# NealB/Bijective-BWT

Measured on AMD Instinct MI355X. Metric: BWTS build MB/s on 1 GiB input (+ inverse MB/s); bit-exact round-trip, higher is better.
Workload: dtype u8

## Files before the change

### bijective-bwt_amd/__init__.py

```python
import ctypes
import os
import subprocess

import numpy as np

PKG_DIR = os.path.dirname(os.path.abspath(__file__))
LIB_PATH = os.environ.get("BWTS_LIB_OVERRIDE") or os.path.join(PKG_DIR, "libbwts_hip.so")

KINDS = {"uniform256": 0, "zipf": 1, "dna": 2, "text": 3}

K_NAMES = ["histogram", "keybuild", "radix_hist", "radix_scan", "radix_scatter", "rerank", "lyndon", "emit",
           "lf_build", "walk", "listrank", "walk_emit", "other", "radix_scatter_main", "round"]
K_COUNT = len(K_NAMES)
MAX_ROUND_STATS = 40
H_NAMES = ["init", "module_load", "io_alloc", "staging_alloc", "arena_alloc"]
H_COUNT = len(H_NAMES)

EXPORTS = [
    "bwts_ctx_create", "bwts_ctx_destroy", "bwts_ctx_release_memory", "bwts_forward", "bwts_inverse", "bwts_forward_sink", "bwts_inverse_sink",
    "bwts_forward_device", "bwts_inverse_device", "bwts_last_timings", "bwts_kernel_class_name", "bwts_strerror",
    "bwts_last_hip_error", "bwts_set_timing", "bwts_host_alloc", "bwts_host_free", "bwts_host_cost_name",
    "bwts_forward_batch", "bwts_inverse_batch",
    "bwts_forward_segments", "bwts_inverse_segments", "bwts_forward_segments_device", "bwts_inverse_segments_device",
]
MTF_EXPORTS = [
    "bwts_mtf_forward_device", "bwts_mtf_inverse_device", "bwts_mtf_forward", "bwts_mtf_inverse",
    "bwts_mtf_forward_segments_device", "bwts_mtf_inverse_segments_device", "bwts_mtf_forward_segments", "bwts_mtf_inverse_segments",
]
EC_EXPORTS = [
    "bwts_ec_bound", "bwts_ec_bound_segments", "bwts_ec_decoded_size", "bwts_ec_encode_device", "bwts_ec_decode_device",
    "bwts_ec_encode", "bwts_ec_decode", "bwts_ec_encode_segments_device", "bwts_ec_decode_segments_device",
]
E_FORMAT, E_SPACE = -8, -9
ZRL_EXPORTS = [
    "bwts_zrl_bound", "bwts_zrl_encode_device", "bwts_zrl_decode_device", "bwts_zrl_encode", "bwts_zrl_decode",
    "bwts_zrl_encode_segments_device", "bwts_zrl_decode_segments_device",
]
PACK_EXPORTS = [
    "bwts_crc32_device", "bwts_crc32_segments_device", "bwts_pack_bound", "bwts_unpack_size",
    "bwts_pack_device", "bwts_unpack_device", "bwts_pack", "bwts_unpack",
    "bwts_pack_bound_v", "bwts_pack_device_v", "bwts_pack_v",
]
E_CHECKSUM = -10
TEST_EXPORTS = [
    "bwts_generate_device", "bwts_device_alloc", "bwts_device_free", "bwts_copy_to_device", "bwts_copy_to_host",
    "bwts_device_equal", "bwts_debug_sort_pairs", "bwts_debug_suffix_array", "bwts_debug_lyndon",
    "bwts_debug_chunk_plan", "bwts_debug_inverse_arena", "bwts_debug_forward_arena", "bwts_debug_wide_forward_arena", "bwts_debug_inverse_report",
    "bwts_debug_forward_report", "bwts_debug_segments_plan", "bwts_debug_segments_report",
    "bwts_debug_mtf_plan", "bwts_debug_last_spans", "bwts_debug_ec_plan", "bwts_debug_crc_plan",
    "bwts_debug_zrl_plan",
]
INV_REPORT_FIELDS = ["g", "mark", "outcome", "s", "virtual", "node_cap", "nu", "nu2", "ucap_first", "second_collect",
                     "listed_classes", "mom_fallback", "unit_rank", "kc", "kt", "form"]
INV_MARKS = {0: "log", 1: "sentinel", 2: "bytemap", 3: "moments"}
INV_OUTCOMES = {0: "DONE", 1: "RETRY_DENSE", 2: "AMBIGUOUS", 3: "NEED_LOG", 255: "ERROR"}
INV_FORMS = {0: "narrow", 1: "wide", 2: "wide_compact", 3: "segmented"}
SEG_PLANS = {0: "lane", 1: "shared", 2: "shared_nomem"}
FWD_HEADER_WORDS, FWD_ROUND_WORDS = 48, 12
FWD_SORT_WORDS = FWD_HEADER_WORDS + MAX_ROUND_STATS * FWD_ROUND_WORDS
FWD_HEADER_FIELDS = ["cyclic", "n", "k", "sigma", "bits", "msym", "key_bits", "varlen", "hstep", "keys", "flags_outside_rank", "tied0",
                     "rank_early", "form", "no_chunks", "need_sa", "end", "rest_chunks", "rest_big", "rest_tiles", "rounds", "directory",
                     "order_sort", "left"]
FWD_DIRECT_WORD = 36
FWD_DIRECT = {0: "not_tried", 1: "settled", 2: "fallback_group", 3: "fallback_depth"}
FWD_CHUNK_FIELDS = ["S", "maxchunks", "a_small", "big0", "m_exit", "m_stay", "groups", "wide_possible", "fsl", "compactions",
                    "compactions_skipped", "enqueued_behind_last"]
FWD_ROUND_FIELDS = {"sparse": ["form", "h", "in", "out", "splits", "probe", "m_big", "whole", "skip_next"],
                    "chunks": ["form", "h", "in", "out", "splits", "chunks_in", "chunks_out", "big_in", "big_stays", "big_leaves", "nchunks"],
                    "tiles": ["form", "h", "in", "out", "splits", "m_big"],
                    "direct": ["form", "h", "in", "out", "splits"]}
FWD_FORMS = {0: "none", 1: "sparse", 2: "chunks", 3: "tiles", 4: "direct"}
FWD_KEYS = {0: "wide", 1: "split32", 2: "split40"}
FWD_NO_CHUNKS = {0: None, 1: "short_list", 2: "knob", 3: "no_room_store", 4: "no_room_order", 5: "no_room_biglist"}
FWD_ENDS = {0: "none", 1: "empty", 2: "stable"}
FWD_PROBES = {0: "short_list", 1: "ran", 2: "skipped"}


class BwtsError(RuntimeError):
    def __init__(self, code, msg):
        super().__init__("bwts error %d: %s" % (code, msg))
        self.code = code


class KernelStat(ctypes.Structure):
    _fields_ = [("ms", ctypes.c_double), ("launches", ctypes.c_uint64), ("elems", ctypes.c_uint64),
                ("alg_bytes", ctypes.c_uint64)]


class Timings(ctypes.Structure):
    _fields_ = [("total_ms", ctypes.c_double), ("h2d_ms", ctypes.c_double), ("d2h_ms", ctypes.c_double),
                ("n", ctypes.c_uint64), ("factors", ctypes.c_uint64), ("rounds", ctypes.c_uint32),
                ("lyndon_rounds", ctypes.c_uint32), ("key_symbols", ctypes.c_uint32), ("key_bits", ctypes.c_uint32),
                ("active_after_round0", ctypes.c_uint64), ("unvisited", ctypes.c_uint64), ("device_bytes", ctypes.c_uint64),
                ("round_active", ctypes.c_uint64 * MAX_ROUND_STATS), ("k", KernelStat * K_COUNT),
                ("host_ms", ctypes.c_double * H_COUNT), ("attempts", ctypes.c_uint32), ("reserved_", ctypes.c_uint32)]

    def as_dict(self):
        d = {f: getattr(self, f) for f, _ in self._fields_ if f not in ("k", "round_active", "host_ms")}
        d["host_ms"] = {H_NAMES[i]: float(self.host_ms[i]) for i in range(H_COUNT)}
        d["round_active"] = [int(v) for v in self.round_active[: max(int(self.rounds), 1)]]
        d["kernels"] = {K_NAMES[i]: {"ms": self.k[i].ms, "launches": self.k[i].launches, "elems": self.k[i].elems,
                                     "alg_bytes": self.k[i].alg_bytes} for i in range(K_COUNT) if self.k[i].launches}
        return d


SINK_FN = ctypes.CFUNCTYPE(ctypes.c_int, ctypes.c_void_p, ctypes.c_void_p, ctypes.c_uint64)

_lib = None


def build(verbose=False):
    out = None if verbose else subprocess.DEVNULL
    subprocess.check_call(["make", "-C", PKG_DIR, "-j4", "all"], stdout=out)


def lib():
    global _lib
    if _lib is None:
        if not os.path.exists(LIB_PATH):
            raise BwtsError(-2, "libbwts_hip.so is not built (run `make -C bijective-bwt_amd` or __graft_entry__.build())")
        L = ctypes.CDLL(LIB_PATH)
        vp, u64, i32 = ctypes.c_void_p, ctypes.c_uint64, ctypes.c_int
        L.bwts_ctx_create.argtypes = [ctypes.POINTER(vp), i32]
        L.bwts_ctx_destroy.argtypes = [vp]
        L.bwts_ctx_destroy.restype = None
        L.bwts_ctx_release_memory.argtypes = [vp]
        L.bwts_ctx_release_memory.restype = ctypes.c_int
        for name in ("bwts_forward", "bwts_inverse", "bwts_forward_device", "bwts_inverse_device"):
            getattr(L, name).argtypes = [vp, vp, u64, vp]
        L.bwts_last_timings.argtypes = [vp, ctypes.POINTER(Timings)]
        L.bwts_kernel_class_name.argtypes = [i32]
        L.bwts_kernel_class_name.restype = ctypes.c_char_p
        L.bwts_strerror.argtypes = [i32]
        L.bwts_strerror.restype = ctypes.c_char_p
        L.bwts_last_hip_error.argtypes = [vp]
        L.bwts_set_timing.argtypes = [vp, i32]
        L.bwts_host_alloc.argtypes = [vp, u64, ctypes.POINTER(vp)]
        L.bwts_host_free.argtypes = [vp, vp]
        for name in ("bwts_forward_batch", "bwts_inverse_batch"):
            getattr(L, name).argtypes = [vp, i32, ctypes.POINTER(vp), ctypes.POINTER(u64), ctypes.POINTER(vp)]
        for name in ("bwts_forward_segments", "bwts_inverse_segments", "bwts_forward_segments_device", "bwts_inverse_segments_device"):
            getattr(L, name).argtypes = [vp, vp, vp, u64, vp]
        for name in ("bwts_mtf_forward", "bwts_mtf_inverse", "bwts_mtf_forward_device", "bwts_mtf_inverse_device"):
            getattr(L, name).argtypes = [vp, vp, u64, vp]
        for name in ("bwts_mtf_forward_segments", "bwts_mtf_inverse_segments", "bwts_mtf_forward_segments_device", "bwts_mtf_inverse_segments_device"):
            getattr(L, name).argtypes = [vp, vp, vp, u64, vp]
        L.bwts_debug_mtf_plan.argtypes = [u64, ctypes.POINTER(u64)]
        L.bwts_debug_last_spans.argtypes = [vp, ctypes.POINTER(ctypes.c_double), u64]
        L.bwts_ec_bound.argtypes = [u64]
        L.bwts_ec_bound.restype = u64
        L.bwts_ec_bound_segments.argtypes = [vp, u64, ctypes.POINTER(u64)]
        L.bwts_ec_decoded_size.argtypes = [vp, u64, ctypes.POINTER(u64)]
        for name in ("bwts_ec_encode_device", "bwts_ec_decode_device", "bwts_ec_encode", "bwts_ec_decode"):
            getattr(L, name).argtypes = [vp, vp, u64, vp, u64, ctypes.POINTER(u64)]
        L.bwts_ec_encode_segments_device.argtypes = [vp, vp, vp, u64, vp, u64, vp]
        L.bwts_ec_decode_segments_device.argtypes = [vp, vp, vp, vp, u64, vp]
        L.bwts_debug_ec_plan.argtypes = [u64, ctypes.POINTER(u64)]
        L.bwts_zrl_bound.argtypes = [u64]
        L.bwts_zrl_bound.restype = u64
        for name in ("bwts_zrl_encode_device", "bwts_zrl_encode"):
            getattr(L, name).argtypes = [vp, vp, u64, vp, u64, ctypes.POINTER(u64)]
        for name in ("bwts_zrl_decode_device", "bwts_zrl_decode"):
            getattr(L, name).argtypes = [vp, vp, u64, vp, u64]
        L.bwts_zrl_encode_segments_device.argtypes = [vp, vp, vp, u64, vp, u64, vp]
        L.bwts_zrl_decode_segments_device.argtypes = [vp, vp, vp, vp, u64, vp]
        L.bwts_debug_zrl_plan.argtypes = [u64, ctypes.POINTER(u64)]
        L.bwts_crc32_device.argtypes = [vp, vp, u64, ctypes.POINTER(ctypes.c_uint32)]
        L.bwts_crc32_segments_device.argtypes = [vp, vp, vp, u64, vp]
        L.bwts_pack_bound.argtypes = [u64, u64]
        L.bwts_pack_bound.restype = u64
        L.bwts_unpack_size.argtypes = [vp, u64, ctypes.POINTER(u64), ctypes.POINTER(u64)]
        for name in ("bwts_pack_device", "bwts_pack"):
            getattr(L, name).argtypes = [vp, vp, u64, u64, vp, u64, ctypes.POINTER(u64)]
        u32 = ctypes.c_uint32
        L.bwts_pack_bound_v.argtypes = [u32, u64, u64]
        L.bwts_pack_bound_v.restype = u64
        for name in ("bwts_pack_device_v", "bwts_pack_v"):
            getattr(L, name).argtypes = [vp, u32, vp, u64, u64, vp, u64, ctypes.POINTER(u64)]
        for name in ("bwts_unpack_device", "bwts_unpack"):
            getattr(L, name).argtypes = [vp, vp, u64, vp, u64, ctypes.POINTER(u64)]
        L.bwts_debug_crc_plan.argtypes = [u64, ctypes.POINTER(u64)]
        for name in ("bwts_forward_sink", "bwts_inverse_sink"):
            getattr(L, name).argtypes = [vp, vp, u64, SINK_FN, vp]
        L.bwts_generate_device.argtypes = [vp, i32, u64, u64, vp]
        L.bwts_device_alloc.argtypes = [vp, u64, ctypes.POINTER(vp)]
        L.bwts_device_free.argtypes = [vp, vp]
        L.bwts_copy_to_device.argtypes = [vp, vp, vp, u64]
        L.bwts_copy_to_host.argtypes = [vp, vp, vp, u64]
        L.bwts_device_equal.argtypes = [vp, vp, vp, u64, ctypes.POINTER(i32)]
        L.bwts_debug_sort_pairs.argtypes = [vp, vp, vp, u64, i32]
        L.bwts_debug_suffix_array.argtypes = [vp, vp, u64, vp]
        L.bwts_debug_lyndon.argtypes = [vp, vp, u64, vp, u64, ctypes.POINTER(u64)]
        L.bwts_debug_chunk_plan.argtypes = [u64, u64, ctypes.POINTER(u64)]
        L.bwts_debug_inverse_arena.argtypes = [u64, i32, i32, ctypes.POINTER(u64)]
        L.bwts_debug_forward_arena.argtypes = [u64, ctypes.POINTER(u64)]
        L.bwts_debug_wide_forward_arena.argtypes = [u64, i32, i32, u64, ctypes.POINTER(u64)]
        L.bwts_debug_inverse_report.argtypes = [vp, ctypes.POINTER(u64), u64, ctypes.POINTER(u64)]
        L.bwts_debug_forward_report.argtypes = [vp, ctypes.POINTER(u64), u64, ctypes.POINTER(u64)]
        L.bwts_debug_segments_plan.argtypes = [vp, u64, ctypes.POINTER(u64)]
        L.bwts_debug_segments_report.argtypes = [vp, ctypes.POINTER(u64)]
        _lib = L
    return _lib


def _u8(data):
    if isinstance(data, np.ndarray):
        return np.ascontiguousarray(data, dtype=np.uint8)
    return np.frombuffer(bytes(data), dtype=np.uint8)


class DeviceBuffer:

    def __init__(self, ctx, nbytes):
        self.ctx, self.nbytes = ctx, int(nbytes)
        p = ctypes.c_void_p()
        ctx._check(lib().bwts_device_alloc(ctx._h, self.nbytes, ctypes.byref(p)))
        self.ptr = p.value

    def free(self):
        if self.ptr:
            lib().bwts_device_free(self.ctx._h, self.ptr)
            self.ptr = None

    def upload(self, data):
        a = _u8(data)
        assert a.size <= self.nbytes
        self.ctx._check(lib().bwts_copy_to_device(self.ctx._h, self.ptr, a.ctypes.data, a.size))

    def download(self, nbytes=None):
        n = self.nbytes if nbytes is None else int(nbytes)
        out = np.empty(n, dtype=np.uint8)
        self.ctx._check(lib().bwts_copy_to_host(self.ctx._h, out.ctypes.data, self.ptr, n))
        return out


class Context:

    def __init__(self, device=0):
        self._h = None
        h = ctypes.c_void_p()
        rc = lib().bwts_ctx_create(ctypes.byref(h), int(device))
        if rc != 0:
            raise BwtsError(rc, lib().bwts_strerror(rc).decode())
        self._h = h
        self.device = int(device)

    def close(self):
        if self._h:
            lib().bwts_ctx_destroy(self._h)
            self._h = None

    def __enter__(self):
        return self

    def __exit__(self, *exc):
        self.close()

    def __del__(self):
        try:
            self.close()
        except Exception:
            pass

    def release_memory(self):
        self._check(lib().bwts_ctx_release_memory(self._h))

    def _check(self, rc):
        if rc != 0:
            msg = lib().bwts_strerror(rc).decode()
            if rc == -4:
                msg += " (hipError %d)" % lib().bwts_last_hip_error(self._h)
            raise BwtsError(rc, msg)

    def _host(self, fn, data):
        a = _u8(data)
        if a.size == 0:
            raise BwtsError(-1, "empty input (the reference fails on empty files: map_file.c:36-40)")
        out = np.empty_like(a)
        self._check(fn(self._h, a.ctypes.data, a.size, out.ctypes.data))
        return out

    def forward(self, data):
        return self._host(lib().bwts_forward, data)

    def inverse(self, data):
        return self._host(lib().bwts_inverse, data)

    def forward_device(self, d_in, n, d_out):
        self._check(lib().bwts_forward_device(self._h, _ptr(d_in), int(n), _ptr(d_out)))

    def inverse_device(self, d_in, n, d_out):
        self._check(lib().bwts_inverse_device(self._h, _ptr(d_in), int(n), _ptr(d_out)))

    def set_timing(self, level=2):
        self._check(lib().bwts_set_timing(self._h, int(level)))

    def _sink(self, fn, data):
        a = _u8(data)
        pieces = []

        def take(_user, ptr, length):
            pieces.append(ctypes.string_at(ptr, length))
            return 0

        cb = SINK_FN(take)
        self._check(fn(self._h, a.ctypes.data, a.size, cb, None))
        return np.frombuffer(b"".join(pieces), dtype=np.uint8)

    def forward_sink(self, data):
        return self._sink(lib().bwts_forward_sink, data)

    def inverse_sink(self, data):
        return self._sink(lib().bwts_inverse_sink, data)

    def host_alloc(self, nbytes):
        p = ctypes.c_void_p()
        self._check(lib().bwts_host_alloc(self._h, int(nbytes), ctypes.byref(p)))
        arr = np.ctypeslib.as_array(ctypes.cast(p, ctypes.POINTER(ctypes.c_uint8)), shape=(int(nbytes),))
        return arr, p.value

    def host_free(self, ptr):
        self._check(lib().bwts_host_free(self._h, ptr))

    def _batch(self, fn, arrays):
        arrs = [_u8(a) for a in arrays]
        outs = [np.empty_like(a) for a in arrs]
        k = len(arrs)
        ins_p = (ctypes.c_void_p * k)(*[a.ctypes.data for a in arrs])
        outs_p = (ctypes.c_void_p * k)(*[o.ctypes.data for o in outs])
        ns = (ctypes.c_uint64 * k)(*[a.size for a in arrs])
        self._check(fn(self._h, k, ins_p, ns, outs_p))
        return outs

    def forward_batch(self, arrays):
        return self._batch(lib().bwts_forward_batch, arrays)

    def inverse_batch(self, arrays):
        return self._batch(lib().bwts_inverse_batch, arrays)

    def _segments(self, fn, data, lengths, out=None):
        a = _u8(data)
        ls = np.ascontiguousarray(lengths, dtype=np.uint64)
        if int(ls.sum(dtype=np.uint64)) != a.size or (ls.size and int(ls.max()) > a.size):
            raise BwtsError(-1, "segment lengths do not add up to the input's size")
        if out is None:
            out = np.empty_like(a)
        elif out.size < a.size:
            raise BwtsError(-1, "output smaller than the input")
        self._check(fn(self._h, a.ctypes.data, ls.ctypes.data, ls.size, out.ctypes.data))
        return out

    def forward_segments(self, data, lengths, out=None):
        return self._segments(lib().bwts_forward_segments, data, lengths, out)

    def inverse_segments(self, data, lengths, out=None):
        return self._segments(lib().bwts_inverse_segments, data, lengths, out)

    def forward_segments_device(self, d_in, lengths, d_out):
        ls = np.ascontiguousarray(lengths, dtype=np.uint64)
        self._check(lib().bwts_forward_segments_device(self._h, _ptr(d_in), ls.ctypes.data, ls.size, _ptr(d_out)))

    def inverse_segments_device(self, d_in, lengths, d_out):
        ls = np.ascontiguousarray(lengths, dtype=np.uint64)
        self._check(lib().bwts_inverse_segments_device(self._h, _ptr(d_in), ls.ctypes.data, ls.size, _ptr(d_out)))

    def mtf_forward(self, data):
        return self._host(lib().bwts_mtf_forward, data)

    def mtf_inverse(self, data):
        return self._host(lib().bwts_mtf_inverse, data)

    def mtf_forward_device(self, d_in, n, d_out):
        self._check(lib().bwts_mtf_forward_device(self._h, _ptr(d_in), int(n), _ptr(d_out)))

    def mtf_inverse_device(self, d_in, n, d_out):
        self._check(lib().bwts_mtf_inverse_device(self._h, _ptr(d_in), int(n), _ptr(d_out)))

    def mtf_forward_segments(self, data, lengths, out=None):
        return self._segments(lib().bwts_mtf_forward_segments, data, lengths, out)

    def mtf_inverse_segments(self, data, lengths, out=None):
        return self._segments(lib().bwts_mtf_inverse_segments, data, lengths, out)

    def mtf_forward_segments_device(self, d_in, lengths, d_out):
        ls = np.ascontiguousarray(lengths, dtype=np.uint64)
        self._check(lib().bwts_mtf_forward_segments_device(self._h, _ptr(d_in), ls.ctypes.data, ls.size, _ptr(d_out)))

    def mtf_inverse_segments_device(self, d_in, lengths, d_out):
        ls = np.ascontiguousarray(lengths, dtype=np.uint64)
        self._check(lib().bwts_mtf_inverse_segments_device(self._h, _ptr(d_in), ls.ctypes.data, ls.size, _ptr(d_out)))

    def ec_encode(self, data, out_cap=None):
        a = _u8(data)
        if a.size == 0:
            raise BwtsError(-1, "empty input")
        out = np.empty(ec_bound(a.size) if out_cap is None else int(out_cap), dtype=np.uint8)
        got = ctypes.c_uint64(0)
        self._check(lib().bwts_ec_encode(self._h, a.ctypes.data, a.size, out.ctypes.data, out.size, ctypes.byref(got)))
        return out[:got.value].copy()

    def ec_decode(self, stream):
        a = _u8(stream)
        n = ec_decoded_size(a)
        out = np.empty(n, dtype=np.uint8)
        got = ctypes.c_uint64(0)
        self._check(lib().bwts_ec_decode(self._h, a.ctypes.data, a.size, out.ctypes.data, out.size, ctypes.byref(got)))
        return out[:got.value]

    def ec_encode_device(self, d_in, n, d_out, out_cap):
        got = ctypes.c_uint64(0)
        self._check(lib().bwts_ec_encode_device(self._h, _ptr(d_in), int(n), _ptr(d_out), int(out_cap), ctypes.byref(got)))
        return int(got.value)

    def ec_decode_device(self, d_in, in_bytes, d_out, out_cap):
        got = ctypes.c_uint64(0)
        self._check(lib().bwts_ec_decode_device(self._h, _ptr(d_in), int(in_bytes), _ptr(d_out), int(out_cap), ctypes.byref(got)))
        return int(got.value)

    def ec_encode_segments_device(self, d_in, lengths, d_out, out_cap):
        ls = np.ascontiguousarray(lengths, dtype=np.uint64)
        sizes = np.zeros(ls.size, dtype=np.uint64)
        self._check(lib().bwts_ec_encode_segments_device(self._h, _ptr(d_in), ls.ctypes.data, ls.size, _ptr(d_out), int(out_cap), sizes.ctypes.data))
        return sizes

    def ec_decode_segments_device(self, d_in, stream_bytes, lengths, d_out):
        ls = np.ascontiguousarray(lengths, dtype=np.uint64)
        sb = np.ascontiguousarray(stream_bytes, dtype=np.uint64)
        if sb.size != ls.size:
            raise BwtsError(-1, "one stream size per segment")
        self._check(lib().bwts_ec_decode_segments_device(self._h, _ptr(d_in), sb.ctypes.data, ls.ctypes.data, ls.size, _ptr(d_out)))

    def zrl_encode(self, data, out_cap=None):
        a = _u8(data)
        if a.size == 0:
            raise BwtsError(-1, "empty input")
        out = np.empty(a.size if out_cap is None else int(out_cap), dtype=np.uint8)
        got = ctypes.c_uint64(0)
        self._check(lib().bwts_zrl_encode(self._h, a.ctypes.data, a.size, out.ctypes.data, out.size, ctypes.byref(got)))
        return out[:got.value].copy()

    def zrl_decode(self, coded, n):
        a = _u8(coded)
        out = np.empty(int(n), dtype=np.uint8)
        self._check(lib().bwts_zrl_decode(self._h, a.ctypes.data, a.size, out.ctypes.data, out.size))
        return out

    def zrl_encode_device(self, d_in, n, d_out, out_cap):
        got = ctypes.c_uint64(0)
        self._check(lib().bwts_zrl_encode_device(self._h, _ptr(d_in), int(n), _ptr(d_out), int(out_cap), ctypes.byref(got)))
        return int(got.value)

    def zrl_decode_device(self, d_in, in_bytes, d_out, n):
        self._check(lib().bwts_zrl_decode_device(self._h, _ptr(d_in), int(in_bytes), _ptr(d_out), int(n)))

    def zrl_encode_segments_device(self, d_in, lengths, d_out, out_cap):
        ls = np.ascontiguousarray(lengths, dtype=np.uint64)
        sizes = np.zeros(ls.size, dtype=np.uint64)
        self._check(lib().bwts_zrl_encode_segments_device(self._h, _ptr(d_in), ls.ctypes.data, ls.size, _ptr(d_out), int(out_cap), sizes.ctypes.data))
        return sizes

    def zrl_decode_segments_device(self, d_in, in_lengths, lengths, d_out):
        ls = np.ascontiguousarray(lengths, dtype=np.uint64)
        il = np.ascontiguousarray(in_lengths, dtype=np.uint64)
        if il.size != ls.size:
            raise BwtsError(-1, "one coded length per segment")
        self._check(lib().bwts_zrl_decode_segments_device(self._h, _ptr(d_in), il.ctypes.data, ls.ctypes.data, ls.size, _ptr(d_out)))

    def crc32_device(self, d_in, n):
        got = ctypes.c_uint32(0)
        self._check(lib().bwts_crc32_device(self._h, _ptr(d_in), int(n), ctypes.byref(got)))
        return int(got.value)

    def crc32_segments_device(self, d_in, lengths):
        ls = np.ascontiguousarray(lengths, dtype=np.uint64)
        crcs = np.zeros(ls.size, dtype=np.uint32)
        self._check(lib().bwts_crc32_segments_device(self._h, _ptr(d_in), ls.ctypes.data, ls.size, crcs.ctypes.data))
        return crcs

    def pack(self, data, block_bytes=0, out_cap=None, version=1):
        a = _u8(data)
        if a.size == 0:
            raise BwtsError(-1, "empty input")
        out = np.empty(pack_bound(a.size, block_bytes, version) if out_cap is None else int(out_cap), dtype=np.uint8)
        got = ctypes.c_uint64(0)
        self._check(lib().bwts_pack_v(self._h, int(version), a.ctypes.data, a.size, int(block_bytes), out.ctypes.data, out.size, ctypes.byref(got)))
        return out[:got.value].copy()

    def unpack(self, frame, out=None):
        a = _u8(frame)
        if out is None:
            out = np.empty(unpack_size(a)[0], dtype=np.uint8)
        got = ctypes.c_uint64(0)
        self._check(lib().bwts_unpack(self._h, a.ctypes.data, a.size, out.ctypes.data, out.size, ctypes.byref(got)))
        return out[:got.value]

    def pack_device(self, d_in, n, block_bytes, d_out, out_cap, version=1):
        got = ctypes.c_uint64(0)
        self._check(lib().bwts_pack_device_v(self._h, int(version), _ptr(d_in), int(n), int(block_bytes), _ptr(d_out), int(out_cap), ctypes.byref(got)))
        return int(got.value)

    def unpack_device(self, d_in, in_bytes, d_out, out_cap):
        got = ctypes.c_uint64(0)
        self._check(lib().bwts_unpack_device(self._h, _ptr(d_in), int(in_bytes), _ptr(d_out), int(out_cap), ctypes.byref(got)))
        return int(got.value)

    def forward_into(self, a, out):
        self._check(lib().bwts_forward(self._h, a.ctypes.data, a.size, out.ctypes.data))

    def inverse_into(self, a, out):
        self._check(lib().bwts_inverse(self._h, a.ctypes.data, a.size, out.ctypes.data))

    def timings(self):
        t = Timings()
        self._check(lib().bwts_last_timings(self._h, ctypes.byref(t)))
        return t

    def alloc(self, nbytes):
        return DeviceBuffer(self, nbytes)

    def generate(self, kind, seed, n, d_out):
        self._check(lib().bwts_generate_device(self._h, KINDS[kind], int(seed), int(n), _ptr(d_out)))

    def device_equal(self, d_a, d_b, nbytes):
        eq = ctypes.c_int(0)
        self._check(lib().bwts_device_equal(self._h, _ptr(d_a), _ptr(d_b), int(nbytes), ctypes.byref(eq)))
        return bool(eq.value)

    def debug_sort_pairs(self, keys, vals, key_bits=64):
        k = np.ascontiguousarray(keys, dtype=np.uint64).copy()
        v = np.ascontiguousarray(vals, dtype=np.uint32).copy()
        self._check(lib().bwts_debug_sort_pairs(self._h, k.ctypes.data, v.ctypes.data, k.size, int(key_bits)))
        return k, v

    def debug_suffix_array(self, data):
        a = _u8(data)
        sa = np.empty(a.size, dtype=np.uint32)
        self._check(lib().bwts_debug_suffix_array(self._h, a.ctypes.data, a.size, sa.ctypes.data))
        return sa

    def debug_lyndon(self, data):
        a = _u8(data)
        st = np.empty(a.size, dtype=np.uint64)
        cnt = ctypes.c_uint64(0)
        self._check(lib().bwts_debug_lyndon(self._h, a.ctypes.data, a.size, st.ctypes.data, st.size, ctypes.byref(cnt)))
        return st[: cnt.value].copy()

    def debug_last_spans(self, cap=4096):
        buf = (ctypes.c_double * cap)()
        got = lib().bwts_debug_last_spans(self._h, buf, cap)
        if got < 0:
            self._check(got)
        return [float(buf[i]) for i in range(got)]

    def debug_inverse_report(self):
        words = len(INV_REPORT_FIELDS)
        buf = (ctypes.c_uint64 * (8 * words))()
        made = ctypes.c_uint64(0)
        got = lib().bwts_debug_inverse_report(self._h, buf, len(buf), ctypes.byref(made))
        if got < 0:
            self._check(got)
        assert got == made.value, "more attempts than records: %d" % made.value
        out = []
        for a in range(got):
            d = {f: int(buf[a * words + i]) for i, f in enumerate(INV_REPORT_FIELDS)}
            d["mark"], d["outcome"], d["form"] = INV_MARKS[d["mark"]], INV_OUTCOMES[d["outcome"]], INV_FORMS[d["form"]]
            for f in ("second_collect", "unit_rank"):
                d[f] = bool(d[f])
            out.append(d)
        return out

    def debug_segments_report(self):
        buf = (ctypes.c_uint64 * 8)()
        self._check(lib().bwts_debug_segments_report(self._h, buf))
        d = _segments_words(buf)
        d["attempts"] = int(buf[7])
        return d

    def debug_forward_report(self):
        buf = (ctypes.c_uint64 * (2 * FWD_SORT_WORDS))()
        made = ctypes.c_uint64(0)
        got = lib().bwts_debug_forward_report(self._h, buf, len(buf), ctypes.byref(made))
        if got < 0:
            self._check(got)
        out = []
        for a in range(got):
            w = [int(v) for v in buf[a * FWD_SORT_WORDS:(a + 1) * FWD_SORT_WORDS]]
            d = {f: w[i] for i, f in enumerate(FWD_HEADER_FIELDS)}
            d["form"], d["keys"], d["no_chunks"], d["end"] = FWD_FORMS[d["form"]], FWD_KEYS[d["keys"]], FWD_NO_CHUNKS[d["no_chunks"]], FWD_ENDS[d["end"]]
            d["direct"], d["direct_word"] = FWD_DIRECT[w[FWD_DIRECT_WORD]], w[FWD_DIRECT_WORD]
            for f in ("cyclic", "varlen", "flags_outside_rank", "rank_early", "need_sa", "order_sort"):
                d[f] = bool(d[f])
            if d["form"] == "chunks":
                d["chunks"] = {f: w[24 + i] for i, f in enumerate(FWD_CHUNK_FIELDS)}
                for f in ("wide_possible", "fsl", "enqueued_behind_last"):
                    d["chunks"][f] = bool(d["chunks"][f])
            d["round"] = []
            for r in range(min(max(d["rounds"] - 1, 0), MAX_ROUND_STATS)):
                rw = w[FWD_HEADER_WORDS + r * FWD_ROUND_WORDS:FWD_HEADER_WORDS + (r + 1) * FWD_ROUND_WORDS]
                form = FWD_FORMS[rw[0]]
                rd = {f: rw[i] for i, f in enumerate(FWD_ROUND_FIELDS[form])}
                rd["form"] = form
                if form == "sparse":
                    rd["probe"], rd["whole"], rd["skip_next"] = FWD_PROBES[rd["probe"]], bool(rd["whole"]), bool(rd["skip_next"])
                d["round"].append(rd)
            out.append(d)
        return out


def _segments_words(w):
    plan = SEG_PLANS[int(w[0])]
    own = "shared" if plan == "shared" else "lane"
    d = {"plan": plan, "big": int(w[1]), "runs": int(w[2]), "lane_segments": 0, "lane_bytes": 0, "shared_segments": 0, "shared_bytes": 0,
         "single_segments": int(w[5]), "single_bytes": int(w[6])}
    d[own + "_segments"], d[own + "_bytes"] = int(w[3]), int(w[4])
    return d


def debug_segments_plan(lengths):
    ls = np.ascontiguousarray(lengths, dtype=np.uint64)
    buf = (ctypes.c_uint64 * 8)()
    if lib().bwts_debug_segments_plan(ls.ctypes.data, ls.size, buf) < 0:
        raise BwtsError(-1, "bad segment lengths")
    d = _segments_words(buf)
    d["arena_bytes"] = int(buf[7])
    return d


def debug_mtf_plan(n):
    buf = (ctypes.c_uint64 * 4)()
    if lib().bwts_debug_mtf_plan(int(n), buf) < 0:
        raise BwtsError(-1, "bad length")
    return {"T": int(buf[0]), "G": int(buf[1]), "tiles": int(buf[2]), "groups": int(buf[3])}


def debug_ec_plan(n):
    buf = (ctypes.c_uint64 * 5)()
    if lib().bwts_debug_ec_plan(int(n), buf) < 0:
        raise BwtsError(-1, "bad length")
    return {"T": int(buf[0]), "K": int(buf[1]), "tiles": int(buf[2]), "blocks": int(buf[3]), "bound": int(buf[4])}


def debug_crc_plan(n):
    buf = (ctypes.c_uint64 * 4)()
    if lib().bwts_debug_crc_plan(int(n), buf) < 0:
        raise BwtsError(-1, "bad length")
    return {"T": int(buf[0]), "G": int(buf[1]), "tiles": int(buf[2]), "groups": int(buf[3])}


def debug_zrl_plan(n):
    buf = (ctypes.c_uint64 * 2)()
    if lib().bwts_debug_zrl_plan(int(n), buf) < 0:
        raise BwtsError(-1, "bad length")
    return {"T": int(buf[0]), "tiles": int(buf[1])}


def zrl_bound(n):
    b = int(lib().bwts_zrl_bound(int(n)))
    if b == 0:
        raise BwtsError(-5 if int(n) > 0 else -1, "no bound for this length")
    return b


def pack_bound(n, block_bytes=0, version=1):
    b = int(lib().bwts_pack_bound_v(int(version), int(n), int(block_bytes)))
    if b == 0:
        raise BwtsError(-5 if int(n) > (1 << 32) else -1, "no bound for these arguments")
    return b


def unpack_size(frame):
    a = _u8(frame)
    n, fb = ctypes.c_uint64(0), ctypes.c_uint64(0)
    rc = lib().bwts_unpack_size(a.ctypes.data, a.size, ctypes.byref(n), ctypes.byref(fb))
    if rc != 0:
        raise BwtsError(rc, lib().bwts_strerror(rc).decode())
    return int(n.value), int(fb.value)


def ec_bound(n):
    b = int(lib().bwts_ec_bound(int(n)))
    if b == 0:
        raise BwtsError(-5 if int(n) > 0 else -1, "no bound for this length")
    return b


def ec_bound_segments(lengths):
    ls = np.ascontiguousarray(lengths, dtype=np.uint64)
    got = ctypes.c_uint64(0)
    rc = lib().bwts_ec_bound_segments(ls.ctypes.data, ls.size, ctypes.byref(got))
    if rc != 0:
        raise BwtsError(rc, lib().bwts_strerror(rc).decode())
    return int(got.value)


def ec_decoded_size(stream):
    a = _u8(stream)
    head = np.zeros(16, dtype=np.uint8)
    head[:min(a.size, 16)] = a[:16]
    got = ctypes.c_uint64(0)
    rc = lib().bwts_ec_decoded_size(head.ctypes.data, a.size, ctypes.byref(got))
    if rc != 0:
        raise BwtsError(rc, lib().bwts_strerror(rc).decode())
    return int(got.value)


def _ptr(x):
    if isinstance(x, DeviceBuffer):
        return x.ptr
    if hasattr(x, "data_ptr"):
        return x.data_ptr()
    return int(x)


def mk_bwts(data, device=0):
    with Context(device) as ctx:
        return ctx.forward(data)


def unbwts(data, device=0):
    with Context(device) as ctx:
        return ctx.inverse(data)
```

### bijective-bwt_amd/csrc/forward.hip

```cpp
#include "internal.h"
#include "device_utils.h"
#include "scan_templ.h"

#include <math.h>
#include <stdio.h>
#include <stdlib.h>
#include <string.h>
#include <vector>

#define SM_HIST      0
#define SM_CODES     256
#define SM_COUNTERS  320
#define   CNT_ACTIVE   (SM_COUNTERS + 0)
#define   CNT_SPLITS   (SM_COUNTERS + 1)
#define   CNT_TOTAL    (SM_COUNTERS + 2)
#define   CNT_CAND     (SM_COUNTERS + 4)
#define   CNT_LYN_K    (SM_COUNTERS + 5)
#define   CNT_LYN_OVF  (SM_COUNTERS + 6)

struct Alphabet {
    int sigma;
    int bits;
    int msym;
    int key_bits;
    int pad_add;
    bool varlen;
    int hstep;
    int patch_span;
};
#define SM_DGCNT  2816
#define SM_SEGCNT 2560
#define SM_VTAB 2048
#define VL_MAXLEN 24

static int bitlen_u64(u64 x) { int b = 0; while (x) { b++; x >>= 1; } return b; }

#define BH_COPIES 16
__global__ __launch_bounds__(256) void byte_hist_kernel(const u8 *__restrict__ T, u64 n, u64 *__restrict__ hist)
{
    __shared__ u32 bins[BH_COPIES][256];
    const int tid = threadIdx.x;
    u32 *mine = bins[tid & (BH_COPIES - 1)];
    for (int i = tid; i < BH_COPIES * 256; i += 256) ((u32 *)bins)[i] = 0;
    __syncthreads();
    const u64 nvec = n / 16;
    const uint4 *T16 = (const uint4 *)T;
    const bool aligned = ((uintptr_t)T & 15) == 0;
    if (aligned) {
        for (u64 v = (u64)blockIdx.x * 256 + tid; v < nvec; v += (u64)gridDim.x * 256) {
            const uint4 q = T16[v];
            const u32 ws[4] = {q.x, q.y, q.z, q.w};
#pragma unroll
            for (int a = 0; a < 4; a++) {
#pragma unroll
                for (int b = 0; b < 4; b++) atomicAdd(&mine[(ws[a] >> (8 * b)) & 255u], 1u);
            }
        }
        for (u64 i = nvec * 16 + (u64)blockIdx.x * 256 + tid; i < n; i += (u64)gridDim.x * 256) atomicAdd(&mine[T[i]], 1u);
    } else {
        for (u64 i = (u64)blockIdx.x * 256 + tid; i < n; i += (u64)gridDim.x * 256) atomicAdd(&mine[T[i]], 1u);
    }
    __syncthreads();
    u32 s = 0;
#pragma unroll
    for (int c = 0; c < BH_COPIES; c++) s += bins[c][tid];
    if (s) atomicAdd((unsigned long long *)&hist[tid], (unsigned long long)s);
}

int byte_histogram_device(bwts_ctx *ctx, const u8 *d_T, u64 n, u64 *d_hist256)
{
    HIPC(hipMemsetAsync(d_hist256, 0, 256 * sizeof(u64), ctx->stream));
    u64 blocks = (n + 256 * 64 - 1) / (256 * 64);
    if (blocks > 2048) blocks = 2048;
    if (blocks < 1) blocks = 1;
    SpanGuard g(ctx, BWTS_K_HISTOGRAM, n, n);
    byte_hist_kernel<<<dim3((unsigned)blocks), dim3(256), 0, ctx->stream>>>(d_T, n, d_hist256);
    HIPC(hipGetLastError());
    return BWTS_OK;
}

static int read_histogram(bwts_ctx *ctx, const u8 *d_T, u64 n)
{
    BWTS_TRY(byte_histogram_device(ctx, d_T, n, ctx->d_small + SM_HIST));
    return read_small(ctx, SM_HIST, 256);
}

static int pick_key_symbols(const u64 *hist, u64 n, int bits, int max_sym)
{
    double sum2 = 0.0;
    for (int c = 0; c < 256; c++) { const double p = (double)hist[c] / (double)n; sum2 += p * p; }
    if (sum2 >= 1.0) return max_sym;
    const double H2 = -log2(sum2);
    const double need = log2((double)n) + 8.0;
    int m = (int)ceil(need / H2 - 0.05);
    if (m < 1) m = 1;
    if (m > max_sym) return max_sym;
    const int passes = (m * bits + 7) / 8;
    while (m < max_sym && ((m + 1) * bits + 7) / 8 <= passes) m++;
    return m;
}

#define KEY_SAMPLES (1u << 17)
#define CNT_SAMPLE (SM_COUNTERS + 16)
__global__ void sample_keys_kernel(const u8 *T, u64 n, const u64 *vtab, u32 samples, u64 *out);
__global__ void count_prefix_matches_kernel(const u64 *keys, u32 samples, unsigned long long *counters);

static int build_alphabetic_code(const u64 *hist, u64 n, u32 *code, u8 *len, double *avg_len, double *entropy, double smooth_scale = 1.0)
{
    std::vector<double> Cv(256 * 256);
    std::vector<u16> Rv(256 * 256);
    double (*C)[256] = (double (*)[256])Cv.data();
    u16 (*R)[256] = (u16 (*)[256])Rv.data();
    int sym[256], sigma = 0;
    double w[256], pre[257];
    for (int c = 0; c < 256; c++) { code[c] = 0; len[c] = 0; if (hist[c]) sym[sigma++] = c; }
    const double smooth = ((double)(n >> 14) + 1.0) * smooth_scale;
    pre[0] = 0;
    for (int i = 0; i < sigma; i++) { w[i] = (double)hist[sym[i]] + smooth; pre[i + 1] = pre[i] + w[i]; }
    if (sigma == 1) { len[sym[0]] = 1; *avg_len = 1; *entropy = 0; return 1; }
    for (int i = 0; i < sigma; i++) { C[i][i] = 0; R[i][i] = (u16)i; }
    for (int L = 2; L <= sigma; L++) {
        for (int i = 0; i + L - 1 < sigma; i++) {
            const int j = i + L - 1;
            int lo = R[i][j - 1], hi = R[i + 1][j];
            if (lo < i) lo = i;
            if (hi > j - 1) hi = j - 1;
            if (hi < lo) hi = lo;
            double best = 1e300; int arg = lo;
            for (int k = lo; k <= hi; k++) {
                const double v = C[i][k] + C[k + 1][j];
                if (v < best) { best = v; arg = k; }
            }
            C[i][j] = best + (pre[j + 1] - pre[i]);
            R[i][j] = (u16)arg;
        }
    }
    struct Item { int i, j, depth; u32 prefix; } stack[512];
    int sp = 0, lmax = 0;
    stack[sp++] = Item{0, sigma - 1, 0, 0u};
    while (sp) {
        const Item it = stack[--sp];
        if (it.i == it.j) {
            len[sym[it.i]] = (u8)it.depth; code[sym[it.i]] = it.prefix;
            if (it.depth > lmax) lmax = it.depth;
            continue;
        }
        if (it.depth >= 31) return 99;
        const int k = R[it.i][it.j];
        stack[sp++] = Item{k + 1, it.j, it.depth + 1, (it.prefix << 1) | 1u};
        stack[sp++] = Item{it.i, k, it.depth + 1, it.prefix << 1};
    }
    double al = 0, h = 0;
    for (int i = 0; i < sigma; i++) {
        const double p = (double)hist[sym[i]] / (double)n;
        al += p * len[sym[i]];
        h -= p * log2(p);
    }
    *avg_len = al; *entropy = h;
    return lmax;
}

static void fixed_codes(const u64 *hist, bool reserve_pad, u8 codes[256], Alphabet *al)
{
    int sigma = 0;
    for (int c = 0; c < 256; c++) codes[c] = hist[c] ? (u8)(sigma++ + (reserve_pad ? 1 : 0)) : (u8)0;
    const int ncodes = sigma + (reserve_pad ? 1 : 0);
    al->sigma = sigma;
    al->bits = bitlen_u64((u64)(ncodes > 1 ? ncodes - 1 : 1));
    al->pad_add = 0;
    if (al->bits > 8) {
        for (int c = 0, s = 0; c < 256; c++) if (hist[c]) codes[c] = (u8)(s++);
        al->pad_add = 1;
    }
}

static int iid_key_bits(const u64 *hist, const u8 *vlen, const u32 *vcode, u64 n, double share[65])
{
    double p[256];
    for (int c = 0; c < 256; c++) p[c] = (double)hist[c] / (double)n;
    share[0] = 1.0;
    for (int b = 1; b <= 64; b++) {
        double s = 0.0;
        for (int c = 0; c < 256; c++)
            if (vlen[c] && vlen[c] <= b) s += p[c] * p[c] * share[b - vlen[c]];
        double mass = 0.0; u32 cur = 0; bool open = false;
        for (int c = 0; c < 256; c++) {
            if (!vlen[c] || vlen[c] <= b) continue;
            const u32 pc = vcode[c] >> (vlen[c] - b);
            if (open && pc == cur) mass += p[c];
            else { s += mass * mass; mass = p[c]; cur = pc; open = true; }
        }
        s += mass * mass;
        share[b] = s;
    }
    for (int b = 32; b <= 64; b += 8)
        if ((double)n * share[b] <= 1.0 / 128.0) return b;
    return 64;
}

static int sampled_key_bits(bwts_ctx *ctx, const u8 *d_T, u64 n, const SortBufs &scratch, const u64 *vtab, const double share[65], int *kb_emp)
{
    HIPC(hipMemcpyAsync(ctx->d_small + SM_VTAB, vtab, 256 * sizeof(u64), hipMemcpyHostToDevice, ctx->stream));
    HIPC(hipMemsetAsync(ctx->d_small + CNT_SAMPLE, 0, 8 * sizeof(u64), ctx->stream));
    SpanGuard g(ctx, BWTS_K_KEYBUILD, KEY_SAMPLES, 0);
    sample_keys_kernel<<<dim3(KEY_SAMPLES / 256), dim3(256), 0, ctx->stream>>>(d_T, n, ctx->d_small + SM_VTAB, KEY_SAMPLES, scratch.keys[0]);
    int sres = 0;
    BWTS_TRY(radix_sort_pairs(ctx, scratch.plan(), KEY_SAMPLES, 64, &sres));
    count_prefix_matches_kernel<<<dim3(KEY_SAMPLES / 256), dim3(256), 0, ctx->stream>>>(
        scratch.keys[sres], KEY_SAMPLES, (unsigned long long *)(ctx->d_small + CNT_SAMPLE));
    HIPC(hipGetLastError());
    BWTS_TRY(read_small(ctx, CNT_SAMPLE, 5));
    const double pairs = 0.5 * (double)KEY_SAMPLES * (double)KEY_SAMPLES;
    *kb_emp = 64;
    for (int b = 32, w = 1; b <= 56; b += 8, w++) {
        const double m = (double)ctx->h_small[CNT_SAMPLE + w];
        const double partners = m >= 8.0 ? (double)n * m / pairs : (double)n * share[b];
        if (1.0 - exp(-partners) <= 1.0 / 64.0) { *kb_emp = b; break; }
    }
    return BWTS_OK;
}

static int set_alphabet(bwts_ctx *ctx, bool reserve_pad, u64 n, Alphabet *al, const u8 *d_T = nullptr, const SortBufs *scratch = nullptr)
{
    const u64 *hist = ctx->h_small + SM_HIST;
    u8 codes[256];
    fixed_codes(hist, reserve_pad, codes, al);
    const int bits = al->bits;
    int msym = pick_key_symbols(hist, n, bits, 64 / bits);
    const char *env = bwts_knob(ctx, "BWTS_KEY_SYMBOLS");
    if (env) { int v = atoi(env); if (v >= 1 && v <= 64 / bits) msym = v; else if (v == 0) msym = 64 / bits; }
    al->msym = al->hstep = msym; al->key_bits = bits * msym; al->varlen = false; al->patch_span = msym - 1;
    const char *vl = bwts_knob(ctx, "BWTS_VARLEN");
    u32 vcode[256]; u8 vlen[256];
    double avg = 0, ent = 0;
    const bool try_vl = !reserve_pad && al->sigma > 1 && !(vl && vl[0] == '0') && !(env && !vl);
    const int lmax = try_vl ? build_alphabetic_code(hist, n, vcode, vlen, &avg, &ent) : 0;
    if (try_vl && lmax <= VL_MAXLEN) {
        u64 *vtab = ctx->h_small + SM_VTAB;
        for (int c = 0; c < 256; c++) vtab[c] = ((u64)vlen[c] << 32) | vcode[c];
        double share[65];
        int kb = iid_key_bits(hist, vlen, vcode, n, share), kb_emp = 0;
        if (d_T && scratch && n >= (1ull << 22)) BWTS_TRY(sampled_key_bits(ctx, d_T, n, *scratch, vtab, share, &kb_emp));
        if (kb_emp > kb) {
            const int keep = 40;
            if (keep / lmax >= 4) kb = keep;
            else {
                kb = kb_emp;
                al->msym = al->hstep = 64 / bits; al->key_bits = bits * al->msym; al->patch_span = al->msym - 1;
            }
        }
        const char *kbe = bwts_knob(ctx, "BWTS_KEY_BITS");
        if (kbe) { int v = atoi(kbe); if (v >= 8 && v >= lmax && v <= 64) kb = v; }
        const int passes_fixed = (al->key_bits + 7) / 8, passes_var = (kb + 7) / 8;
        if ((vl && vl[0] == '1') || passes_var < passes_fixed || (passes_var == passes_fixed && avg < (double)bits - 0.25)) {
            al->varlen = true; al->key_bits = kb; al->patch_span = 64;
            al->msym = al->hstep = kb / lmax < 1 ? 1 : kb / lmax;
            HIPC(hipMemcpyAsync(ctx->d_small + SM_VTAB, vtab, 256 * sizeof(u64), hipMemcpyHostToDevice, ctx->stream));
        }
    }
    memcpy(ctx->h_small + SM_CODES, codes, 256);
    HIPC(hipMemcpyAsync(ctx->d_small + SM_CODES, ctx->h_small + SM_CODES, 256, hipMemcpyHostToDevice, ctx->stream));
    HIPC(hipStreamSynchronize(ctx->stream));
    return BWTS_OK;
}

__device__ __forceinline__ u64 factor_of(const u32 *__restrict__ fstart, u64 k, u64 p)
{
    u64 lo = 0, hi = k - 1;
    while (lo < hi) {
        const u64 mid = (lo + hi + 1) >> 1;
        if ((u64)fstart[mid] <= p) lo = mid; else hi = mid - 1;
    }
    return lo;
}
__device__ __forceinline__ u64 factor_end(const u32 *__restrict__ fstart, u64 k, u64 n, u64 f)
{
    return f + 1 < k ? (u64)fstart[f + 1] : n;
}

struct KeyStore { u64 *wide; u32 *lo; u8 *c; bool c16; u8 *wprev;  };
__device__ __forceinline__ void ks_store(const KeyStore &ks, u64 i, u64 key)
{
    if (ks.wide) ks.wide[i] = key;
    else { ks.lo[i] = (u32)key; if (ks.c16) ks.c[2 * i] = (u8)(key >> 32); }
}
__device__ __forceinline__ void ks_store_with_prev(const KeyStore &ks, u64 i, u64 key, u32 prev)
{
    if (ks.wide) { ks.wide[i] = key; if (ks.wprev) ks.wprev[i] = (u8)prev; }
    else {
        ks.lo[i] = (u32)key;
        if (ks.c16) ((u16 *)ks.c)[i] = (u16)(((u32)(key >> 32) & 255u) | (prev << 8));
        else ks.c[i] = (u8)prev;
    }
}
__device__ __forceinline__ u64 ks_load(const KeyStore &ks, u64 i)
{
    return ks.wide ? ks.wide[i] : ((u64)ks.lo[i] | (ks.c16 ? (u64)ks.c[2 * i] << 32 : 0ull));
}
static KeyStore key_store_of(u64 *keys0, u64 n, bool split, int key_bits)
{
    KeyStore ks;
    ks.wide = split ? nullptr : keys0;
    ks.lo = (u32 *)keys0;
    ks.c = (u8 *)keys0 + align_up((size_t)n * 4, 256);
    ks.c16 = key_bits > 32;
    ks.wprev = nullptr;
    return ks;
}
__global__ __launch_bounds__(256) void carried_head_fix_kernel(const u8 *__restrict__ T, u64 n, const u32 *__restrict__ fstart, u64 k, KeyStore ks);

#define KB_THREADS 256
#define KB_ITEMS   8
#define KB_TILE    (KB_THREADS * KB_ITEMS)
#define KB_HALO    64

#define KB_RX_TILE 8192
#define KB_SUB     (KB_RX_TILE / KB_TILE)
__device__ __forceinline__ void kb_hist_clear(u32 (*bins)[256])
{
    for (int i = threadIdx.x; i < KB_THREADS / 64 * 256; i += KB_THREADS) ((u32 *)bins)[i] = 0;
}
__device__ __forceinline__ void kb_hist_flush(u32 (*bins)[256], u32 *__restrict__ hist0)
{
    __syncthreads();
    u32 s = 0;
#pragma unroll
    for (int w = 0; w < KB_THREADS / 64; w++) s += bins[w][threadIdx.x];
    hist0[(u64)blockIdx.x * 256 + threadIdx.x] = s;
}
static_assert(KB_THREADS == 256, "one thread per digit of the first pass's table row");

__global__ __launch_bounds__(KB_THREADS) void keybuild0_kernel(const u8 *__restrict__ T, u64 n, const u8 *__restrict__ codes_g,
                                                               int bits, int msym, int pad_add,
                                                               KeyStore keys, u64 *__restrict__ tile_min , u64 pos0, u64 lim,
                                                               u32 *__restrict__ hist0)
{
    __shared__ u16 sc[KB_TILE + KB_HALO + 16];
    __shared__ u64 skey[KB_TILE + KB_TILE / 8];
    __shared__ u8 codes[256];
    __shared__ u64 wmin[KB_THREADS / 64];
    __shared__ __attribute__((aligned(16))) u8 sraw[KB_TILE + KB_HALO + 16];
    __shared__ u8 before_tile;
    __shared__ u32 bins[KB_THREADS / 64][256];

    const int tid = threadIdx.x;
    codes[tid] = codes_g[tid];
    if (hist0) kb_hist_clear(bins);
    const int key_bits = bits * msym;
    const u64 mask = key_bits >= 64 ? ~0ull : ((1ull << key_bits) - 1ull);

    for (int sub = 0; sub < KB_SUB; sub++) {
        const u64 tile = (u64)blockIdx.x * KB_SUB + (u64)sub;
        const u64 base = pos0 + tile * KB_TILE;
        if (base >= lim) break;
        const u64 end = base + KB_TILE < lim ? base + KB_TILE : lim;
        __syncthreads();
        if (tid == 0) before_tile = base ? T[base - 1] : T[n - 1];

        const u32 span = (u32)(end - base) + (u32)msym;
        const bool vec_ok = ((uintptr_t)T & 15) == 0;
        for (u32 c = tid; c * 16 < span; c += KB_THREADS) {
            const u64 q0 = base + (u64)c * 16;
            if (vec_ok && q0 + 16 <= n) {
                const uint4 v = *(const uint4 *)(T + q0);
                *(uint4 *)(sraw + c * 16) = v;
                const u32 w[4] = {v.x, v.y, v.z, v.w};
#pragma unroll
                for (int a = 0; a < 4; a++)
#pragma unroll
                    for (int bb = 0; bb < 4; bb++)
                        sc[c * 16 + a * 4 + bb] = (u16)((u32)codes[(w[a] >> (8 * bb)) & 255u] + (u32)pad_add);
            } else {
                for (int bb = 0; bb < 16; bb++) {
                    const u64 q = q0 + bb;
                    const u8 t = q < n ? T[q] : (u8)0;
                    sraw[c * 16 + bb] = t;
                    sc[c * 16 + bb] = q < n ? (u16)((u32)codes[t] + (u32)pad_add) : (u16)0;
                }
            }
        }
        __syncthreads();
        const u32 o = (u32)tid * KB_ITEMS;
        u64 lo = ~0ull;
        if (base + o < end) {
            u64 key = 0;
            for (int j = 0; j < msym; j++) key = (key << bits) | sc[o + j];
#pragma unroll
            for (int e = 0; e < KB_ITEMS; e++) {
                if (base + o + e < end) {
                    skey[o + e + ((o + e) >> 3)] = key;
                    lo = key < lo ? key : lo;
                    key = ((key << bits) | sc[o + e + msym]) & mask;
                }
            }
        }
        if (tile_min) {
            lo = wave_scan_inclusive(lo, OpMin());
            if (lane_id() == 63) wmin[wave_id()] = lo;
        }
        __syncthreads();
#pragma unroll
        for (int j = 0; j < KB_ITEMS; j++) {
            const u32 e = (u32)j * KB_THREADS + tid;
            const bool valid = base + e < end;
            u64 key = 0;
            if (valid) {
                const u64 q = base + e;
                key = skey[e + (e >> 3)];
                const u32 prev = e ? (u32)sraw[e - 1] : (u32)before_tile;
                ks_store_with_prev(keys, q - pos0, key, prev);
            }
            if (hist0) hist_add_runs(bins[wave_id()], (u32)key & 255u, valid);
        }
        if (tile_min && tid == 0) {
            u64 t = wmin[0];
            for (int w = 1; w < KB_THREADS / 64; w++) t = wmin[w] < t ? wmin[w] : t;
            tile_min[tile] = t;
        }
    }
    if (hist0) kb_hist_flush(bins, hist0);
}

__device__ __forceinline__ u64 vl_key_plain(const u8 *__restrict__ T, u64 n, const u64 *__restrict__ vtab, int key_bits, u64 q)
{
    u64 acc = 0;
    int filled = 0;
    while (filled < key_bits) {
        if (q >= n) { acc <<= (key_bits - filled); break; }
        const u64 e = vtab[T[q++]];
        const int l = (int)(e >> 32), room = key_bits - filled;
        const u64 c = (u32)e;
        if (l <= room) { acc = (acc << l) | c; filled += l; }
        else { acc = (acc << room) | (c >> (l - room)); filled = key_bits; }
    }
    return acc;
}
__device__ __forceinline__ u64 vl_key_cyclic(const u8 *__restrict__ T, const u64 *__restrict__ vtab, int key_bits, u64 q, u64 s, u64 e_)
{
    u64 acc = 0;
    int filled = 0;
    while (filled < key_bits) {
        const u64 e = vtab[T[q]];
        if (++q == e_) q = s;
        const int l = (int)(e >> 32), room = key_bits - filled;
        const u64 c = (u32)e;
        if (l <= room) { acc = (acc << l) | c; filled += l; }
        else { acc = (acc << room) | (c >> (l - room)); filled = key_bits; }
    }
    return acc;
}

struct __attribute__((packed, aligned(1))) TextChunk16 { u64 w[2]; };
__device__ __forceinline__ u64 vl_key_cyclic_fast(const u8 *__restrict__ T, const u64 *vtab_lds, const u64 *__restrict__ vtab_g, int key_bits,
                                                  u64 q, u64 s, u64 e_)
{
    if (q + 16 > e_) return vl_key_cyclic(T, vtab_g, key_bits, q, s, e_);
    const TextChunk16 ch = *(const TextChunk16 *)(T + q);
    u64 acc = 0;
    int filled = 0;
#pragma unroll
    for (int b = 0; b < 16; b++) {
        if (filled < key_bits) {
            const u32 sym = (u32)((b < 8 ? ch.w[0] >> (8 * b) : ch.w[1] >> (8 * (b - 8))) & 255u);
            const u64 e = vtab_lds[sym];
            const int l = (int)(e >> 32), room = key_bits - filled;
            const u64 c = (u32)e;
            if (l <= room) { acc = (acc << l) | c; filled += l; }
            else { acc = (acc << room) | (c >> (l - room)); filled = key_bits; }
        }
    }
    if (filled < key_bits) return vl_key_cyclic(T, vtab_g, key_bits, q, s, e_);
    return acc;
}

__global__ __launch_bounds__(256) void sample_keys_kernel(const u8 *__restrict__ T, u64 n, const u64 *__restrict__ vtab, u32 samples,
                                                          u64 *__restrict__ out)
{
    const u32 i = blockIdx.x * 256 + threadIdx.x;
    if (i >= samples) return;
    const u64 pos = (((u64)i * 0x9E3779B97F4A7C15ull) >> 11) % n;
    out[i] = vl_key_plain(T, n, vtab, 64, pos);
}
__global__ __launch_bounds__(256) void count_prefix_matches_kernel(const u64 *__restrict__ keys, u32 samples,
                                                                   unsigned long long *__restrict__ counters)
{
    const u32 i = blockIdx.x * 256 + threadIdx.x;
    const bool ok = i > 0 && i < samples;
    const u64 a = ok ? keys[i] : 0, b = ok ? keys[i - 1] : ~0ull;
#pragma unroll
    for (int w = 0; w < 5; w++) {
        const int bits = 24 + 8 * w;
        const u64 m = __ballot(ok && (a >> (64 - bits)) == (b >> (64 - bits)));
        if (m && lane_id() == 0) atomicAdd(&counters[w], (unsigned long long)__popcll(m));
    }
}

#define KB_SYMS      (KB_TILE + KB_HALO)
#define KB_SYM_PER   ((KB_SYMS + KB_THREADS - 1) / KB_THREADS)
#define KB_BS_WORDS  ((KB_SYMS * VL_MAXLEN + 31) / 32 + 4)
__global__ __launch_bounds__(KB_THREADS) void keybuild0v_kernel(const u8 *__restrict__ T, u64 n, const u64 *__restrict__ vtab_g,
                                                                int key_bits, KeyStore keys, u64 *__restrict__ tile_min, u64 pos0, u64 lim,
                                                                u32 *__restrict__ hist0)
{
    __shared__ u64 vtab[256];
    __shared__ __attribute__((aligned(16))) u8 sb[KB_SYMS + 16];
    __shared__ u32 bs[KB_BS_WORDS];
    __shared__ u16 symoff[KB_SYMS + 8];
    __shared__ u64 wmin[KB_THREADS / 64];
    __shared__ u32 scan_sm[KB_THREADS / 64];
    __shared__ u8 before_tile;
    __shared__ u32 bins[KB_THREADS / 64][256];

    const int tid = threadIdx.x;
    vtab[tid] = vtab_g[tid];
    if (hist0) kb_hist_clear(bins);
    for (int sub = 0; sub < KB_SUB; sub++) {
        const u64 tile = (u64)blockIdx.x * KB_SUB + (u64)sub;
        const u64 base = pos0 + tile * KB_TILE;
        if (base >= lim) break;
        const u64 end = base + KB_TILE < lim ? base + KB_TILE : lim;
        __syncthreads();
        if (tid == 0) before_tile = base ? T[base - 1] : T[n - 1];
        const u32 span = KB_SYMS;
        const u64 avail = n - base;
        const u32 nvalid = avail < span ? (u32)avail : span;
        const bool vec_ok = ((uintptr_t)T & 15) == 0;
        for (u32 c = tid; c * 16 < span; c += KB_THREADS) {
            const u64 q0 = base + (u64)c * 16;
            if (vec_ok && q0 + 16 <= n) {
                *(uint4 *)(sb + c * 16) = *(const uint4 *)(T + q0);
            } else {
                for (int bb = 0; bb < 16; bb++) sb[c * 16 + bb] = q0 + bb < n ? T[q0 + bb] : (u8)0;
            }
        }
        for (u32 i = tid; i < KB_BS_WORDS; i += KB_THREADS) bs[i] = 0;
        __syncthreads();

        const u32 s0 = (u32)tid * KB_SYM_PER;
        u32 ent_len[KB_SYM_PER], ent_code[KB_SYM_PER];
        u32 mine = 0;
#pragma unroll
        for (int i = 0; i < KB_SYM_PER; i++) {
            const u32 sidx = s0 + i;
            u64 ent = 0;
            if (sidx < nvalid) ent = vtab[sb[sidx]];
            ent_len[i] = (u32)(ent >> 32);
            ent_code[i] = (u32)ent;
            mine += ent_len[i];
        }
        u32 total;
        u32 off = block_scan_exclusive<u32, OpAdd, KB_THREADS / 64>(mine, OpAdd(), 0u, scan_sm, &total);
#pragma unroll
        for (int i = 0; i < KB_SYM_PER; i++) {
            const u32 sidx = s0 + i;
            if (sidx < KB_SYMS) symoff[sidx] = (u16)off;
            const u32 l = ent_len[i];
            if (l) {
                const u32 wd = off >> 5, r = off & 31u;
// ... 283 lines not shown
        *note = (f0 ? 1u : 0u) | (f1 ? 2u : 0u) | (so ? 4u : 0u);
        return ((u64)(f0 ? r.slot : 0u) << 32) | (u64)((f0 && f1) ? 0u : 1u);
    }
    __device__ __forceinline__ u64 operator()(u64 i, u32 *note) const { return make(i, load(i), note); }
    __device__ __forceinline__ u64 operator()(u64 i) const { u32 note; return make(i, load(i), &note); }
};

struct GroupOut {
    const u32 *S; const u32 *V; u64 a; int rb;
    const u64 *K;
    const u32 *tpos; u32 *trank; u64 a0;
    u32 *SA;
    u32 *n_idx, *n_slot, *n_head;
    u64 *cnt_active, *cnt_splits;
    __device__ __forceinline__ void operator()(u64 i, u64 v, u32 note) const
    {
        const bool f0 = note & 1u, f1 = note & 2u, same_old = note & 4u;
        const bool keep = !(f0 && f1);
        const u32 head = (u32)(v >> 32);
        const u32 val = V[i];
        const u32 slot = S[i];
        const bool moved = (u32)(K[i] >> rb) != head;
        if (tpos && moved) { const u64 j = tied_find(tpos, a0, val); if (j != ~0ull) trank[j] = head; }
        SA[slot] = val;
        if (keep) {
            const u32 dst = (u32)v - 1u;
            n_idx[dst] = val; n_slot[dst] = slot; n_head[dst] = head;
        }
        if (i + 1 == a) *cnt_active = ((u32)v == 0u && keep) ? 0x100000000ull : (u64)(u32)v;
        const u64 ms = __ballot(f0 && same_old);
        if (ms && lane_id() == __ffsll((unsigned long long)__ballot(true)) - 1 &&
            __hip_atomic_load(cnt_splits, __ATOMIC_RELAXED, __HIP_MEMORY_SCOPE_AGENT) == 0)
            __hip_atomic_store(cnt_splits, (u64)1, __ATOMIC_RELAXED, __HIP_MEMORY_SCOPE_AGENT);
    }
};

#define GF_WORDS 8
struct GfWide {
    const u64 *k; u64 mask;
    __device__ __forceinline__ u64 operator()(u64 i) const { return k[i] & mask; }
};
template <bool HI>
struct GfSplit {
    const u32 *lo; const u8 *hi;
    __device__ __forceinline__ u64 operator()(u64 i) const { return (u64)lo[i] | (HI ? (u64)hi[i] << 32 : 0ull); }
};
template <class KL>
__global__ __launch_bounds__(256) void group_flags_kernel(const KL K, u64 n, u64 *__restrict__ headw, u64 *__restrict__ keepw)
{
    const int lane = lane_id();
    const u64 words = (n + 63) / 64;
    const u64 wave = ((u64)blockIdx.x * 256 + threadIdx.x) >> 6, waves = ((u64)gridDim.x * 256) >> 6;
    for (u64 w0 = wave * GF_WORDS; w0 < words; w0 += waves * GF_WORDS) {
        u64 k[GF_WORDS];
#pragma unroll
        for (int q = 0; q < GF_WORDS; q++) {
            const u64 i = (w0 + q) * 64 + lane;
            k[q] = K(i < n ? i : n - 1);
        }
        const u64 first = w0 * 64, after = (w0 + GF_WORDS) * 64;
        const u64 before_key = K(first > 0 ? first - 1 : 0);
        const u64 after_key = K(after < n ? after : n - 1);
        u64 hm[GF_WORDS], vm[GF_WORDS];
        u64 prev63 = before_key;
#pragma unroll
        for (int q = 0; q < GF_WORDS; q++) {
            const u64 i = (w0 + q) * 64 + lane;
            const u32 lo = (u32)k[q], hi = (u32)(k[q] >> 32);
            const u32 plo = (u32)__builtin_amdgcn_update_dpp((int)lo, (int)lo, 0x138 , 0xf, 0xf, false);
            const u32 phi = (u32)__builtin_amdgcn_update_dpp((int)hi, (int)hi, 0x138, 0xf, 0xf, false);
            const bool valid = i < n;
            const bool diff = lane == 0 ? (i == 0 || k[q] != prev63) : (lo != plo || hi != phi);
            vm[q] = __ballot(valid);
            hm[q] = __ballot(!valid || diff);
            prev63 = ((u64)(u32)__builtin_amdgcn_readlane((int)hi, 63) << 32) | (u64)(u32)__builtin_amdgcn_readlane((int)lo, 63);
        }
        const bool after_starts = after >= n || after_key != prev63;
        u64 mine_h = 0, mine_k = 0;
#pragma unroll
        for (int q = 0; q < GF_WORDS; q++) {
            const u64 nextbit = q + 1 < GF_WORDS ? (hm[q + 1 < GF_WORDS ? q + 1 : q] & 1ull) : (after_starts ? 1ull : 0ull);
            const u64 lastm = (hm[q] >> 1) | (nextbit << 63);
            const u64 h = hm[q] & vm[q];
            if (lane == q) { mine_h = h; mine_k = vm[q] & ~(h & lastm); }
        }
        if (lane < GF_WORDS && w0 + lane < words) { headw[w0 + lane] = mine_h; keepw[w0 + lane] = mine_k; }
    }
}

struct WordIn {
    const u64 *headw, *keepw;
    __device__ __forceinline__ u64 operator()(u64 w) const
    {
        const u64 hm = headw[w], km = keepw[w];
        const u64 pos = hm ? w * 64 + (u64)(63 - __clzll((long long)hm)) : 0ull;
        return (pos << 32) | (u64)__popcll(km);
    }
};

__global__ __launch_bounds__(256) void tied_from_flags_kernel(const u64 *__restrict__ headw, const u64 *__restrict__ keepw,
                                                              const u64 *__restrict__ pre, u64 n, const u32 *__restrict__ V,
                                                              u32 *__restrict__ n_idx, u32 *__restrict__ n_slot, u32 *__restrict__ n_head,
                                                              u64 *__restrict__ cnt_active)
{
    const int lane = lane_id();
    const u64 words = (n + 63) / 64;
    const u64 wave = ((u64)blockIdx.x * 256 + threadIdx.x) >> 6, waves = ((u64)gridDim.x * 256) >> 6;
    for (u64 wb = wave * 64; wb < words; wb += waves * 64) {
        const u64 w = wb + lane;
        u64 hm = 0, km = 0, pr = 0;
        if (w < words) { hm = headw[w]; km = keepw[w]; pr = pre[w]; }
        if (w + 1 == words) *cnt_active = (u64)(u32)pr + (u64)__popcll(km);
        u64 todo = __ballot(km != 0);
        while (todo) {
            int q[4];
            u32 v[4];
#pragma unroll
            for (int t = 0; t < 4; t++) {
                q[t] = todo ? __ffsll((unsigned long long)todo) - 1 : -1;
                todo &= todo - 1;
            }
#pragma unroll
            for (int t = 0; t < 4; t++) {
                const u64 i = (wb + (u64)(q[t] < 0 ? 0 : q[t])) * 64 + lane;
                v[t] = V[i < n ? i : n - 1];
            }
#pragma unroll
            for (int t = 0; t < 4; t++) {
                if (q[t] < 0) continue;
                const u64 h = shfl_t(hm, q[t]), kk = shfl_t(km, q[t]), pq = shfl_t(pr, q[t]);
                if ((kk >> lane) & 1ull) {
                    const u64 i = (wb + q[t]) * 64 + lane;
                    const u64 below = lane == 63 ? h : h & ((2ull << lane) - 1ull);
                    const u32 head = below ? (u32)((wb + q[t]) * 64 + (u64)(63 - __clzll((long long)below))) : (u32)(pq >> 32);
                    const u32 dst = (u32)pq + (u32)__popcll(kk & lanemask_lt());
                    n_idx[dst] = v[t]; n_slot[dst] = (u32)i; n_head[dst] = head;
                }
            }
        }
    }
}

__global__ __launch_bounds__(256) void rank_from_sa_kernel(const u32 *__restrict__ SA, u64 n, u32 *__restrict__ rank)
{
    for (u64 i = (u64)blockIdx.x * 256 + threadIdx.x; i < n; i += (u64)gridDim.x * 256) rank[SA[i]] = (u32)i;
}
__global__ __launch_bounds__(256) void rank_from_list_kernel(const u32 *__restrict__ idx, const u32 *__restrict__ head, u64 a,
                                                             u32 *__restrict__ rank)
{
    const u64 i = (u64)blockIdx.x * 256 + threadIdx.x;
    if (i < a) rank[idx[i]] = head[i];
}

struct SortSpace : SortBufs {
    u32 *rank = nullptr;
    const u8 *carry_src = nullptr;
    u8 *carry_buf[2] = {nullptr, nullptr};
    u8 *carry_out = nullptr;
    bool want_split = false;
    bool split_keys = false;
    u32 *first_hist = nullptr;
    const u32 *tie_slots = nullptr;
    u64 tie_count = 0;
    bool ties_emitted = false;
};

static int ensure_rank(bwts_ctx *ctx, SortSpace &sp, u64 n)
{
    if (sp.rank) return BWTS_OK;
    char *p = nullptr;
    BWTS_TRY(aux_reserve_slot(ctx, 4, align_up((size_t)n * 4, 256), &p));
    sp.rank = (u32 *)p;
    return BWTS_OK;
}

__global__ __launch_bounds__(256) void rank_keys_kernel(const u32 *__restrict__ SA, u64 n, const u64 *__restrict__ headw,
                                                        const u64 *__restrict__ pre, u64 *__restrict__ keys)
{
    const int lane = lane_id();
    const u64 words = (n + 63) >> 6;
    const u64 wave = ((u64)blockIdx.x * 256 + threadIdx.x) >> 6, waves = ((u64)gridDim.x * 256) >> 6;
    for (u64 w0 = wave * 4; w0 < words; w0 += waves * 4) {
        u64 hm[4], pr[4];
        u32 sa[4];
#pragma unroll
        for (int q = 0; q < 4; q++) {
            const u64 w = w0 + q < words ? w0 + q : words - 1;
            const u64 i = (w << 6) + lane;
            hm[q] = headw[w]; pr[q] = pre[w];
            sa[q] = SA[i < n ? i : n - 1];
        }
#pragma unroll
        for (int q = 0; q < 4; q++) {
            const u64 w = w0 + q, i = (w << 6) + lane;
            if (w >= words || i >= n) continue;
            const u64 below = lane == 63 ? hm[q] : hm[q] & ((2ull << lane) - 1ull);
            const u32 h = below ? (u32)((w << 6) + (u64)(63 - __clzll((long long)below))) : (u32)(pr[q] >> 32);
            keys[i] = ((u64)h << 32) | (u64)sa[q];
        }
    }
}
#define RA_WLOG_MAX 14
__global__ __launch_bounds__(1024) void rank_apply_kernel(const u64 *__restrict__ keys, u64 n, int wlog, u32 *__restrict__ rank)
{
    extern __shared__ __attribute__((aligned(16))) u32 ra_img[];
    const u64 lo = (u64)blockIdx.x << wlog;
    const u64 hi = lo + (1ull << wlog) < n ? lo + (1ull << wlog) : n;
    for (u64 i = lo + threadIdx.x; i < hi; i += 1024) { const u64 kv = keys[i]; ra_img[(u32)kv - (u32)lo] = (u32)(kv >> 32); }
    __syncthreads();
    for (u64 i = lo + threadIdx.x; i < hi; i += 1024) rank[i] = ra_img[i - lo];
}
__global__ void count_tied_kernel(const u64 *__restrict__ keepw, const u64 *__restrict__ pre, u64 words, u64 *__restrict__ cnt_active)
{
    if (threadIdx.x == 0 && blockIdx.x == 0) *cnt_active = (u64)(u32)pre[words - 1] + (u64)__popcll(keepw[words - 1]);
}

#define SEG_CAP 8
#define SEG_HALO 8
#define SEG_OWN  (64 - SEG_HALO - SEG_CAP - 1)
__global__ __launch_bounds__(256) void seg_small_sort_kernel(const u32 *__restrict__ head, u64 *__restrict__ K, u32 *__restrict__ V, u64 a,
                                                             u8 *__restrict__ big, u64 *__restrict__ big_count)
{
    const int lane = lane_id();
    const u64 wave = ((u64)blockIdx.x * 256 + threadIdx.x) >> 6;
    const u64 own0 = wave * SEG_OWN;
    if (own0 >= a) return;
    const long long e = (long long)own0 - SEG_HALO + lane;
    const bool inside = e >= 0 && (u64)e < a;
    const u32 h = inside ? head[e] : 0u;
    u32 hp = (u32)__shfl_up((int)h, 1, 64);
    if (lane == 0) hp = (e > 0 && (u64)(e - 1) < a) ? head[e - 1] : 0u;
    const bool start = !inside || e == 0 || h != hp;
    const u64 starts = __ballot(start);
    const u64 below = lane == 63 ? starts : starts & ((2ull << lane) - 1ull);
    const int s_lane = below ? 63 - __clzll((long long)below) : -1;
    u32 sz = 0;
    bool too_big = s_lane < 0 || lane - s_lane >= SEG_CAP;
    if (!too_big) {
        const u64 above = s_lane == 63 ? 0ull : starts >> (s_lane + 1);
        const int e_lane = above ? s_lane + 1 + (__ffsll((unsigned long long)above) - 1) : 64;
        sz = (u32)(e_lane - s_lane);
        if (sz > SEG_CAP) too_big = true;
    }
    const bool owned = inside && lane >= SEG_HALO && lane < SEG_HALO + SEG_OWN;
    if (owned) big[e] = too_big ? 1 : 0;
    const u64 bm = __ballot(owned && too_big);
    if (bm && lane == 0) atomicAdd((unsigned long long *)&big_count[wave & 255], (unsigned long long)__popcll(bm));
    const bool member = inside && !too_big && sz >= 2 && s_lane >= SEG_HALO && s_lane < SEG_HALO + SEG_OWN;
    if (__ballot(member) == 0) return;
    u64 k = 0;
    u32 v = 0;
    if (member) { k = K[e]; v = V[e]; }
    const u32 o = member ? (u32)(lane - s_lane) : 0u;
    u32 rank = 0;
#pragma unroll
    for (int j = 0; j < SEG_CAP; j++) {
        const int src = (s_lane < 0 ? 0 : s_lane) + j;
        const u64 ko = shfl_t(k, src & 63);
        if (member && (u32)j < sz && (ko < k || (ko == k && (u32)j < o))) rank++;
    }
    if (member) { const u64 dst = (u64)e - o + rank; K[dst] = k; V[dst] = v; }
}
struct SegFlagIn {
    const u8 *big; const u32 *head;
    __device__ __forceinline__ u64 operator()(u64 i) const
    {
        const u32 f = big[i];
        const u32 st = f && (i == 0 || head[i] != head[i - 1]) ? 1u : 0u;
        return ((u64)st << 32) | f;
    }
};
struct SegBigOut {
    const u8 *big; const u32 *head; const u64 *K; const u32 *V; u64 a; int rb; u64 *bk; u32 *bv; u32 *bpos; u64 *count;
    __device__ __forceinline__ void operator()(u64 i, u64 before) const
    {
        const u32 f = big[i];
        if (f) {
            const u32 st = (i == 0 || head[i] != head[i - 1]) ? 1u : 0u;
            const u64 ord = (before >> 32) + st - 1;
            const u32 at = (u32)before;
            bk[at] = (ord << rb) | (K[i] & ((1ull << rb) - 1ull));
            bv[at] = V[i];
            bpos[at] = (u32)i;
        }
        if (i + 1 == a) *count = (u64)(u32)before + f;
    }
};
__global__ __launch_bounds__(256) void seg_writeback_kernel(const u64 *__restrict__ sk, const u32 *__restrict__ sv, const u32 *__restrict__ bpos,
                                                            u64 m, const u32 *__restrict__ head, int rb, u64 *__restrict__ K, u32 *__restrict__ V)
{
    const u64 j = (u64)blockIdx.x * 256 + threadIdx.x;
    if (j < m) {
        const u32 p = bpos[j];
        K[p] = ((u64)head[p] << rb) | (sk[j] & ((1ull << rb) - 1ull));
        V[p] = sv[j];
    }
}

enum FwdReportWord { FR_CYCLIC, FR_N, FR_K, FR_SIGMA, FR_BITS, FR_MSYM, FR_KEY_BITS, FR_VARLEN, FR_HSTEP, FR_KEYS, FR_FLAGS_OUTSIDE_RANK,
                     FR_TIED0, FR_RANK_EARLY, FR_FORM, FR_NO_CHUNKS, FR_NEED_SA, FR_END, FR_REST_CHUNKS, FR_REST_BIG, FR_REST_TILES,
                     FR_ROUNDS, FR_DIRECTORY, FR_ORDER_SORT, FR_LEFT,
                     FC_S = 24, FC_MAXCHUNKS, FC_A_SMALL, FC_BIG0, FC_M_EXIT, FC_M_STAY, FC_GROUPS, FC_WIDE_POSSIBLE, FC_FSL, FC_COMPACTIONS,
                     FC_COMPACTIONS_SKIPPED, FC_ENQUEUED_BEHIND_LAST,
                     FR_DIRECT = 36  };
enum FwdRoundWord { FRR_FORM, FRR_H, FRR_IN, FRR_OUT, FRR_SPLITS, FRR_PROBE = 5, FRR_MBIG, FRR_WHOLE, FRR_SKIP_NEXT,
                    FRR_CHUNKS_IN = 5, FRR_CHUNKS_OUT, FRR_BIG_IN, FRR_BIG_STAYS, FRR_BIG_LEAVES, FRR_NCHUNKS, FRR_TILE_MBIG = 5 };
enum FwdForm { FR_FORM_NONE, FR_FORM_SPARSE, FR_FORM_CHUNKS, FR_FORM_TILES, FR_FORM_DIRECT };
enum FwdNoChunks { FR_NC_NA, FR_NC_SHORT, FR_NC_KNOB, FR_NC_STORE, FR_NC_ORDER, FR_NC_BIGLIST };
enum FwdEnd { FR_END_NONE, FR_END_EMPTY, FR_END_STABLE };
static_assert(FC_ENQUEUED_BEHIND_LAST < FR_DIRECT && FR_DIRECT < FWD_HEADER_WORDS && FRR_NCHUNKS < FWD_ROUND_WORDS && FR_LEFT < FC_S, "the forward report's layout");
static u64 *fwd_report_open(bwts_ctx *ctx)
{
    u64 *w = ctx->fwd_report[ctx->fwd_sorts_made < FWD_REPORT_SORTS ? ctx->fwd_sorts_made : FWD_REPORT_SORTS - 1];
    memset(w, 0, FWD_SORT_WORDS * sizeof(u64));
    ctx->fwd_sorts_made++;
    return w;
}
static inline u64 *fwd_report_of(bwts_ctx *ctx) { assert(ctx->fwd_sorts_made > 0); return ctx->fwd_report[ctx->fwd_sorts_made < FWD_REPORT_SORTS ? ctx->fwd_sorts_made - 1 : FWD_REPORT_SORTS - 1]; }
static inline u64 *fwd_report_round(bwts_ctx *ctx, u32 rounds)
{
    return rounds >= 2 && rounds - 2 < BWTS_MAX_ROUND_STATS ? fwd_report_of(ctx) + FWD_HEADER_WORDS + (size_t)(rounds - 2) * FWD_ROUND_WORDS : nullptr;
}

#include "dense_rounds.h"
#include "chunk_rounds.h"

struct Round0 {
    int res;
    K0Keys k0v;
    u32 *SA;
    u64 *headw, *keepw, *pre;
    bool flags_outside_rank;
    u64 a;
};

template <bool CYCLIC>
static int round0_sort(bwts_ctx *ctx, u64 n, const Alphabet &al, SortSpace &sp, Round0 *r0)
{
    u64 *cnt = ctx->d_small + SM_COUNTERS;
    SortPlan plan = sp.plan();
    plan.sym_src = sp.carry_src; plan.sym_buf[0] = sp.carry_buf[0]; plan.sym_buf[1] = sp.carry_buf[1]; plan.sym_final = sp.carry_out;
    plan.vals_identity = true;
    plan.keys_split = CYCLIC && sp.split_keys && plan.sym_final;
    plan.first_hist = plan.keys_split ? sp.first_hist : nullptr;
    if (CYCLIC && sp.split_keys && !plan.keys_split) return BWTS_E_INTERNAL;
    int res = 0;
    STAGE("cyclic patch (before round 0)");
    BWTS_TRY(radix_sort_pairs(ctx, plan, n, al.key_bits, &res));
    STAGE("round-0 sort");
    u64 *K0 = sp.keys[res];
    K0Keys k0v{K0, nullptr, nullptr};
    if (plan.keys_split) k0v = K0Keys{nullptr, (const u32 *)K0, al.key_bits > 32 ? (const u8 *)K0 + align_up((size_t)n * 4, 256) : nullptr};

    HIPC(hipMemsetAsync(cnt, 0, 4 * sizeof(u64), ctx->stream));
    const u64 words = (n + 63) / 64;
    u64 *headw, *keepw, *pre;
    const bool flags_outside_rank = sp.carry_buf[0] && sp.carry_buf[1] && n >= 4096;
    {
        SpanGuard g(ctx, BWTS_K_RERANK, n, (k0v.wide ? 8 : k0v.hi ? 5 : 4) * n);
        if (flags_outside_rank) {
            headw = (u64 *)sp.carry_buf[0]; keepw = headw + words; pre = (u64 *)sp.carry_buf[1];
        } else {
            BWTS_TRY(ensure_rank(ctx, sp, n));
            headw = (u64 *)sp.rank; keepw = headw + words; pre = keepw + words;
        }
        u64 waves = (words + GF_WORDS - 1) / GF_WORDS;
        unsigned blocks = (unsigned)((waves + 3) / 4 < 16384 ? (waves + 3) / 4 : 16384);
        if (k0v.wide) group_flags_kernel<GfWide><<<dim3(blocks), dim3(256), 0, ctx->stream>>>(GfWide{K0, ~0ull}, n, headw, keepw);
        else if (k0v.hi) group_flags_kernel<GfSplit<true>><<<dim3(blocks), dim3(256), 0, ctx->stream>>>(GfSplit<true>{k0v.lo, k0v.hi}, n, headw, keepw);
        else group_flags_kernel<GfSplit<false>><<<dim3(blocks), dim3(256), 0, ctx->stream>>>(GfSplit<false>{k0v.lo, nullptr}, n, headw, keepw);
        WordIn in{headw, keepw};
        ScanStoreArr<u64> out{pre};
        BWTS_TRY((device_scan<false, u64>(ctx, words, in, out, OpHeadCount(), (u64)0, sp.scan_temp)));
        count_tied_kernel<<<dim3(1), dim3(64), 0, ctx->stream>>>(keepw, pre, words, cnt + 0);
        HIPC(hipGetLastError());
        STAGE("group flags + word scan + count");
    }
    BWTS_TRY(read_small(ctx, SM_COUNTERS, 4));
    *r0 = Round0{res, k0v, sp.vals[res], headw, keepw, pre, flags_outside_rank, ctx->h_small[CNT_ACTIVE]};
    return BWTS_OK;
}

static int early_ranks(bwts_ctx *ctx, u64 n, SortSpace &sp, const Round0 &r0)
{
    BWTS_TRY(ensure_rank(ctx, sp, n));
    SpanGuard g(ctx, BWTS_K_RERANK, n, 28 * n);
    u64 *rk[2] = {sp.keys[r0.res ^ 1], sp.keys[r0.res]};
    u64 blocks = (n + 255) / 256; if (blocks > 16384) blocks = 16384;
    rank_keys_kernel<<<dim3((unsigned)blocks), dim3(256), 0, ctx->stream>>>(r0.SA, n, r0.headw, r0.pre, rk[0]);
    HIPC(hipGetLastError());
    const int pb = bitlen_u64(n - 1);
    const int sbits = pb - 16 <= RA_WLOG_MAX ? 16 : 24;
    int rres = 0;
    BWTS_TRY(radix_sort_keys(ctx, rk, sp.tile_hist, sp.scan_temp, n, pb - sbits, sbits, &rres));
    const int wlog = RA_WLOG_MAX;
    BWTS_TRY(ensure_dyn_lds(ctx, (const void *)rank_apply_kernel, (size_t)4 << RA_WLOG_MAX));
    rank_apply_kernel<<<dim3((unsigned)((n + (1ull << wlog) - 1) >> wlog)), dim3(1024), (size_t)4 << wlog, ctx->stream>>>(rk[rres], n, wlog, sp.rank);
    HIPC(hipGetLastError());
    return BWTS_OK;
}

static int tied_list(bwts_ctx *ctx, u64 n, SortSpace &sp, const Round0 &r0, ActiveList *cur)
{
    u64 *cnt = ctx->d_small + SM_COUNTERS;
    cur->idx = (u32 *)sp.keys[r0.res ^ 1];
    cur->slot = cur->idx + n;
    cur->head = sp.vals[r0.res ^ 1];
    SpanGuard g(ctx, BWTS_K_RERANK, r0.a, 12 * r0.a);
    const u64 waves = ((n + 63) / 64 + 63) / 64;
    const unsigned blocks = (unsigned)((waves + 3) / 4 < 16384 ? (waves + 3) / 4 : 16384);
    tied_from_flags_kernel<<<dim3(blocks), dim3(256), 0, ctx->stream>>>(r0.headw, r0.keepw, r0.pre, n, r0.SA, cur->idx, cur->slot, cur->head, cnt + 0);
    HIPC(hipGetLastError());
    STAGE("tied list");
    sp.tie_slots = cur->slot;
    sp.tie_count = r0.a;
    return BWTS_OK;
}

#define DIRECT_GROUP 8
#define DIRECT_DEPTH 640u
#define DIRECT_POLL  64u
#define CNT_DIRECT   (SM_COUNTERS + 28)
enum FwdDirect { FR_DIRECT_NONE, FR_DIRECT_SETTLED, FR_DIRECT_GROUP, FR_DIRECT_DEEP };
static_assert(DIRECT_GROUP >= SEG_CAP, "the direct form takes every group the small-groups sort takes");

enum RotCmp { ROT_LESS, ROT_NOT_LESS, ROT_DEEP, ROT_STOP };
__device__ __forceinline__ RotCmp rotation_less(const u8 *__restrict__ T, u64 ps, u64 pl, u64 op, u64 qs, u64 ql, u64 oq, const u64 *flag)
{
    const u64 lim = pl + ql < DIRECT_DEPTH ? pl + ql : DIRECT_DEPTH;
    u64 next_poll = DIRECT_POLL;
    for (u64 d = 0; d < lim;) {
        if (pl - op >= 16 && ql - oq >= 16) {
            u64 x[2], y[2];
            __builtin_memcpy(x, T + ps + op, 16);
            __builtin_memcpy(y, T + qs + oq, 16);
            const int w = x[0] != y[0] ? 0 : 1;
            if (x[w] != y[w]) {
                const int sh = (__ffsll((unsigned long long)(x[w] ^ y[w])) - 1) & ~7;
                return ((x[w] >> sh) & 255u) < ((y[w] >> sh) & 255u) ? ROT_LESS : ROT_NOT_LESS;
            }
            op += 16; oq += 16; d += 16;
        } else {
            const u8 cp = T[ps + op], cq = T[qs + oq];
            if (cp != cq) return cp < cq ? ROT_LESS : ROT_NOT_LESS;
            op++; oq++; d++;
        }
        if (op == pl) op = 0;
        if (oq == ql) oq = 0;
        if (d >= next_poll) {
            if (__hip_atomic_load(flag, __ATOMIC_RELAXED, __HIP_MEMORY_SCOPE_AGENT)) return ROT_STOP;
            next_poll += DIRECT_POLL;
        }
    }
    return pl + ql > DIRECT_DEPTH ? ROT_DEEP : ROT_NOT_LESS;
}

__global__ __launch_bounds__(256) void direct_ties_kernel(const u32 *__restrict__ idx, const u32 *__restrict__ head, u64 a,
                                                          const u8 *__restrict__ T, u64 n, const u32 *__restrict__ fstart, u64 k, u64 skip,
                                                          u8 *__restrict__ out, u64 *flag)
{
    __shared__ u32 s_pos[DIRECT_GROUP][256], s_first[DIRECT_GROUP][256], s_last[DIRECT_GROUP][256];
    const int t = threadIdx.x;
    const u64 i = (u64)blockIdx.x * 256 + t;
    if (i >= a) return;
    const u32 h0 = head[i];
    if (i > 0 && head[i - 1] == h0) return;
    if (__hip_atomic_load(flag, __ATOMIC_RELAXED, __HIP_MEMORY_SCOPE_AGENT)) return;
    u32 cnt = 1;
    while (cnt <= DIRECT_GROUP && i + cnt < a && head[i + cnt] == h0) cnt++;
    if (cnt > DIRECT_GROUP) { atomicCAS((unsigned long long *)flag, 0ull, (unsigned long long)FR_DIRECT_GROUP); return; }
    for (u32 j = 0; j < cnt; j++) {
        const u32 p = idx[i + j];
        const u64 f = factor_of(fstart, k, p);
        s_pos[j][t] = p; s_first[j][t] = fstart[f]; s_last[j][t] = (u32)(factor_end(fstart, k, n, f) - 1);
    }
    for (u32 m = 1; m < cnt; m++) {
        const u32 p = s_pos[m][t], pf = s_first[m][t], pe = s_last[m][t];
        const u64 ps = pf, pl = (u64)pe - pf + 1, op = ((u64)p - pf + skip) % pl;
        u32 j = m;
        while (j > 0) {
            const u32 q = s_pos[j - 1][t], qf = s_first[j - 1][t], qe = s_last[j - 1][t];
            const u64 ql = (u64)qe - qf + 1;
            const RotCmp c = rotation_less(T, ps, pl, op, qf, ql, ((u64)q - qf + skip) % ql, flag);
            if (c == ROT_STOP) return;
            if (c == ROT_DEEP) { atomicCAS((unsigned long long *)flag, 0ull, (unsigned long long)FR_DIRECT_DEEP); return; }
            if (c != ROT_LESS) break;
            s_pos[j][t] = q; s_first[j][t] = qf; s_last[j][t] = qe;
            j--;
        }
        s_pos[j][t] = p; s_first[j][t] = pf; s_last[j][t] = pe;
    }
    for (u32 j = 0; j < cnt; j++) {
        const u32 p = s_pos[j][t];
        out[(u64)h0 + j] = T[p == s_first[j][t] ? s_last[j][t] : p - 1];
    }
}

static int direct_ties(bwts_ctx *ctx, const u8 *d_T, u64 n, const Alphabet &al, const u32 *d_fstart, u64 k, const SortSpace &sp,
                       const ActiveList &cur, u64 a, u64 *outcome)
{
    u64 *flag = ctx->d_small + CNT_DIRECT;
    HIPC(hipMemsetAsync(flag, 0, sizeof(u64), ctx->stream));
    {
        SpanGuard g(ctx, BWTS_K_RERANK, a, 24 * a);
        direct_ties_kernel<<<dim3((unsigned)((a + 255) / 256)), dim3(256), 0, ctx->stream>>>(cur.idx, cur.head, a, d_T, n, d_fstart, k, (u64)al.hstep,
                                                                                             sp.carry_out, flag);
        HIPC(hipGetLastError());
        STAGE("direct ties");
    }
    BWTS_TRY(read_small(ctx, CNT_DIRECT, 1));
    const u64 f = ctx->h_small[CNT_DIRECT];
    if (f != 0 && f != FR_DIRECT_GROUP && f != FR_DIRECT_DEEP) return BWTS_E_INTERNAL;
    *outcome = f ? f : (u64)FR_DIRECT_SETTLED;
    return BWTS_OK;
}
static bool direct_ties_allowed(const bwts_ctx *ctx, u64 n)
{
    int lg = 24;
    if (const char *e = bwts_knob(ctx, "BWTS_DIRECT_MIN_LOG2")) lg = atoi(e);
    if (lg < 0) lg = 0;
    return lg < 64 && n >= (1ull << lg);
}

struct SegBufs { u8 *big; u64 *bk[2]; u32 *bv[2], *bpos; };

static int seg_sort_round(bwts_ctx *ctx, SortSpace &sp, const SegBufs &sb, const u32 *head, u64 *K, u32 *V, u64 a, int rb, int round_key_bits,
                          bool *whole, bool *skip_next, u64 *m_big_out)
{
    u64 *cnt = ctx->d_small + SM_COUNTERS;
    u64 m_big = 0;
    {
        SpanGuard g(ctx, BWTS_K_RERANK, a, 20 * a);
        u64 *segcnt = ctx->d_small + SM_SEGCNT;
        HIPC(hipMemsetAsync(segcnt, 0, 256 * sizeof(u64), ctx->stream));
        const u64 waves = (a + SEG_OWN - 1) / SEG_OWN;
        seg_small_sort_kernel<<<dim3((unsigned)((waves + 3) / 4)), dim3(256), 0, ctx->stream>>>(head, K, V, a, sb.big, segcnt);
        HIPC(hipGetLastError());
    }
    BWTS_TRY(read_small(ctx, SM_SEGCNT, 256));
    for (int c = 0; c < 256; c++) m_big += ctx->h_small[SM_SEGCNT + c];
    if (m_big > a) return BWTS_E_INTERNAL;
    *m_big_out = m_big;
    *skip_next = m_big * 10 > a * 9;
    *whole = m_big * 5 > a * 4;
    if (*whole || !m_big) return BWTS_OK;
    {
        SpanGuard g(ctx, BWTS_K_RERANK, a, 20 * a);
        SegFlagIn fin{sb.big, head};
        SegBigOut fout{sb.big, head, K, V, a, rb, sb.bk[0], sb.bv[0], sb.bpos, cnt + 3};
        BWTS_TRY((device_scan<false, u64>(ctx, a, fin, fout, OpAdd(), (u64)0, sp.scan_temp)));
    }
    const SortPlan bp = sort_plan(sb.bk[0], sb.bk[1], sb.bv[0], sb.bv[1], sp.tile_hist, sp.scan_temp);
    int rbig = 0;
    const int big_bits = bitlen_u64(m_big / (SEG_CAP + 1)) + rb;
    BWTS_TRY(radix_sort_pairs(ctx, bp, m_big, big_bits < round_key_bits ? big_bits : round_key_bits, &rbig));
    SpanGuard g(ctx, BWTS_K_RERANK, m_big, 28 * m_big);
    seg_writeback_kernel<<<dim3((unsigned)((m_big + 255) / 256)), dim3(256), 0, ctx->stream>>>(sb.bk[rbig], sb.bv[rbig], sb.bpos, m_big, head, rb, K, V);
    HIPC(hipGetLastError());
    return BWTS_OK;
}

struct SparseRun {
    u64 *akeys[2], *dir_at;
    u32 *scratch, *tpos, *trank, *pdir_at;
    ActiveList sets[2];
    SegBufs sb;
    void declare(BlockLayout &L, u64 a)
    {
        L.arrays(a, &akeys[0], &akeys[1]); L.array(&scratch, a);
        for (int s = 0; s < 2; s++) L.arrays(a, &sets[s].idx, &sets[s].slot, &sets[s].head);
        L.arrays(a, &tpos, &trank);
        L.array(&dir_at, ((u64)1 << K0_DIR_LOG2_MAX) + 1); L.array(&pdir_at, ((u64)1 << K0_DIR_LOG2_MAX) + 2);
        L.array(&sb.big, a); L.arrays(a, &sb.bk[0], &sb.bk[1]); L.arrays(a, &sb.bv[0], &sb.bv[1], &sb.bpos);
    }
    u64 a0;
    int rb, round_key_bits;
    u64 *dir = nullptr;
    u32 *pdir = nullptr;
    int dlog = 0, psh = 0;
    ActiveList cur;
    u64 a, splits = 0;
    int nxt = 0;
    u32 rounds;
    bool seg_skip_next = false;
};

static int sparse_map(bwts_ctx *ctx, SparseRun &r, u64 n, const Alphabet &al, SortSpace &sp, const K0Keys &k0v)
{
    const u64 a = r.a0;
    SpanGuard g(ctx, BWTS_K_RERANK, a, 24 * a);
    const int kb = al.key_bits;
    r.dlog = kb < K0_DIR_LOG2_MAX ? kb : K0_DIR_LOG2_MAX;
    if (r.dlog > bitlen_u64(n)) r.dlog = bitlen_u64(n);
    if (r.dlog >= 8) {
        r.dir = r.dir_at;
        k0_directory_kernel<<<dim3((unsigned)(((1ull << r.dlog) + 1 + 255) / 256)), dim3(256), 0, ctx->stream>>>(k0v, n, kb, r.dlog, r.dir);
    }
    if (k0v.hi && (!r.dir || kb - r.dlog > 32)) return BWTS_E_INTERNAL;
    tied_map_keys_kernel<<<dim3((unsigned)((a + 255) / 256)), dim3(256), 0, ctx->stream>>>(r.cur.idx, a, r.akeys[0]);
    HIPC(hipMemcpyAsync(r.scratch, r.cur.head, a * sizeof(u32), hipMemcpyDeviceToDevice, ctx->stream));
    const SortPlan mp = sort_plan(r.akeys[0], r.akeys[1], r.scratch, r.trank, sp.tile_hist, sp.scan_temp);
    int mr = 0;
    BWTS_TRY(radix_sort_pairs(ctx, mp, a, bitlen_u64(n - 1) > 0 ? bitlen_u64(n - 1) : 1, &mr));
    tied_map_finish_kernel<<<dim3((unsigned)((a + 255) / 256)), dim3(256), 0, ctx->stream>>>(r.akeys[mr], a, r.tpos);
    if (mr == 0) HIPC(hipMemcpyAsync(r.trank, r.scratch, a * sizeof(u32), hipMemcpyDeviceToDevice, ctx->stream));
    fwd_report_of(ctx)[FR_DIRECTORY] = r.dir ? (u64)r.dlog : 0;
    if (r.dir) {
        const int pb = bitlen_u64(n - 1);
        r.psh = pb > K0_DIR_LOG2_MAX ? pb - K0_DIR_LOG2_MAX : 0;
        const u64 buckets = ((n - 1) >> r.psh) + 1;
        r.pdir = r.pdir_at;
        tpos_directory_kernel<<<dim3((unsigned)((buckets + 1 + 255) / 256)), dim3(256), 0, ctx->stream>>>(r.tpos, a, r.psh, buckets, r.pdir);
    }
    HIPC(hipGetLastError());
    return BWTS_OK;
}

template <bool CYCLIC>
static int sparse_round(bwts_ctx *ctx, SparseRun &r, const u8 *d_T, u64 n, const Alphabet &al, const u32 *d_fstart, u64 k, SortSpace &sp, const Round0 &r0, u64 h)
{
    u64 *cnt = ctx->d_small + SM_COUNTERS;
    const u64 a = r.a;
    ActiveList &cur = r.cur;
    r.rounds++;
    {
        SpanGuard g(ctx, BWTS_K_KEYBUILD, a, 20 * a);
        const unsigned blocks = (unsigned)((a + 255) / 256);
        keybuild_sparse_kernel<CYCLIC><<<dim3(blocks), dim3(256), 0, ctx->stream>>>(
            cur.idx, cur.head, a, d_T, n, (const u8 *)(ctx->d_small + SM_CODES), al.bits, al.msym, al.pad_add, h, r0.k0v, r.rb, d_fstart, k, r.akeys[0],
            al.varlen ? ctx->d_small + SM_VTAB : nullptr, al.key_bits, r.tpos, r.trank, r.a0, r.dir, r.dlog, r.pdir, r.psh);
        HIPC(hipGetLastError());
    }
    const u64 *AK = r.akeys[0];
    const u32 *AV = cur.idx;
    const bool seg_probe = !r.seg_skip_next;
    r.seg_skip_next = false;
    bool whole = true;
    u64 m_big = 0;
    if (a > 4096 && seg_probe) BWTS_TRY(seg_sort_round(ctx, sp, r.sb, cur.head, r.akeys[0], cur.idx, a, r.rb, r.round_key_bits, &whole, &r.seg_skip_next, &m_big));
    u64 *rr = fwd_report_round(ctx, r.rounds);
    if (rr) {
        rr[FRR_FORM] = FR_FORM_SPARSE; rr[FRR_H] = h; rr[FRR_IN] = a;
        rr[FRR_PROBE] = a <= 4096 ? 0 : seg_probe ? 1 : 2; rr[FRR_MBIG] = m_big; rr[FRR_WHOLE] = whole; rr[FRR_SKIP_NEXT] = r.seg_skip_next;
    }
    if (whole) {
        const SortPlan ap = sort_plan(r.akeys[0], r.akeys[1], cur.idx, r.scratch, sp.tile_hist, sp.scan_temp);
        int r2 = 0;
        BWTS_TRY(radix_sort_pairs(ctx, ap, a, r.round_key_bits, &r2));
        AK = r.akeys[r2];
        AV = r2 ? r.scratch : cur.idx;
    }
    HIPC(hipMemsetAsync(cnt, 0, 4 * sizeof(u64), ctx->stream));
    {
        SpanGuard g(ctx, BWTS_K_RERANK, a, 24 * a);
        const ActiveList &to = r.sets[r.nxt];
        GroupIn in{AK, cur.slot, a, r.rb};
        GroupOut out{cur.slot, AV, a, r.rb, AK, r.tpos, r.trank, r.a0, r0.SA, to.idx, to.slot, to.head, cnt + 0, cnt + 1};
        BWTS_TRY((device_scan<true, u64>(ctx, a, in, out, OpHeadCount(), (u64)0, sp.scan_temp)));
    }
    BWTS_TRY(read_small(ctx, SM_COUNTERS, 4));
    r.a = ctx->h_small[CNT_ACTIVE]; r.splits = ctx->h_small[CNT_SPLITS];
    cur = r.sets[r.nxt]; r.nxt ^= 1;
    if (CYCLIC && r.rounds - 1 < BWTS_MAX_ROUND_STATS) ctx->tm.round_active[r.rounds - 1] = r.a;
    if (rr) { rr[FRR_OUT] = r.a; rr[FRR_SPLITS] = r.splits; }
    return BWTS_OK;
}

template <bool CYCLIC>
static int sparse_rounds(bwts_ctx *ctx, const u8 *d_T, u64 n, const Alphabet &al, const u32 *d_fstart, u64 k, SortSpace &sp,
                         const Round0 &r0, ActiveList *cur_io, u64 *a_io, u32 *rounds_io)
{
    SparseRun r;
    BlockLayout L;
    r.cur = *cur_io; r.a = r.a0 = *a_io; r.rounds = *rounds_io; r.declare(L, r.a0);
    char *base = nullptr;
    BWTS_TRY(aux_reserve(ctx, L.bytes(), &base));
    L.place(base);
    r.rb = CYCLIC ? bitlen_u64(n - 1) : bitlen_u64(n);
    if (2 * r.rb > 64) return BWTS_E_RANGE;
    r.round_key_bits = 2 * r.rb > 1 ? 2 * r.rb : 1;
    BWTS_TRY(sparse_map(ctx, r, n, al, sp, r0.k0v));
    for (u64 h = (u64)al.hstep;; h <<= 1) {
        BWTS_TRY((sparse_round<CYCLIC>(ctx, r, d_T, n, al, d_fstart, k, sp, r0, h)));
        fwd_report_of(ctx)[FR_END] = r.a == 0 ? FR_END_EMPTY : CYCLIC && r.splits == 0 ? FR_END_STABLE : FR_END_NONE;
        if (r.a == 0) break;
        if (CYCLIC && r.splits == 0) break;
        if (!CYCLIC && h >= n) return BWTS_E_INTERNAL;
        if (r.rounds > 80) return BWTS_E_INTERNAL;
    }
    *cur_io = r.cur; *a_io = r.a; *rounds_io = r.rounds;
    return BWTS_OK;
}

template <bool CYCLIC>
static int doubling_sort(bwts_ctx *ctx, const u8 *d_T, u64 n, const Alphabet &al, const u32 *d_fstart, u64 k,
                         SortSpace &sp, bool want_ranks, u32 **sa_out, u32 *rounds_out, u64 *active0_out)
{
    Round0 r0;
    BWTS_TRY((round0_sort<CYCLIC>(ctx, n, al, sp, &r0)));
    u64 a = r0.a;
    u32 *SA = r0.SA;
    *active0_out = a;
    if (CYCLIC) ctx->tm.round_active[0] = a;
    const bool rank_early = a > n / 32 && r0.flags_outside_rank && n >= (1ull << 22);
    u64 *rep = fwd_report_open(ctx);
    rep[FR_CYCLIC] = CYCLIC; rep[FR_N] = n; rep[FR_K] = k; rep[FR_SIGMA] = (u64)al.sigma; rep[FR_BITS] = (u64)al.bits; rep[FR_MSYM] = (u64)al.msym;
    rep[FR_KEY_BITS] = (u64)al.key_bits; rep[FR_VARLEN] = al.varlen; rep[FR_HSTEP] = (u64)al.hstep;
    rep[FR_KEYS] = r0.k0v.wide ? 0 : r0.k0v.hi ? 2 : 1; rep[FR_FLAGS_OUTSIDE_RANK] = r0.flags_outside_rank; rep[FR_TIED0] = a;
    rep[FR_RANK_EARLY] = rank_early; rep[FR_ROUNDS] = 1;
    if (rank_early) BWTS_TRY(early_ranks(ctx, n, sp, r0));
    ActiveList cur, none{nullptr, nullptr, nullptr};
    BWTS_TRY(tied_list(ctx, n, sp, r0, &cur));
    u32 rounds = 1;

    if (a > 0xffffffffull) return BWTS_E_NOMEM;
    if (a > 0 && a <= n / 32) {
        u64 direct = FR_DIRECT_NONE;
        if (CYCLIC && sp.carry_out && !want_ranks && direct_ties_allowed(ctx, n)) BWTS_TRY(direct_ties(ctx, d_T, n, al, d_fstart, k, sp, cur, a, &direct));
        rep[FR_DIRECT] = direct;
        if (direct == FR_DIRECT_SETTLED) {
            rounds++;
            if (u64 *rr = fwd_report_round(ctx, rounds)) { rr[FRR_FORM] = FR_FORM_DIRECT; rr[FRR_H] = (u64)al.hstep; rr[FRR_IN] = a; rr[FRR_OUT] = 0; rr[FRR_SPLITS] = 1; }
            if (rounds - 1 < BWTS_MAX_ROUND_STATS) ctx->tm.round_active[rounds - 1] = 0;
            rep[FR_FORM] = FR_FORM_DIRECT; rep[FR_END] = FR_END_EMPTY;
            sp.ties_emitted = true;
            a = 0;
        } else {
            rep[FR_FORM] = FR_FORM_SPARSE;
            BWTS_TRY((sparse_rounds<CYCLIC>(ctx, d_T, n, al, d_fstart, k, sp, r0, &cur, &a, &rounds)));
        }
        rep[FR_ROUNDS] = rounds; rep[FR_LEFT] = a;
    } else if (a > 0) {
        BWTS_TRY(ensure_rank(ctx, sp, n));
        if (!rank_early) BWTS_TRY(build_ranks(ctx, SA, n, cur, a, sp.rank));
        const bool need_sa = !CYCLIC || !sp.carry_out;
        const bool tiles_only = [ctx] { const char *e = bwts_knob(ctx, "BWTS_DENSE"); return e && !strcmp(e, "tiles"); }();
        bool handled = false;
        rep[FR_NEED_SA] = need_sa;
        if (tiles_only) rep[FR_NO_CHUNKS] = FR_NC_KNOB;
        if (!tiles_only) BWTS_TRY((chunk_rounds<CYCLIC>(ctx, d_T, n, al, d_fstart, k, sp, cur, a, SA, need_sa, &rounds, &handled)));
        rep[FR_FORM] = handled ? FR_FORM_CHUNKS : FR_FORM_TILES;
        if (!handled) BWTS_TRY((dense_rounds<CYCLIC>(ctx, d_T, n, al, d_fstart, k, sp, cur, a, SA, need_sa, &rounds)));
        rep[FR_ROUNDS] = rounds;
        sp.ties_emitted = CYCLIC && sp.carry_out;
        *sa_out = SA;
        *rounds_out = rounds;
        return BWTS_OK;
    }
    if (want_ranks && !rank_early) { BWTS_TRY(ensure_rank(ctx, sp, n)); BWTS_TRY(build_ranks(ctx, SA, n, a ? cur : none, a, sp.rank)); }
    *sa_out = SA;
    *rounds_out = rounds;
    return BWTS_OK;
}

static_assert(KB_TILE == SCAN_TILE, "keybuild0's tile minima feed the scan's final sweep");

static int launch_keybuild0_seg(bwts_ctx *ctx, const u8 *d_T, u64 n, const Alphabet &al, u64 *keys0, u64 *tile_min, bool split, u64 pos0, u64 count,
                                u8 *wprev = nullptr , u32 *hist0 = nullptr)
{
    if (hist0 && (pos0 != 0 || !split)) return BWTS_E_INTERNAL;
    SpanGuard g(ctx, BWTS_K_KEYBUILD, count, count + (split ? 5 : 8) * count);
    const u64 blocks = (count + KB_RX_TILE - 1) / KB_RX_TILE;
    KeyStore ks = key_store_of(keys0, count, split, al.key_bits);
    ks.wprev = split ? nullptr : wprev;
    if (al.varlen) {
        keybuild0v_kernel<<<dim3((unsigned)blocks), dim3(KB_THREADS), 0, ctx->stream>>>(d_T, n, ctx->d_small + SM_VTAB, al.key_bits,
                                                                                        ks, tile_min, pos0, pos0 + count, hist0);
        HIPC(hipGetLastError());
        return BWTS_OK;
    }
    keybuild0_kernel<<<dim3((unsigned)blocks), dim3(KB_THREADS), 0, ctx->stream>>>(
        d_T, n, (const u8 *)(ctx->d_small + SM_CODES), al.bits, al.msym, al.pad_add, ks, tile_min, pos0, pos0 + count, hist0);
    HIPC(hipGetLastError());
    return BWTS_OK;
}

struct RankIn { const u32 *r; __device__ __forceinline__ u32 operator()(u64 i) const { return r[i]; } };
struct MinFlagOut {
    const u32 *r; u8 *flag;
    __device__ __forceinline__ void operator()(u64 i, u32 min_before) const { flag[i] = (i == 0 || r[i] < min_before) ? 1 : 0; }
};
struct FlagIn { const u8 *flag; __device__ __forceinline__ u32 operator()(u64 i) const { return flag[i]; } };
struct StartOut {
    const u8 *flag; u32 *starts; u64 n; u64 *total;
    __device__ __forceinline__ void operator()(u64 i, u32 dst) const
    {
        if (flag[i]) starts[dst] = (u32)i;
        if (i + 1 == n) *total = (u64)dst + flag[i];
    }
};

static int suffix_sort_in(bwts_ctx *ctx, const u8 *d_T, u64 n, SortSpace &sp, bool want_ranks, u32 **d_sa, u32 *rounds)
{
    if (n > 0xffffffffull) return BWTS_E_RANGE;
    Alphabet al;
    BWTS_TRY(set_alphabet(ctx, true, n, &al));
    BWTS_TRY(launch_keybuild0_seg(ctx, d_T, n, al, sp.keys[0], nullptr, false, 0, n));
    u64 active0 = 0;
    return doubling_sort<false>(ctx, d_T, n, al, nullptr, 0, sp, want_ranks, d_sa, rounds, &active0);
}

static int take_factor_list(bwts_ctx *ctx, u64 n, u64 k_min, SortSpace &sp, u32 **d_fstart, u64 *k_out)
{
    BWTS_TRY(read_small(ctx, CNT_TOTAL, 1));
    const u64 k = ctx->h_small[CNT_TOTAL];
    if (k < k_min || k > n) return BWTS_E_INTERNAL;
    char *fl = nullptr;
    BWTS_TRY(aux_reserve_slot(ctx, 2, (size_t)k * 4, &fl));
    HIPC(hipMemcpyAsync(fl, sp.keys[1], k * sizeof(u32), hipMemcpyDeviceToDevice, ctx->stream));
    *d_fstart = (u32 *)fl; *k_out = k;
    return BWTS_OK;
}

static int lyndon_general(bwts_ctx *ctx, const u8 *d_T, u64 n, SortSpace &sp, u32 **d_fstart, u64 *k_out, u32 *rounds)
{
    u32 *sa = nullptr;
    BWTS_TRY(suffix_sort_in(ctx, d_T, n, sp, true, &sa, rounds));
    u8 *flag = (u8 *)sp.keys[0];
    {
        SpanGuard g(ctx, BWTS_K_LYNDON, n, 8 * n);
        RankIn in{sp.rank};
        MinFlagOut out{sp.rank, flag};
        BWTS_TRY((device_scan<false, u32>(ctx, n, in, out, OpMin(), 0xffffffffu, sp.scan_temp)));
        FlagIn fin{flag};
        StartOut sout{flag, (u32 *)sp.keys[1], n, ctx->d_small + CNT_TOTAL};
        BWTS_TRY((device_scan<false, u32>(ctx, n, fin, sout, OpAdd(), 0u, sp.scan_temp)));
    }
    return take_factor_list(ctx, n, 1, sp, d_fstart, k_out);
}

#define LYN_CAND_CAP   65536ull
#define LYN_WORK_CAP   (64ull << 20)

struct KeyIn { KeyStore K; __device__ __forceinline__ u64 operator()(u64 i) const { return ks_load(K, i); } };
struct CandOut {
    KeyStore K; u64 n; int msym; u64 *cand; u64 cap; u64 *counter;
    u64 pos0 = 0;
    __device__ __forceinline__ void operator()(u64 j, u64 min_before) const
    {
        const u64 ki = ks_load(K, j);
        const u64 i = pos0 + j;
        const bool c = i == 0 || ki <= min_before;
        const u64 m = __ballot(c);
        if (m == 0) return;
        const int leader = __ffsll((unsigned long long)m) - 1;
        unsigned long long base = 0;
        if (lane_id() == leader) base = atomicAdd((unsigned long long *)counter, (unsigned long long)__popcll(m));
        base = shfl_t((u64)base, leader);
        if (c) {
            const u64 at = base + (u64)__popcll(m & lanemask_lt());
            const bool definite = i == 0 || (ki < min_before && i + (u64)msym <= n);
            if (at < cap) cand[at] = (i << 1) | (definite ? 1ull : 0ull);
        }
    }
};

struct TileMayHoldCandidate {
    const u64 *tile_min;
    __device__ __forceinline__ bool operator()(u64 t, u64 min_before) const { return tile_min[t] <= min_before; }
};

#define LYN_LOCAL_LCE  (64u << 10)
struct LynState {
    u64 next;
    u64 cur;
    u64 k;
    u64 status;
    u64 forced;
    u64 forced_less;
    u64 work;
};

template <typename POS>
__global__ __launch_bounds__(256) void lyndon_resolve_kernel(const u8 *__restrict__ T, u64 n, const u64 *__restrict__ cand, u64 cnt,
                                                             POS *__restrict__ fstart, LynState *__restrict__ st, u64 work_cap)
{
    __shared__ int s_mis[4];
    __shared__ int s_less[4];
    const int tid = threadIdx.x, w = tid >> 6, lane = tid & 63;
    u64 cur = st->cur, k = st->k, work = st->work;
    const u64 first = st->next;
    const bool forced = st->forced != 0, forced_less = st->forced_less != 0;
    __syncthreads();
    for (u64 c = first; c < cnt; c++) {
        const u64 e = cand[c];
        const u64 p = e >> 1;
        bool is_start;
        if (p == 0 || (e & 1)) {
            is_start = true;
        } else if (forced && c == first) {
            is_start = forced_less;
        } else {
            is_start = false;
            for (u64 off = 0;; off += 256) {
                const u64 i = off + tid;
                const int a = p + i < n ? (int)T[p + i] : -1;
                const int b = cur + i < n ? (int)T[cur + i] : -1;
                const u64 mm = __ballot(a != b);
                if (lane == 0) s_mis[w] = mm ? __ffsll((unsigned long long)mm) - 1 : -1;
                if (mm && lane == __ffsll((unsigned long long)mm) - 1) s_less[w] = a < b;
                __syncthreads();
                int found = -1;
#pragma unroll
                for (int ww = 3; ww >= 0; ww--) if (s_mis[ww] >= 0) found = ww;
                const int less = found >= 0 ? s_less[found] : 0;
                __syncthreads();
                work += 256;
                if (found >= 0) { is_start = less != 0; break; }
                if (off + 256 >= LYN_LOCAL_LCE || work > work_cap) {
                    if (tid == 0) { st->next = c; st->cur = cur; st->k = k; st->work = work; st->forced = 0; st->status = work > work_cap ? 2 : 1; }
                    return;
                }
            }
        }
        if (is_start) {
            if (tid == 0) fstart[k] = (POS)p;
            k++;
            cur = p;
        }
    }
    if (tid == 0) { st->next = cnt; st->cur = cur; st->k = k; st->work = work; st->forced = 0; st->status = 0; }
}

__global__ __launch_bounds__(256) void suffix_mismatch_grid_kernel(const u8 *__restrict__ T, u64 n, u64 p, u64 q,
                                                                   unsigned long long *__restrict__ result)
{
    const u64 len = n - p;
    for (u64 i = (u64)blockIdx.x * 256 + threadIdx.x; i < len; i += (u64)gridDim.x * 256) {
        if (i >= __hip_atomic_load(result, __ATOMIC_RELAXED, __HIP_MEMORY_SCOPE_AGENT)) break;
        if (T[p + i] != T[q + i]) { atomicMin(result, (unsigned long long)i); break; }
    }
}

template <typename IDX>
static int lyndon_resolve_candidates(bwts_ctx *ctx, const u8 *d_T, u64 n, u64 *const cand[2], u32 *const cvals[2], u32 *tile_hist, void *scan_temp, u64 cnt_c,
                                     IDX *fstart, u64 *k, bool *settled)
{
    *settled = false;
    SortPlan cp = sort_plan(cand[0], cand[1], cvals[0], cvals[1], tile_hist, scan_temp);
    int res = 0;
    BWTS_TRY(radix_sort_pairs(ctx, cp, cnt_c, bitlen_u64(n) + 1, &res));
    LynState *d_st = (LynState *)(ctx->d_small + CNT_LYN_K);
    LynState *h_st = (LynState *)(ctx->h_small + CNT_LYN_K);
    unsigned long long *d_mis = (unsigned long long *)(ctx->d_small + CNT_LYN_K + 8);
    HIPC(hipMemsetAsync(d_st, 0, sizeof(LynState), ctx->stream));
    for (int iter = 0;; iter++) {
        {
            SpanGuard g(ctx, BWTS_K_LYNDON, cnt_c, 0);
            lyndon_resolve_kernel<IDX><<<dim3(1), dim3(256), 0, ctx->stream>>>(d_T, n, cand[res], cnt_c, fstart, d_st, LYN_WORK_CAP);
            HIPC(hipGetLastError());
        }
        BWTS_TRY(read_small(ctx, CNT_LYN_K, 8));
        if (h_st->status == 0) break;
        if (h_st->status == 2 || iter > 4096) return BWTS_OK;
        u64 e = 0;
        HIPC(hipMemcpyAsync(&e, cand[res] + h_st->next, sizeof(u64), hipMemcpyDeviceToHost, ctx->stream));
        HIPC(hipStreamSynchronize(ctx->stream));
        const u64 pp = e >> 1, qq = h_st->cur;
        const u64 len = n - pp;
        HIPC(hipMemcpyAsync(d_mis, &len, sizeof(u64), hipMemcpyHostToDevice, ctx->stream));
        {
            SpanGuard g(ctx, BWTS_K_LYNDON, len, 2 * len);
            u64 blocks = (len + 255) / 256; if (blocks > 4096) blocks = 4096;
            suffix_mismatch_grid_kernel<<<dim3((unsigned)blocks), dim3(256), 0, ctx->stream>>>(d_T, n, pp, qq, d_mis);
            HIPC(hipGetLastError());
        }
        BWTS_TRY(read_small(ctx, CNT_LYN_K + 8, 1));
        const u64 at = ctx->h_small[CNT_LYN_K + 8];
        bool less;
        if (at >= len) less = true;
        else {
            u8 ab[2];
            HIPC(hipMemcpyAsync(&ab[0], d_T + pp + at, 1, hipMemcpyDeviceToHost, ctx->stream));
            HIPC(hipMemcpyAsync(&ab[1], d_T + qq + at, 1, hipMemcpyDeviceToHost, ctx->stream));
            HIPC(hipStreamSynchronize(ctx->stream));
            less = ab[0] < ab[1];
        }
        h_st->forced = 1; h_st->forced_less = less ? 1 : 0; h_st->status = 0;
        HIPC(hipMemcpyAsync(d_st, h_st, sizeof(LynState), hipMemcpyHostToDevice, ctx->stream));
        HIPC(hipStreamSynchronize(ctx->stream));
    }
    *k = h_st->k;
    if (*k == 0) return BWTS_E_INTERNAL;
    *settled = true;
    return BWTS_OK;
}

static int lyndon_fast(bwts_ctx *ctx, const u8 *d_T, u64 n, const Alphabet &al, SortSpace &sp, const u64 *tile_min, u64 *cand[2],
                       u32 *cvals[2], u32 *fstart, u64 *k_out, bool *done)
{
    *done = false;
    u64 *cnt = ctx->d_small + SM_COUNTERS;
    HIPC(hipMemsetAsync(cnt + 4, 0, 4 * sizeof(u64), ctx->stream));
    {
        SpanGuard g(ctx, BWTS_K_LYNDON, n, 0);
        const u64 tiles = scan_tiles(n);
        HIPC(hipMemcpyAsync(sp.scan_temp, tile_min, tiles * sizeof(u64), hipMemcpyDeviceToDevice, ctx->stream));
        BWTS_TRY((device_scan_partials<u64, OpMin>(ctx, tiles, OpMin(), ~0ull, sp.scan_temp)));
        const KeyStore ks = key_store_of(sp.keys[0], n, sp.split_keys, al.key_bits);
        KeyIn in{ks};
        CandOut out{ks, n, al.varlen ? 64 : al.msym, cand[0], LYN_CAND_CAP, ctx->d_small + CNT_CAND};
        TileMayHoldCandidate filter{tile_min};
        BWTS_TRY((device_scan_final<false, u64>(ctx, n, in, out, OpMin(), ~0ull, sp.scan_temp, filter)));
    }
    BWTS_TRY(read_small(ctx, CNT_CAND, 1));
    const u64 cnt_c = ctx->h_small[CNT_CAND];
    if (cnt_c == 0) return BWTS_E_INTERNAL;
    if (cnt_c > LYN_CAND_CAP) return BWTS_OK;
    return lyndon_resolve_candidates<u32>(ctx, d_T, n, cand, cvals, sp.tile_hist, sp.scan_temp, cnt_c, fstart, k_out, done);
}

__global__ __launch_bounds__(256) void seg_duval_kernel(const u8 *__restrict__ T, const u64 *__restrict__ seg_off, u64 count, u8 *__restrict__ flag)
{
    const u64 s = (u64)blockIdx.x * 4 + (threadIdx.x >> 6);
    if (s >= count) return;
    const int lane = lane_id();
    const u64 base = seg_off[s], L = seg_off[s + 1] - base;
    const u8 *S = T + base;
    u64 i = 0;
    while (i < L) {
        u64 j = i + 1, k = i;
// ... 428 lines not shown
```

### bijective-bwt_amd/csrc/internal.h

```cpp
#pragma once

#include <hip/hip_runtime.h>
#include <stdint.h>
#include <stddef.h>
#include <assert.h>
#include <string>
#include <vector>
#include <functional>

#include "../../include/bwts.h"
#include "seg_layout.h"
#include "stage_cut.h"

typedef uint64_t u64;
typedef uint32_t u32;
typedef uint16_t u16;
typedef uint8_t  u8;

struct TimedSpan {
    int cls;
    hipEvent_t a, b;
};

struct CopyPool;

#define INV_REPORT_MAX 8
#define INV_REPORT_WORDS 16
#define SEG_REPORT_WORDS 8
enum SegReportWord { SR_PLAN, SR_BIG, SR_RUNS, SR_OWN_SEGS, SR_OWN_BYTES, SR_SINGLE_SEGS, SR_SINGLE_BYTES, SR_ATTEMPTS };
#define FWD_REPORT_SORTS 2
#define FWD_HEADER_WORDS 48
#define FWD_ROUND_WORDS 12
#define FWD_SORT_WORDS (FWD_HEADER_WORDS + BWTS_MAX_ROUND_STATS * FWD_ROUND_WORDS)
#define STAGE_SLOTS 4
#define BWTS_AUX_SLOTS 5

struct KeptBlock { char *p; size_t cap; const char *name; };
enum { KB_ARENA, KB_AUX, KB_IO = KB_AUX + BWTS_AUX_SLOTS, KB_SEG_TABLE = KB_IO + 4, KB_SEG_SCRATCH, KB_PACK, KB_COUNT = KB_PACK + 2 };

#define SM_RX_SYNC 4090
#define SM_EC_TOTAL 4020
#define SM_EC_FLAG  4021
#define SM_EC_HEAD  4022
#define SM_CRC_OUT  4024
#define SM_PACK_HEAD 4026
#define SM_ZRL_TOTAL 4034
#define SM_ZRL_FLAG  4035

struct Stager {
    hipStream_t stream;
    bool own_stream;
    char *pinned[STAGE_SLOTS];
    hipEvent_t slot_ev[STAGE_SLOTS], slot_ev2[STAGE_SLOTS];
    hipStream_t copy_stream;
    CopyPool *pool;
};

struct bwts_ctx {
    int device;
    hipStream_t stream;
    size_t call_block_bytes = 0;
    int last_hip;

    KeptBlock kept[KB_COUNT] = {{nullptr, 0, "arena"},
                                {nullptr, 0, "side block 0"}, {nullptr, 0, "side block 1"}, {nullptr, 0, "side block 2"},
                                {nullptr, 0, "side block 3"}, {nullptr, 0, "side block 4"},
                                {nullptr, 0, "device input 0"}, {nullptr, 0, "device input 1"},
                                {nullptr, 0, "device output 0"}, {nullptr, 0, "device output 1"},
                                {nullptr, 0, "segment table"}, {nullptr, 0, "segment scratch"},
                                {nullptr, 0, "pack stage 0"}, {nullptr, 0, "pack stage 1"}};
    size_t arena_off;
    size_t unv_hint;
    u64 inv_report[INV_REPORT_MAX][INV_REPORT_WORDS];
    u32 inv_attempts_made = 0;
    u64 fwd_report[FWD_REPORT_SORTS][FWD_SORT_WORDS];
    u32 fwd_sorts_made = 0;
    std::vector<char *> tied_blk;
    int tied_blk_lg = 0;
    size_t guard = 0;
    struct GuardBlock { char *user; size_t bytes; const char *name; };
    std::vector<GuardBlock> guard_blocks;
    std::vector<GuardBlock> guard_freed;

    u64 *h_small;
    u64 *d_small;

    Stager stg[3];
    std::vector<std::pair<char *, size_t>> host_blocks;

    std::vector<hipEvent_t> ev_pool;
    size_t ev_used;
    std::vector<TimedSpan> spans;
    hipEvent_t ev_begin, ev_end;
    int timing;

    std::vector<const void *> lds_granted;

    std::vector<std::pair<std::string, std::string>> knobs;
    int fused_scan_cap;

    std::vector<u64> seg_off;
    u64 *h_seg_off = nullptr;
    size_t h_seg_cap = 0;
    u64 seg_report[SEG_REPORT_WORDS] = {0};
    bool crc_tables = false;

    bwts_timings tm;
    double host_ms[BWTS_H_COUNT];
    bool launched;
};

void bwts_stage_mark(bwts_ctx *ctx, const char *name);
#define STAGE(name) bwts_stage_mark(ctx, name)

#define HIPC(call)                                                        \
    do {                                                                  \
        hipError_t e__ = (call);                                          \
        if (e__ != hipSuccess) { ctx->last_hip = (int)e__; return BWTS_E_HIP; } \
    } while (0)

void bwts_trace_error(const char *file, int line, int rc);
#define BWTS_TRY(call)                   \
    do {                                 \
        int rc__ = (call);               \
        if (rc__ != BWTS_OK) { bwts_trace_error(__FILE__, __LINE__, rc__); return rc__; } \
    } while (0)

const char *bwts_knob(const bwts_ctx *ctx, const char *name);

static inline size_t align_up(size_t x, size_t a) { return (x + a - 1) / a * a; }
double wall_ms(void);
#define NARROW_N 0x100000000ull
static inline bool ranges_overlap(const void *a, u64 na, const void *b, u64 nb)
{
    const uintptr_t x = (uintptr_t)a, y = (uintptr_t)b;
    return x <= y ? y - x < na : x - y < nb;
}

struct Transform {
    int (*fn)(bwts_ctx *, const u8 *, u64, u8 *);
    const char *name, *in_label;
    size_t (*arena_hint)(const bwts_ctx *ctx, u64 n);
};
int run_device(bwts_ctx *ctx, const Transform &t, const void *d_in, u64 n, void *d_out);
__global__ void pcie_copy_kernel(uint4 *__restrict__ dst, const uint4 *__restrict__ src, u64 vecs, u8 *__restrict__ dst_tail, const u8 *__restrict__ src_tail, u32 tail);

struct HostTrip {
    const u8 *in; u64 in_bytes;
    u64 io_bytes;
    u8 *out; u64 *out_bytes;
    bwts_sink_fn sink = nullptr; void *user = nullptr;
    const Transform *ahead = nullptr;
};
int host_round_trip(bwts_ctx *ctx, const HostTrip &trip, const std::function<int(const u8 *, u8 *, u64 *)> &device_form);
int run_batch(bwts_ctx *ctx, const Transform &t, int count, const uint8_t *const *ins, const uint64_t *ns, uint8_t *const *outs);
void staging_destroy(bwts_ctx *ctx);

hipError_t ctx_malloc(bwts_ctx *ctx, void **out, size_t bytes, const char *name);
hipError_t ctx_free(bwts_ctx *ctx, void *user);
int  guard_check(bwts_ctx *ctx, const char *what);
void trace_alloc(const bwts_ctx *ctx, const char *what, const char *name, const void *p, size_t bytes);
bool poison_on(const bwts_ctx *ctx);
int  kept_grow(bwts_ctx *ctx, KeptBlock &b, size_t bytes, size_t round, int host_cost);
int  kept_give_up(bwts_ctx *ctx, KeptBlock &b);
size_t ctx_device_bytes(const bwts_ctx *ctx);
int  tied_release(bwts_ctx *ctx);
static inline u8 *d_io(const bwts_ctx *ctx, int i) { return (u8 *)ctx->kept[KB_IO + i].p; }
static inline u64 *d_seg_off(const bwts_ctx *ctx) { return (u64 *)ctx->kept[KB_SEG_TABLE].p; }
int  seg_table_set(bwts_ctx *ctx, const uint64_t *lengths, uint64_t count, u64 *total);
int  seg_upload_extra(bwts_ctx *ctx, const u64 *words, u64 count, u64 **d_words);
int  seg_pinned_region(bwts_ctx *ctx, u64 at, u64 words, void **p);
void seg_pinned_free(bwts_ctx *ctx);
int  seg_scratch_reserve(bwts_ctx *ctx, size_t bytes, u8 **p);

int  arena_reserve(bwts_ctx *ctx, size_t bytes);
int  arena_release(bwts_ctx *ctx);
void arena_install(bwts_ctx *ctx, void *block, size_t bytes, double alloc_ms);
void arena_reset(bwts_ctx *ctx);
void *arena_alloc(bwts_ctx *ctx, size_t bytes);
struct BlockLayout;
int  arena_take(bwts_ctx *ctx, const BlockLayout &L);
template <typename T> static inline T *arena_array(bwts_ctx *ctx, u64 count)
{
    return (T *)arena_alloc(ctx, (size_t)count * sizeof(T));
}

int ensure_dyn_lds(bwts_ctx *ctx, const void *kernel, size_t bytes);

int  span_begin(bwts_ctx *ctx, int cls, u64 elems, u64 alg_bytes);
void span_end(bwts_ctx *ctx, int span);
void spans_reset(bwts_ctx *ctx);
int  spans_resolve(bwts_ctx *ctx);

struct SpanGuard {
    bwts_ctx *c;
    int h;
    SpanGuard(bwts_ctx *ctx, int cls, u64 elems, u64 alg_bytes) : c(ctx), h(span_begin(ctx, cls, elems, alg_bytes)) {}
    ~SpanGuard() { span_end(c, h); }
};

int read_small(bwts_ctx *ctx, int first, int count);

size_t scan_temp_bytes(u64 n);
int exclusive_sum_u32(bwts_ctx *ctx, u32 *data, u64 n, void *temp);

struct SortPlan {
    u64  *keys[2];
    u32  *vals[2];
    u32  *tile_hist;
    void *scan_temp;
    const u8 *sym_src = nullptr;
    u8 *sym_buf[2] = {nullptr, nullptr};
    u8 *sym_final = nullptr;
    bool vals_identity = false;
    bool keys_split = false;
    u32 *first_hist = nullptr;
};
static inline SortPlan sort_plan(u64 *k0, u64 *k1, u32 *v0, u32 *v1, u32 *tile_hist, void *scan_temp)
{
    SortPlan p;
    p.keys[0] = k0; p.keys[1] = k1; p.vals[0] = v0; p.vals[1] = v1; p.tile_hist = tile_hist; p.scan_temp = scan_temp;
    return p;
}
bool radix_packed_applicable(const bwts_ctx *ctx, u64 m, int key_bits);
size_t radix_tile_hist_bytes(u64 m);
int radix_sort_pairs(bwts_ctx *ctx, const SortPlan &plan, u64 m, int key_bits, int *result_buf);
int radix_column_scan(bwts_ctx *ctx, u32 *tile_hist, u64 tiles, void *scan_temp);
int radix_sort_keys(bwts_ctx *ctx, u64 *keys[2], u32 *tile_hist, void *scan_temp, u64 m, int lo_bit, int bits, int *result_buf);

int forward_device_impl(bwts_ctx *ctx, const u8 *d_in, u64 n, u8 *d_out);
struct SegTable { const u64 *d_off; u64 count; u8 *flag; };
#define SEG_FWD_BIG (1ull << 21)
int forward_segments_impl(bwts_ctx *ctx, const u8 *d_in, u64 n, u8 *d_out);
int inverse_segments_impl(bwts_ctx *ctx, const u8 *d_in, u64 n, u8 *d_out);
size_t inverse_segments_arena_bytes(const bwts_ctx *ctx, u64 n);
int inverse_segments_plan_words(const u64 *lengths, u64 count, u64 out[8]);
int inverse_device_impl(bwts_ctx *ctx, const u8 *d_in, u64 n, u8 *d_out);
size_t forward_arena_bytes(u64 n);
int forward_wide_arena_probe(u64 n, int mode, int seg_log2, u64 bucket_cap, u64 *bytes);
int    inverse_splitter_log2(u64 n);
size_t inverse_attempt_bytes(u64 n, int g, int mark);
size_t inverse_arena_bytes(u64 n);

static inline SegMode seg_mode(const bwts_ctx *ctx) { return SegMode{ctx->seg_off.empty() ? 0 : (u64)ctx->seg_off.size() - 1}; }
static inline StageCut stage_cut_call(const bwts_ctx *ctx, SegMode segs, u64 n, u64 unit_a, u64 unit_b = 0)
{
    return stage_cut_call(ctx->seg_off, segs, n, unit_a, unit_b);
}

int mtf_impl(bwts_ctx *ctx, const u8 *d_in, u64 n, u8 *d_out, bool inverse, SegMode segs);
size_t mtf_arena_bytes(const bwts_ctx *ctx, u64 n, SegMode segs);
void bwts_mtf_plan(u64 n, u64 out[4]);

int ec_encode_impl(bwts_ctx *ctx, const u8 *d_in, u64 n, u8 *d_out, u64 out_cap, SegMode segs, u64 *sizes);
int ec_decode_impl(bwts_ctx *ctx, const u8 *d_in, u64 in_bytes, u8 *d_out, u64 out_cap, u64 *n_out, SegMode segs, const u64 *stream_bytes);
void bwts_ec_plan(u64 n, u64 out[5]);

int zrl_encode_impl(bwts_ctx *ctx, const u8 *d_in, u64 n, u8 *d_out, u64 out_cap, SegMode segs, u64 *sizes);
int zrl_decode_impl(bwts_ctx *ctx, const u8 *d_in, u64 in_bytes, u8 *d_out, u64 n, SegMode segs, const u64 *in_lengths);
void bwts_zrl_plan(u64 n, u64 out[2]);

int crc_impl(bwts_ctx *ctx, const u8 *d_in, u64 n, SegMode segs, u32 *crcs);
void bwts_crc_plan(u64 n, u64 out[4]);
int pack_device_impl(bwts_ctx *ctx, u32 version, const u8 *d_in, u64 n, u64 B, u8 *d_out, u64 out_cap, u64 *out_bytes);
int unpack_device_impl(bwts_ctx *ctx, const u8 *d_in, u64 in_bytes, u8 *d_out, u64 out_cap, u64 *n_out);

struct ChunkRecut { u32 S; u64 nc; bool allowed; };
u32 chunk_nominal_size(u64 a);
u64 chunk_table_capacity(u64 a0);
ChunkRecut chunk_recut_plan(u64 a0, u64 a_chunks);

int suffix_sort_device(bwts_ctx *ctx, const u8 *d_T, u64 n, u32 **d_sa, u32 **d_rank, u32 *rounds);
int lyndon_factors_device(bwts_ctx *ctx, const u8 *d_T, u64 n, u32 **d_fstart, u64 *k, u32 *rounds);
int byte_histogram_device(bwts_ctx *ctx, const u8 *d_T, u64 n, u64 *d_hist256);
int constant_input_probe(bwts_ctx *ctx, const u8 *d_in, u64 n, bool *constant);
int aux_reserve_slot(bwts_ctx *ctx, int slot, size_t bytes, char **base);
static inline int aux_reserve(bwts_ctx *ctx, size_t bytes, char **base) { return aux_reserve_slot(ctx, 0, bytes, base); }
int aux_release(bwts_ctx *ctx);

struct BlockLayout {
    struct Field { void *var; size_t off; void (*set)(void *var, char *p); };
    Field f[32];
    int count = 0;
    size_t total = 0;
    template <typename T> static size_t padded(u64 n) { return align_up((size_t)n * sizeof(T), 256); }
    template <typename T> void array(T **var, u64 n) { raw(var, padded<T>(n)); }
    template <typename... T> void arrays(u64 n, T **...vars) { (array(vars, n), ...); }
    template <typename T> void raw(T **var, size_t bytes)
    {
        assert(count < (int)(sizeof f / sizeof f[0]));
        f[count++] = Field{var, total, [](void *v, char *p) { *(T **)v = (T *)p; }};
        total += bytes;
    }
    void pad(size_t bytes) { total += bytes; }
    size_t bytes() const { return total; }
    void place(char *base) const { for (int i = 0; i < count; i++) f[i].set(f[i].var, base + f[i].off); }
    bool place_within(char *base, size_t cap) const { if (bytes() > cap) return false; place(base); return true; }
};

struct SortBufs {
    u64  *keys[2];
    u32  *vals[2], *tile_hist;
    void *scan_temp;
    void declare(BlockLayout &L, u64 m)
    {
        L.arrays(m, &keys[0], &keys[1]); L.arrays(m, &vals[0], &vals[1]);
        L.raw(&tile_hist, radix_tile_hist_bytes(m)); L.raw(&scan_temp, scan_temp_bytes(m));
    }
    SortPlan plan() const { return sort_plan(keys[0], keys[1], vals[0], vals[1], tile_hist, scan_temp); }
};

int generate_device_impl(bwts_ctx *ctx, int kind, u64 seed, u64 n, u8 *d_out);
int device_equal_impl(bwts_ctx *ctx, const u8 *a, const u8 *b, u64 bytes, int *equal);
```

### bijective-bwt_amd/csrc/radix.hip

```cpp
#include "internal.h"
#include "device_utils.h"
#include "scan_templ.h"

#include <stdlib.h>

#define RX_CHUNK   128
#define RX_XCDS    8
constexpr int RX_THREADS = 512, RX_ITEMS = 16, RX_MINW = 4, RX_WAVES = RX_THREADS / 64, RX_TILE = RX_THREADS * RX_ITEMS;
constexpr u64 RX_HIST_TILE = 3072;

__device__ __forceinline__ u64 rx_tile_of_block(u64 tiles)
{
    const u64 per = (tiles + RX_XCDS - 1) / RX_XCDS;
    return (u64)(blockIdx.x % RX_XCDS) * per + (u64)(blockIdx.x / RX_XCDS);
}
static inline u64 rx_grid(u64 tiles) { return (tiles + RX_XCDS - 1) / RX_XCDS * RX_XCDS; }

static inline u64 rx_tiles(u64 m) { return (m + RX_TILE - 1) / RX_TILE; }
static inline u64 radix_chunks(u64 tiles) { return (tiles + RX_CHUNK - 1) / RX_CHUNK; }

size_t radix_tile_hist_bytes(u64 m)
{
    const u64 tiles = (m + RX_HIST_TILE - 1) / RX_HIST_TILE + 1;
    return align_up((size_t)tiles * 256 * sizeof(u32), 256) +
// ... 106 lines not shown
    u32 *dbase = L::dbase(rx_smem), *gbase = L::gbase(rx_smem), *scan_sm = L::scan_sm(rx_smem);
    u16 (*whist)[256] = L::whist(rx_smem);
    u8 *sdig = L::sdig(rx_smem);
    const int tid = threadIdx.x, lane = tid & 63, w = tid >> 6;
    const u64 tile = rx_tile_of_block((m + TILE - 1) / TILE);
    const u64 tile_base = tile * TILE;
    if (tile_base >= m) return;
    const u64 wave_base = tile_base + (u64)w * (64 * IT);
    const u64 remain = m - tile_base;
    const u32 tile_count = remain < TILE ? (u32)remain : (u32)TILE;

    for (int i = tid; i < WAVES * 128; i += TH) ((u32 *)whist)[i] = 0;

    u64 key[IT];
    Pos16<IT> pos;
#pragma unroll
    for (int j = 0; j < IT; j++) {
        const u64 i = wave_base + (u64)j * 64 + lane;
        key[j] = i < m ? kin[i] : ~0ull;
    }
    __syncthreads();

#pragma unroll
    for (int j = 0; j < IT; j++) {
        const bool valid = wave_base + (u64)j * 64 + lane < m;
        const u32 d = (u32)(key[j] >> shift) & 255u;
        wave_rank_step(whist[w], d, valid, [&](u32 r) { pos.init(j, r); });
    }
    __syncthreads();
    {
        const u32 exc = digit_bases<WAVES>(whist, scan_sm);
        if (tid < 256) {
            dbase[tid] = exc;
            gbase[tid] = tile_off[tile * 256 + tid] - exc;
        }
    }
    __syncthreads();

    constexpr int HB = IT % 8 == 0 ? 8 : 4;
#pragma unroll
    for (int j0 = 0; j0 < IT; j0 += HB) {
        u32 add[HB];
#pragma unroll
        for (int jj = 0; jj < HB; jj++) {
            const u32 d = (u32)(key[j0 + jj] >> shift) & 255u;
            add[jj] = dbase[d] + whist[w][d];
        }
#pragma unroll
        for (int jj = 0; jj < HB; jj++) {
            const int j = j0 + jj;
            const bool valid = wave_base + (u64)j * 64 + lane < m;
            const u32 p = pos.get(j) + add[jj];
            pos.set(j, p);
            if (valid) stage[p] = key[j];
        }
    }
    u32 val[KEYS_ONLY ? 1 : IT];
    u32 sym[HAS_SYM ? IT : 1];
    if (!KEYS_ONLY) {
#pragma unroll
        for (int j = 0; j < IT; j++) {
            const u64 i = wave_base + (u64)j * 64 + lane;
            val[KEYS_ONLY ? 0 : j] = IDENT ? (u32)i : (i < m ? vin[i] : 0u);
        }
    }
    if (HAS_SYM) {
#pragma unroll
        for (int j = 0; j < IT; j++) {
            const u64 i = wave_base + (u64)j * 64 + lane;
            sym[j] = i < m ? (u32)sin[i] : 0u;
        }
    }
    __syncthreads();
#pragma unroll
    for (int j0 = 0; j0 < IT; j0 += HB) {
        u64 k[HB];
        u32 g[HB];
#pragma unroll
        for (int jj = 0; jj < HB; jj++) {
            const u32 s = (u32)(j0 + jj) * TH + tid;
            k[jj] = s < tile_count ? stage[s] : 0ull;
        }
#pragma unroll
        for (int jj = 0; jj < HB; jj++) g[jj] = gbase[(u32)(k[jj] >> shift) & 255u];
#pragma unroll
        for (int jj = 0; jj < HB; jj++) {
            const u32 s = (u32)(j0 + jj) * TH + tid;
            if (s < tile_count) {
                sdig[s] = (u8)((u32)(k[jj] >> shift) & 255u);
                kout[g[jj] + s] = k[jj];
            }
        }
    }
    if (KEYS_ONLY) return;
    __syncthreads();
#pragma unroll
    for (int j = 0; j < IT; j++) {
        const bool valid = wave_base + (u64)j * 64 + lane < m;
        const u32 p = pos.get(j);
        if (valid) {
            if (HAS_SYM) stage[p] = (u64)val[KEYS_ONLY ? 0 : j] | ((u64)sym[j] << 32);
            else ((u32 *)stage)[p] = val[KEYS_ONLY ? 0 : j];
        }
    }
    __syncthreads();
#pragma unroll
    for (int j0 = 0; j0 < IT; j0 += HB) {
        u64 e[HAS_SYM ? HB : 1];
        u32 v32[HAS_SYM ? 1 : HB];
        u32 g[HB];
#pragma unroll
        for (int jj = 0; jj < HB; jj++) {
            const u32 s = (u32)(j0 + jj) * TH + tid;
            const u32 sc = s < tile_count ? s : 0u;
            if (HAS_SYM) e[jj] = stage[sc]; else v32[jj] = ((u32 *)stage)[sc];
            g[jj] = sdig[sc];
        }
#pragma unroll
        for (int jj = 0; jj < HB; jj++) g[jj] = gbase[g[jj]];
#pragma unroll
        for (int jj = 0; jj < HB; jj++) {
            const u32 s = (u32)(j0 + jj) * TH + tid;
            if (s < tile_count) {
                const u32 dst = g[jj] + s;
                if (HAS_SYM) { vout[dst] = (u32)e[jj]; sout[dst] = (u8)(e[jj] >> 32); }
                else vout[dst] = v32[jj];
            }
        }
    }
}

struct PackedIO {
    const u32 *lo_in; const void *c_in;
    const u32 *val_in;
    u32 *lo_out;
    void *c_out;
    u8 *hi_out, *sym_out;
    u32 *val_out;
};

template <bool FIRST, bool LAST, bool HI16>
__global__ __launch_bounds__(RX_THREADS, RX_MINW) void radix_scatter_packed_kernel(PackedIO io, const u32 *__restrict__ tile_off, u64 m, int shift)
{
    extern __shared__ __attribute__((aligned(16))) char rx_smem[];
    using L = RxTile<RX_THREADS, RX_ITEMS>;
    u64 *stage = L::stage(rx_smem);
    u32 *dbase = L::dbase(rx_smem), *gbase = L::gbase(rx_smem), *scan_sm = L::scan_sm(rx_smem);
    u16 (*whist)[256] = L::whist(rx_smem);
    u8 *sdig = L::sdig(rx_smem);
    const int tid = threadIdx.x, lane = tid & 63, w = tid >> 6;
    const u64 tile = rx_tile_of_block((m + RX_TILE - 1) / RX_TILE);
    const u64 tile_base = tile * RX_TILE;
    if (tile_base >= m) return;
    const u64 wave_base = tile_base + (u64)w * (64 * RX_ITEMS);
    const u64 remain = m - tile_base;
    const u32 tile_count = remain < RX_TILE ? (u32)remain : (u32)RX_TILE;

    for (int i = tid; i < RX_WAVES * 128; i += RX_THREADS) ((u32 *)whist)[i] = 0;

    const u64 i0 = wave_base + (u64)lane;
    u32 vmask = 0;
#pragma unroll
    for (int j = 0; j < RX_ITEMS; j++) vmask |= (i0 + (u64)j * 64 < m ? 1u : 0u) << j;
#define PK_VALID(j) ((vmask >> (j)) & 1u)

    constexpr bool DIG_C = HI16 && LAST;
    u32 dsrc[RX_ITEMS];
    Pos16<RX_ITEMS> pos;
    {
        const u16 *c16 = (const u16 *)io.c_in + i0;
        const u32 *lop = io.lo_in + i0;
#pragma unroll
        for (int j = 0; j < RX_ITEMS; j++) {
            if (DIG_C) dsrc[j] = PK_VALID(j) ? (u32)c16[j * 64] : 0xffffu;
            else dsrc[j] = PK_VALID(j) ? lop[j * 64] : ~0u;
        }
    }
#define PK_DIGIT(j) (DIG_C ? (dsrc[j] & 255u) : ((dsrc[j] >> shift) & 255u))
    __syncthreads();

#pragma unroll
    for (int j = 0; j < RX_ITEMS; j++) {
        const bool valid = PK_VALID(j);
        const u32 d = PK_DIGIT(j);
        wave_rank_step(whist[w], d, valid, [&](u32 r) { pos.init(j, r); });
    }
    __syncthreads();
    {
        const u32 exc = digit_bases<RX_WAVES>(whist, scan_sm);
        if (tid < 256) {
            dbase[tid] = exc;
            gbase[tid] = tile_off[tile * 256 + tid] - exc;
        }
    }
    __syncthreads();

    constexpr int HB = 8;
    u32 *stage32 = (u32 *)stage;
#pragma unroll
    for (int j0 = 0; j0 < RX_ITEMS; j0 += HB) {
        u32 add[HB];
#pragma unroll
        for (int jj = 0; jj < HB; jj++) {
            const u32 d = PK_DIGIT(j0 + jj);
            add[jj] = dbase[d] + whist[w][d];
        }
#pragma unroll
        for (int jj = 0; jj < HB; jj++) {
            const int j = j0 + jj;
            const bool valid = PK_VALID(j);
            const u32 p = pos.get(j) + add[jj];
            pos.set(j, p);
            if (valid) { stage32[p] = dsrc[j]; sdig[p] = (u8)PK_DIGIT(j); }
        }
    }
    u32 sa[RX_ITEMS], sb[RX_ITEMS];
    {
        const u32 *lop = io.lo_in + i0, *valp = io.val_in + i0;
        const u8 *c8 = (const u8 *)io.c_in + i0;
        const u16 *c16 = (const u16 *)io.c_in + i0;
#pragma unroll
        for (int j = 0; j < RX_ITEMS; j++) {
            if (FIRST) sa[j] = 0u;
            else if (DIG_C) sa[j] = PK_VALID(j) ? lop[j * 64] : 0u;
            else sa[j] = PK_VALID(j) ? valp[j * 64] : 0u;
        }
#pragma unroll
        for (int j = 0; j < RX_ITEMS; j++) {
            if (DIG_C) sb[j] = PK_VALID(j) ? valp[j * 64] : 0u;
            else sb[j] = PK_VALID(j) ? (HI16 ? (u32)c16[j * 64] : (u32)c8[j * 64]) : 0u;
        }
    }
    __syncthreads();
    u32 hi_s[DIG_C ? RX_ITEMS : 1];
#pragma unroll
    for (int j0 = 0; j0 < RX_ITEMS; j0 += HB) {
        u32 x[HB], g[HB];
#pragma unroll
        for (int jj = 0; jj < HB; jj++) {
            const u32 s = (u32)(j0 + jj) * RX_THREADS + tid;
            const u32 sc = s < tile_count ? s : 0u;
            x[jj] = stage32[sc];
            g[jj] = sdig[sc];
        }
#pragma unroll
        for (int jj = 0; jj < HB; jj++) g[jj] = gbase[g[jj]];
#pragma unroll
        for (int jj = 0; jj < HB; jj++) {
            const u32 s = (u32)(j0 + jj) * RX_THREADS + tid;
            if (DIG_C) hi_s[j0 + jj] = x[jj] & 255u;
            if (s < tile_count) {
                const u32 dst = g[jj] + s;
                if (DIG_C) io.sym_out[dst] = (u8)(x[jj] >> 8);
                else io.lo_out[dst] = x[jj];
            }
        }
    }
    __syncthreads();
    u32 idx_base = (u32)wave_base + (u32)lane;
    asm volatile("" : "+v"(idx_base));
#pragma unroll
    for (int j = 0; j < RX_ITEMS; j++) {
        const bool valid = PK_VALID(j);
        const u32 second = sb[j];
        const u32 firstw = FIRST ? idx_base + (u32)j * 64u : sa[j];
        if (valid) ((uint2 *)stage)[pos.get(j)] = make_uint2(firstw, second);
    }
    __syncthreads();
#pragma unroll
    for (int j0 = 0; j0 < RX_ITEMS; j0 += HB) {
        uint2 e[HB];
        u32 g[HB];
#pragma unroll
        for (int jj = 0; jj < HB; jj++) {
            const u32 s = (u32)(j0 + jj) * RX_THREADS + tid;
            const u32 sc = s < tile_count ? s : 0u;
            e[jj] = ((const uint2 *)stage)[sc];
            g[jj] = sdig[sc];
        }
#pragma unroll
        for (int jj = 0; jj < HB; jj++) g[jj] = gbase[g[jj]];
#pragma unroll
        for (int jj = 0; jj < HB; jj++) {
            const u32 s = (u32)(j0 + jj) * RX_THREADS + tid;
            if (s < tile_count) {
                const u32 dst = g[jj] + s;
                if (DIG_C) {
                    io.lo_out[dst] = e[jj].x;
                    io.hi_out[dst] = (u8)hi_s[j0 + jj];
                    io.val_out[dst] = e[jj].y;
                } else {
                    io.val_out[dst] = e[jj].x;
                    if (LAST) io.sym_out[dst] = (u8)e[jj].y;
                    else if (HI16) ((u16 *)io.c_out)[dst] = (u16)e[jj].y;
                    else ((u8 *)io.c_out)[dst] = (u8)e[jj].y;
                }
            }
        }
    }
#undef PK_DIGIT
#undef PK_VALID
}

static bool knob_off(const bwts_ctx *ctx, const char *name) { const char *e = bwts_knob(ctx, name); return e && atoi(e) == 0; }

template <typename T>
static int radix_pass_offsets(bwts_ctx *ctx, const T *src, u64 m, int shift, u32 *tile_hist, bool counted, void *scan_temp)
{
    const u64 tiles = rx_tiles(m);
    if (!counted) {
        SpanGuard g(ctx, BWTS_K_RADIX_HIST, m, sizeof(T) * m);
        radix_hist_kernel<T><<<dim3((unsigned)tiles), dim3(RX_THREADS), 0, ctx->stream>>>(src, m, shift, tile_hist);
    }
    SpanGuard g(ctx, BWTS_K_RADIX_SCAN, tiles * 256, tiles * 256 * 12);
    STAGE("radix pass: histogram");
    BWTS_TRY(radix_column_scan(ctx, tile_hist, tiles, scan_temp));
    STAGE("radix pass: column scan");
    return BWTS_OK;
}

template <typename... P, typename... A>
static int launch_scatter(bwts_ctx *ctx, void (*kernel)(P...), u64 m, u64 alg_bytes, bool roofline, A... args)
{
    constexpr size_t lds = RxTile<RX_THREADS, RX_ITEMS>::bytes;
    {
        SpanGuard g(ctx, BWTS_K_RADIX_SCATTER, m, alg_bytes);
        const int gm = roofline ? span_begin(ctx, BWTS_K_RADIX_SCATTER_MAIN, m, alg_bytes) : -1;
        const int rc = ensure_dyn_lds(ctx, (const void *)kernel, lds);
        if (rc == BWTS_OK) kernel<<<dim3((unsigned)rx_grid(rx_tiles(m))), dim3(RX_THREADS), lds, ctx->stream>>>(args...);
        span_end(ctx, gm);
        BWTS_TRY(rc);
    }
    HIPC(hipGetLastError());
    STAGE("radix pass: scatter");
    return BWTS_OK;
}

template <bool HI16>
static int radix_sort_packed(bwts_ctx *ctx, const SortPlan &plan, u64 m, int passes, int *result_buf)
{
    const size_t lo_bytes = align_up((size_t)m * 4, 256);
    const u64 pass_bytes = HI16 ? 20 : 18;
    int cur = 0;
    for (int p = 0; p < passes; p++) {
        const int shift = 8 * p;
        const bool first = p == 0, last = p == passes - 1;
        char *src = (char *)plan.keys[cur], *dst = (char *)plan.keys[cur ^ 1];
        PackedIO io{};
        io.lo_in = (const u32 *)src; io.c_in = src + lo_bytes; io.val_in = plan.vals[cur];
        io.lo_out = (u32 *)dst; io.c_out = dst + lo_bytes; io.val_out = plan.vals[cur ^ 1];
        io.hi_out = (u8 *)dst + lo_bytes; io.sym_out = plan.sym_final;
        u32 *tile_hist = first && plan.first_hist ? plan.first_hist : plan.tile_hist;
        const bool counted = tile_hist != plan.tile_hist;
        if (HI16 && shift >= 32) BWTS_TRY(radix_pass_offsets(ctx, (const u16 *)io.c_in, m, 0, tile_hist, counted, plan.scan_temp));
        else BWTS_TRY(radix_pass_offsets(ctx, io.lo_in, m, shift, tile_hist, counted, plan.scan_temp));
        const u64 bytes = first ? pass_bytes - 4 : last ? pass_bytes / 2 + (HI16 ? 10 : 9) : pass_bytes;
        const auto kernel = first ? radix_scatter_packed_kernel<true, false, HI16>
                          : last  ? radix_scatter_packed_kernel<false, true, HI16> : radix_scatter_packed_kernel<false, false, HI16>;
        BWTS_TRY(launch_scatter(ctx, kernel, m, bytes * m, !first && !last, io, tile_hist, m, shift));
        cur ^= 1;
    }
    *result_buf = cur;
    return BWTS_OK;
}

#define RS_THREADS 1024
#define RS_WAVES   (RS_THREADS / 64)
#define RS_ITEMS   4
#define RS_MAX     (RS_THREADS * RS_ITEMS)
__global__ __launch_bounds__(RS_THREADS) void radix_sort_small_kernel(const u64 *__restrict__ kin, const u32 *__restrict__ vin,
                                                                      u64 *__restrict__ kout, u32 *__restrict__ vout, u32 m, int passes)
{
    __shared__ u64 sk[2][RS_MAX];
    __shared__ u32 sv[2][RS_MAX];
    __shared__ u16 whist[RS_WAVES][256];
    __shared__ u32 dbase[256];
    __shared__ u32 scan_sm[RS_WAVES];
    const int tid = threadIdx.x, lane = tid & 63, w = tid >> 6;
    for (u32 i = tid; i < m; i += RS_THREADS) { sk[0][i] = kin[i]; sv[0][i] = vin[i]; }
    int cur = 0;
    for (int p = 0; p < passes; p++) {
        const int shift = 8 * p;
        for (int i = tid; i < RS_WAVES * 128; i += RS_THREADS) ((u32 *)whist)[i] = 0;
        __syncthreads();
        const u32 wbase = (u32)w * (64 * RS_ITEMS);
        u64 key[RS_ITEMS];
        u32 val[RS_ITEMS], pos[RS_ITEMS];
#pragma unroll
        for (int j = 0; j < RS_ITEMS; j++) {
            const u32 i = wbase + (u32)j * 64 + lane;
            key[j] = i < m ? sk[cur][i] : ~0ull;
            val[j] = i < m ? sv[cur][i] : 0u;
        }
#pragma unroll
        for (int j = 0; j < RS_ITEMS; j++) {
            const bool valid = wbase + (u32)j * 64 + lane < m;
            const u32 d = (u32)(key[j] >> shift) & 255u;
            wave_rank_step(whist[w], d, valid, [&](u32 r) { pos[j] = r; });
        }
        __syncthreads();
        {
            const u32 exc = digit_bases<RS_WAVES>(whist, scan_sm);
            if (tid < 256) dbase[tid] = exc;
        }
        __syncthreads();
#pragma unroll
        for (int j = 0; j < RS_ITEMS; j++) {
            const bool valid = wbase + (u32)j * 64 + lane < m;
            const u32 d = (u32)(key[j] >> shift) & 255u;
            if (valid) {
                const u32 dst = dbase[d] + whist[w][d] + pos[j];
                sk[cur ^ 1][dst] = key[j];
                sv[cur ^ 1][dst] = val[j];
            }
        }
        __syncthreads();
        cur ^= 1;
    }
    for (u32 i = tid; i < m; i += RS_THREADS) { kout[i] = sk[cur][i]; vout[i] = sv[cur][i]; }
}

#define RX_FUSED_CHUNKS 256
__global__ __launch_bounds__(256) void radix_column_scan_fused_kernel(u32 *__restrict__ tile_hist, u64 tiles, u32 chunks, u32 *__restrict__ chunk_sum,
                                                                      unsigned int *__restrict__ sync)
{
    __shared__ u32 scan_sm[4];
    const u32 c = blockIdx.x, d = threadIdx.x;
    const u64 t0 = (u64)c * RX_CHUNK;
    const u64 t1 = t0 + RX_CHUNK < tiles ? t0 + RX_CHUNK : tiles;
    u32 s = 0;
    {
        u64 t = t0;
        for (; t + 8 <= t1; t += 8) {
            u32 v[8];
#pragma unroll
            for (int j = 0; j < 8; j++) v[j] = tile_hist[(t + j) * 256 + d];
#pragma unroll
            for (int j = 0; j < 8; j++) s += v[j];
        }
        for (; t < t1; t++) s += tile_hist[t * 256 + d];
    }
    u32 before = 0, total = s;
    if (chunks > 1) {
        chunk_sum[(u64)c * 256 + d] = s;
        __threadfence();
        __syncthreads();
        if (d == 0) {
            __hip_atomic_fetch_add(&sync[0], 1u, __ATOMIC_RELEASE, __HIP_MEMORY_SCOPE_AGENT);
            while (__hip_atomic_load(&sync[0], __ATOMIC_ACQUIRE, __HIP_MEMORY_SCOPE_AGENT) < chunks) __builtin_amdgcn_s_sleep(1);
        }
        __syncthreads();
        __threadfence();
        total = 0;
        u32 cc = 0;
        for (; cc + 4 <= chunks; cc += 4) {
            const u32 v0 = chunk_sum[(u64)cc * 256 + d], v1 = chunk_sum[(u64)(cc + 1) * 256 + d];
            const u32 v2 = chunk_sum[(u64)(cc + 2) * 256 + d], v3 = chunk_sum[(u64)(cc + 3) * 256 + d];
            total += v0 + v1 + v2 + v3;
            before += (cc < c ? v0 : 0u) + (cc + 1 < c ? v1 : 0u) + (cc + 2 < c ? v2 : 0u) + (cc + 3 < c ? v3 : 0u);
        }
        for (; cc < chunks; cc++) { const u32 v = chunk_sum[(u64)cc * 256 + d]; total += v; before += cc < c ? v : 0u; }
    }
    u32 all;
    const u32 base = block_scan_exclusive<u32, OpAdd, 4>(total, OpAdd(), 0u, scan_sm, &all);
    u32 run = base + before;
    {
        u64 t = t0;
        for (; t + 8 <= t1; t += 8) {
            u32 v[8];
#pragma unroll
            for (int j = 0; j < 8; j++) v[j] = tile_hist[(t + j) * 256 + d];
#pragma unroll
            for (int j = 0; j < 8; j++) { tile_hist[(t + j) * 256 + d] = run; run += v[j]; }
        }
        for (; t < t1; t++) { const u32 v = tile_hist[t * 256 + d]; tile_hist[t * 256 + d] = run; run += v; }
    }
    if (chunks > 1) {
        __syncthreads();
        if (d == 0) {
            const u32 left = __hip_atomic_fetch_add(&sync[1], 1u, __ATOMIC_ACQ_REL, __HIP_MEMORY_SCOPE_AGENT);
            if (left + 1 == chunks) {
                __hip_atomic_store(&sync[0], 0u, __ATOMIC_RELAXED, __HIP_MEMORY_SCOPE_AGENT);
                __hip_atomic_store(&sync[1], 0u, __ATOMIC_RELEASE, __HIP_MEMORY_SCOPE_AGENT);
            }
        }
    }
}

int radix_column_scan(bwts_ctx *ctx, u32 *tile_hist, u64 tiles, void *scan_temp)
{
    const u64 chunks = radix_chunks(tiles);
    u32 *chunk_sum = (u32 *)((char *)tile_hist + align_up((size_t)tiles * 256 * sizeof(u32), 256));
    const bool fused_ok = !knob_off(ctx, "BWTS_RX_FUSED_SCAN");
    if (ctx->fused_scan_cap == 0) {
        int per_cu = 0, cus = 0;
        if (hipOccupancyMaxActiveBlocksPerMultiprocessor(&per_cu, radix_column_scan_fused_kernel, 256, 0) != hipSuccess ||
            hipDeviceGetAttribute(&cus, hipDeviceAttributeMultiprocessorCount, ctx->device) != hipSuccess) { (void)hipGetLastError(); per_cu = 0; }
        ctx->fused_scan_cap = per_cu > 0 && cus > 0 ? per_cu * cus : -1;
    }
    if (fused_ok && chunks <= RX_FUSED_CHUNKS && (long long)chunks <= (long long)ctx->fused_scan_cap) {
        radix_column_scan_fused_kernel<<<dim3((unsigned)chunks), dim3(256), 0, ctx->stream>>>(tile_hist, tiles, (u32)chunks, chunk_sum,
                                                                                             (unsigned int *)(ctx->d_small + SM_RX_SYNC));
        HIPC(hipGetLastError());
        return BWTS_OK;
    }
    radix_chunk_sum_kernel<<<dim3((unsigned)chunks), dim3(256), 0, ctx->stream>>>(tile_hist, tiles, chunks, chunk_sum);
    BWTS_TRY(exclusive_sum_u32(ctx, chunk_sum, chunks * 256, scan_temp));
    radix_chunk_apply_kernel<<<dim3((unsigned)chunks), dim3(256), 0, ctx->stream>>>(tile_hist, tiles, chunks, chunk_sum);
    HIPC(hipGetLastError());
    return BWTS_OK;
}

int radix_sort_keys(bwts_ctx *ctx, u64 *keys[2], u32 *tile_hist, void *scan_temp, u64 m, int lo_bit, int bits, int *result_buf)
{
    int cur = 0;
    for (int shift = lo_bit; shift < lo_bit + bits; shift += 8) {
        BWTS_TRY(radix_pass_offsets(ctx, keys[cur], m, shift, tile_hist, false, scan_temp));
        BWTS_TRY(launch_scatter(ctx, radix_scatter2_kernel<RX_THREADS, RX_ITEMS, RX_MINW, false, false, true>, m, 16 * m, false,
                                keys[cur], nullptr, keys[cur ^ 1], nullptr, tile_hist, m, shift,
                                nullptr, nullptr));
        cur ^= 1;
    }
    *result_buf = cur;
    return BWTS_OK;
}

bool radix_packed_applicable(const bwts_ctx *ctx, u64 m, int key_bits)
{
    const int passes = ((key_bits < 1 ? 1 : key_bits) + 7) / 8;
    return !knob_off(ctx, "BWTS_RX_PACK") && passes >= 3 && passes <= 5 && m >= 65536;
}

int radix_sort_pairs(bwts_ctx *ctx, const SortPlan &plan, u64 m, int key_bits, int *result_buf)
{
    int cur = 0;
    if (m == 0) { *result_buf = 0; return BWTS_OK; }
    if (key_bits < 1) key_bits = 1;
    if (key_bits > 64) key_bits = 64;
    const int passes = (key_bits + 7) / 8;

    if (!knob_off(ctx, "BWTS_RX_SMALL") && m <= RS_MAX && !plan.sym_src && !plan.vals_identity && !plan.keys_split) {
        SpanGuard g(ctx, BWTS_K_RADIX_SCATTER, m, 24 * m);
        radix_sort_small_kernel<<<dim3(1), dim3(RS_THREADS), 0, ctx->stream>>>(plan.keys[0], plan.vals[0], plan.keys[1], plan.vals[1], (u32)m, passes);
        HIPC(hipGetLastError());
        *result_buf = 1;
        return BWTS_OK;
    }
    if (plan.keys_split) {
        if (!plan.sym_final || !plan.vals_identity || !radix_packed_applicable(ctx, m, key_bits)) return BWTS_E_INTERNAL;
        if (passes == 5) return radix_sort_packed<true>(ctx, plan, m, passes, result_buf);
        return radix_sort_packed<false>(ctx, plan, m, passes, result_buf);
    }

    for (int p = 0; p < passes; p++) {
        const int shift = 8 * p;
        BWTS_TRY(radix_pass_offsets(ctx, plan.keys[cur], m, shift, plan.tile_hist, false, plan.scan_temp));
        const bool ident = plan.vals_identity && p == 0, has_sym = plan.sym_src != nullptr;
        const u8 *sin = !has_sym ? nullptr : p == 0 ? plan.sym_src : plan.sym_buf[(p - 1) & 1];
        u8 *sout = !has_sym ? nullptr : p == passes - 1 ? plan.sym_final : plan.sym_buf[p & 1];
        const auto kernel = has_sym ? (ident ? radix_scatter2_kernel<RX_THREADS, RX_ITEMS, RX_MINW, true, true>
                                             : radix_scatter2_kernel<RX_THREADS, RX_ITEMS, RX_MINW, true, false>)
                                    : (ident ? radix_scatter2_kernel<RX_THREADS, RX_ITEMS, RX_MINW, false, true>
                                             : radix_scatter2_kernel<RX_THREADS, RX_ITEMS, RX_MINW, false, false>);
        BWTS_TRY(launch_scatter(ctx, kernel, m, ((has_sym ? 26 : 24) - (ident ? 4 : 0)) * m, has_sym && !ident,
                                plan.keys[cur], plan.vals[cur], plan.keys[cur ^ 1], plan.vals[cur ^ 1],
                                plan.tile_hist, m, shift, sin, sout));
        cur ^= 1;
    }
    *result_buf = cur;
    return BWTS_OK;
}
```

Measured before the change: 33340.

## Fuse tie-group flagging into a lean final radix pass for round-0 sort

Adds a 'lean' final scatter pass for the 5-pass split-key round-0 sort. It writes only the output symbols, plus values and head/keep flag bits for tied positions, instead of full keys, and it checks tile seams for ties that span tiles. This is meant to skip writing full sorted keys and the separate group-flags kernel when the alphabet statistics predict few ties. If a seam is undecided, the tie count is too high, or the direct tie resolution fails, it falls back to redoing the classic last pass, which adds extra work in that case.

```diff
diff --git a/bijective-bwt_amd/__init__.py b/bijective-bwt_amd/__init__.py
--- a/bijective-bwt_amd/__init__.py
+++ b/bijective-bwt_amd/__init__.py
@@ -63,6 +63,8 @@
                      "order_sort", "left"]
 FWD_DIRECT_WORD = 36
 FWD_DIRECT = {0: "not_tried", 1: "settled", 2: "fallback_group", 3: "fallback_depth"}
+FWD_LEAN_WORD = 37
+FWD_LEAN = {0: "not_tried", 1: "held", 2: "gave_up_seam", 3: "gave_up_count", 4: "gave_up_direct"}
 FWD_CHUNK_FIELDS = ["S", "maxchunks", "a_small", "big0", "m_exit", "m_stay", "groups", "wide_possible", "fsl", "compactions",
                     "compactions_skipped", "enqueued_behind_last"]
 FWD_ROUND_FIELDS = {"sparse": ["form", "h", "in", "out", "splits", "probe", "m_big", "whole", "skip_next"],
@@ -588,6 +590,7 @@
             d = {f: w[i] for i, f in enumerate(FWD_HEADER_FIELDS)}
             d["form"], d["keys"], d["no_chunks"], d["end"] = FWD_FORMS[d["form"]], FWD_KEYS[d["keys"]], FWD_NO_CHUNKS[d["no_chunks"]], FWD_ENDS[d["end"]]
             d["direct"], d["direct_word"] = FWD_DIRECT[w[FWD_DIRECT_WORD]], w[FWD_DIRECT_WORD]
+            d["lean"], d["lean_word"] = FWD_LEAN[w[FWD_LEAN_WORD]], w[FWD_LEAN_WORD]
             for f in ("cyclic", "varlen", "flags_outside_rank", "rank_early", "need_sa", "order_sort"):
                 d[f] = bool(d[f])
             if d["form"] == "chunks":
diff --git a/bijective-bwt_amd/csrc/forward.hip b/bijective-bwt_amd/csrc/forward.hip
--- a/bijective-bwt_amd/csrc/forward.hip
+++ b/bijective-bwt_amd/csrc/forward.hip
@@ -1,6 +1,7 @@
 #include "internal.h"
 #include "device_utils.h"
 #include "scan_templ.h"
+#include "../../include/bwts_test.h"
 
 #include <math.h>
 #include <stdio.h>
@@ -27,6 +28,7 @@
     bool varlen;
     int hstep;
     int patch_span;
+    bool few_ties;
 };
 #define SM_DGCNT  2816
 #define SM_SEGCNT 2560
@@ -198,7 +200,8 @@
     return 64;
 }
 
-static int sampled_key_bits(bwts_ctx *ctx, const u8 *d_T, u64 n, const SortBufs &scratch, const u64 *vtab, const double share[65], int *kb_emp)
+static int sampled_key_bits(bwts_ctx *ctx, const u8 *d_T, u64 n, const SortBufs &scratch, const u64 *vtab, const double share[65], int *kb_emp,
+                            double partners_of[65])
 {
     HIPC(hipMemcpyAsync(ctx->d_small + SM_VTAB, vtab, 256 * sizeof(u64), hipMemcpyHostToDevice, ctx->stream));
     HIPC(hipMemsetAsync(ctx->d_small + CNT_SAMPLE, 0, 8 * sizeof(u64), ctx->stream));
@@ -215,7 +218,8 @@
     for (int b = 32, w = 1; b <= 56; b += 8, w++) {
         const double m = (double)ctx->h_small[CNT_SAMPLE + w];
         const double partners = m >= 8.0 ? (double)n * m / pairs : (double)n * share[b];
-        if (1.0 - exp(-partners) <= 1.0 / 64.0) { *kb_emp = b; break; }
+        partners_of[b] = partners;
+        if (*kb_emp == 64 && 1.0 - exp(-partners) <= 1.0 / 64.0) *kb_emp = b;
     }
     return BWTS_OK;
 }
@@ -230,6 +234,13 @@
     const char *env = bwts_knob(ctx, "BWTS_KEY_SYMBOLS");
     if (env) { int v = atoi(env); if (v >= 1 && v <= 64 / bits) msym = v; else if (v == 0) msym = 64 / bits; }
     al->msym = al->hstep = msym; al->key_bits = bits * msym; al->varlen = false; al->patch_span = msym - 1;
+    const auto few = [](double partners) { return 1.0 - exp(-partners) <= 1.0 / 64.0; };
+    const auto fixed_partners = [&](int m) {
+        double sum2 = 0.0;
+        for (int c = 0; c < 256; c++) { const double p = (double)hist[c] / (double)n; sum2 += p * p; }
+        return (double)n * pow(sum2, (double)m);
+    };
+    al->few_ties = few(fixed_partners(msym));
     const char *vl = bwts_knob(ctx, "BWTS_VARLEN");
     u32 vcode[256]; u8 vlen[256];
     double avg = 0, ent = 0;
@@ -238,15 +249,17 @@
     if (try_vl && lmax <= VL_MAXLEN) {
         u64 *vtab = ctx->h_small + SM_VTAB;
         for (int c = 0; c < 256; c++) vtab[c] = ((u64)vlen[c] << 32) | vcode[c];
-        double share[65];
+        double share[65], partners_of[65];
+        for (int b = 0; b <= 64; b++) partners_of[b] = -1.0;
         int kb = iid_key_bits(hist, vlen, vcode, n, share), kb_emp = 0;
-        if (d_T && scratch && n >= (1ull << 22)) BWTS_TRY(sampled_key_bits(ctx, d_T, n, *scratch, vtab, share, &kb_emp));
+        if (d_T && scratch && n >= (1ull << 22)) BWTS_TRY(sampled_key_bits(ctx, d_T, n, *scratch, vtab, share, &kb_emp, partners_of));
         if (kb_emp > kb) {
             const int keep = 40;
             if (keep / lmax >= 4) kb = keep;
             else {
                 kb = kb_emp;
                 al->msym = al->hstep = 64 / bits; al->key_bits = bits * al->msym; al->patch_span = al->msym - 1;
+                al->few_ties = few(fixed_partners(al->msym));
             }
         }
         const char *kbe = bwts_knob(ctx, "BWTS_KEY_BITS");
@@ -254,6 +267,7 @@
         const int passes_fixed = (al->key_bits + 7) / 8, passes_var = (kb + 7) / 8;
         if ((vl && vl[0] == '1') || passes_var < passes_fixed || (passes_var == passes_fixed && avg < (double)bits - 0.25)) {
             al->varlen = true; al->key_bits = kb; al->patch_span = 64;
+            al->few_ties = few(partners_of[kb] >= 0.0 ? partners_of[kb] : (double)n * share[kb]);
             al->msym = al->hstep = kb / lmax < 1 ? 1 : kb / lmax;
             HIPC(hipMemcpyAsync(ctx->d_small + SM_VTAB, vtab, 256 * sizeof(u64), hipMemcpyHostToDevice, ctx->stream));
         }
@@ -1143,13 +1157,16 @@
                      FR_ROUNDS, FR_DIRECTORY, FR_ORDER_SORT, FR_LEFT,
                      FC_S = 24, FC_MAXCHUNKS, FC_A_SMALL, FC_BIG0, FC_M_EXIT, FC_M_STAY, FC_GROUPS, FC_WIDE_POSSIBLE, FC_FSL, FC_COMPACTIONS,
                      FC_COMPACTIONS_SKIPPED, FC_ENQUEUED_BEHIND_LAST,
-                     FR_DIRECT = 36  };
+                     FR_DIRECT = 36 ,
+                     FR_LEAN = 37  };
 enum FwdRoundWord { FRR_FORM, FRR_H, FRR_IN, FRR_OUT, FRR_SPLITS, FRR_PROBE = 5, FRR_MBIG, FRR_WHOLE, FRR_SKIP_NEXT,
                     FRR_CHUNKS_IN = 5, FRR_CHUNKS_OUT, FRR_BIG_IN, FRR_BIG_STAYS, FRR_BIG_LEAVES, FRR_NCHUNKS, FRR_TILE_MBIG = 5 };
 enum FwdForm { FR_FORM_NONE, FR_FORM_SPARSE, FR_FORM_CHUNKS, FR_FORM_TILES, FR_FORM_DIRECT };
 enum FwdNoChunks { FR_NC_NA, FR_NC_SHORT, FR_NC_KNOB, FR_NC_STORE, FR_NC_ORDER, FR_NC_BIGLIST };
 enum FwdEnd { FR_END_NONE, FR_END_EMPTY, FR_END_STABLE };
-static_assert(FC_ENQUEUED_BEHIND_LAST < FR_DIRECT && FR_DIRECT < FWD_HEADER_WORDS && FRR_NCHUNKS < FWD_ROUND_WORDS && FR_LEFT < FC_S, "the forward report's layout");
+enum FwdLean { FR_LEAN_NONE, FR_LEAN_HELD, FR_LEAN_SEAM, FR_LEAN_COUNT, FR_LEAN_DIRECT };
+static_assert(FR_LEAN == BWTS_FWD_LEAN_WORD, "include/bwts_test.h names the word");
+static_assert(FC_ENQUEUED_BEHIND_LAST < FR_DIRECT && FR_LEAN < FWD_HEADER_WORDS && FRR_NCHUNKS < FWD_ROUND_WORDS && FR_LEFT < FC_S, "the forward report's layout");
 static u64 *fwd_report_open(bwts_ctx *ctx)
 {
     u64 *w = ctx->fwd_report[ctx->fwd_sorts_made < FWD_REPORT_SORTS ? ctx->fwd_sorts_made : FWD_REPORT_SORTS - 1];
@@ -1173,53 +1190,101 @@
     u64 *headw, *keepw, *pre;
     bool flags_outside_rank;
     u64 a;
+    bool lean, seam;
 };
-
-template <bool CYCLIC>
-static int round0_sort(bwts_ctx *ctx, u64 n, const Alphabet &al, SortSpace &sp, Round0 *r0)
+#define CNT_SEAM (SM_COUNTERS + 3)
+__global__ void flag_tail_kernel(u64 *headw, u64 n)
+{
+    if (threadIdx.x == 0 && blockIdx.x == 0 && (n & 63)) headw[n >> 6] = (1ull << (n & 63)) - 1ull;
+}
+
+static int round0_flag_words(bwts_ctx *ctx, u64 n, SortSpace &sp, Round0 *r0)
+{
+    const u64 words = (n + 63) / 64;
+    r0->flags_outside_rank = sp.carry_buf[0] && sp.carry_buf[1] && n >= 4096;
+    if (r0->flags_outside_rank) {
+        r0->headw = (u64 *)sp.carry_buf[0]; r0->keepw = r0->headw + words; r0->pre = (u64 *)sp.carry_buf[1];
+    } else {
+        BWTS_TRY(ensure_rank(ctx, sp, n));
+        r0->headw = (u64 *)sp.rank; r0->keepw = r0->headw + words; r0->pre = r0->keepw + words;
+    }
+    return BWTS_OK;
+}
+
+static int round0_flags(bwts_ctx *ctx, u64 n, SortSpace &sp, Round0 *r0)
 {
     u64 *cnt = ctx->d_small + SM_COUNTERS;
+    const u64 words = (n + 63) / 64;
+    const K0Keys &k0v = r0->k0v;
+    u64 *K0 = sp.keys[r0->res];
+    {
+        SpanGuard g(ctx, BWTS_K_RERANK, n, r0->lean ? 16 * words : (k0v.wide ? 8 : k0v.hi ? 5 : 4) * n);
+        if (!r0->lean) {
+            u64 waves = (words + GF_WORDS - 1) / GF_WORDS;
+            unsigned blocks = (unsigned)((waves + 3) / 4 < 16384 ? (waves + 3) / 4 : 16384);
+            if (k0v.wide) group_flags_kernel<GfWide><<<dim3(blocks), dim3(256), 0, ctx->stream>>>(GfWide{K0, ~0ull}, n, r0->headw, r0->keepw);
+            else if (k0v.hi) group_flags_kernel<GfSplit<true>><<<dim3(blocks), dim3(256), 0, ctx->stream>>>(GfSplit<true>{k0v.lo, k0v.hi}, n, r0->headw, r0->keepw);
+            else group_flags_kernel<GfSplit<false>><<<dim3(blocks), dim3(256), 0, ctx->stream>>>(GfSplit<false>{k0v.lo, nullptr}, n, r0->headw, r0->keepw);
+        }
+        WordIn in{r0->headw, r0->keepw};
+        ScanStoreArr<u64> out{r0->pre};
+        BWTS_TRY((device_scan<false, u64>(ctx, words, in, out, OpHeadCount(), (u64)0, sp.scan_temp)));
+        count_tied_kernel<<<dim3(1), dim3(64), 0, ctx->stream>>>(r0->keepw, r0->pre, words, cnt + 0);
+        HIPC(hipGetLastError());
+        STAGE("group flags + word scan + count");
+    }
+    BWTS_TRY(read_small(ctx, SM_COUNTERS, 4));
+    r0->a = ctx->h_small[CNT_ACTIVE];
+    r0->seam = r0->lean && ctx->h_small[CNT_SEAM] != 0;
+    return BWTS_OK;
+}
+
+static SortPlan round0_plan(const SortSpace &sp, bool cyclic)
+{
     SortPlan plan = sp.plan();
     plan.sym_src = sp.carry_src; plan.sym_buf[0] = sp.carry_buf[0]; plan.sym_buf[1] = sp.carry_buf[1]; plan.sym_final = sp.carry_out;
     plan.vals_identity = true;
-    plan.keys_split = CYCLIC && sp.split_keys && plan.sym_final;
+    plan.keys_split = cyclic && sp.split_keys && plan.sym_final;
     plan.first_hist = plan.keys_split ? sp.first_hist : nullptr;
+    return plan;
+}
+
+template <bool CYCLIC>
+static int round0_sort(bwts_ctx *ctx, u64 n, const Alphabet &al, SortSpace &sp, bool lean_ok, Round0 *r0)
+{
+    u64 *cnt = ctx->d_small + SM_COUNTERS;
+    SortPlan plan = round0_plan(sp, CYCLIC);
     if (CYCLIC && sp.split_keys && !plan.keys_split) return BWTS_E_INTERNAL;
+    BWTS_TRY(round0_flag_words(ctx, n, sp, r0));
+    r0->lean = lean_ok && plan.keys_split && al.key_bits > 32 && al.key_bits <= 40;
+    HIPC(hipMemsetAsync(cnt, 0, 4 * sizeof(u64), ctx->stream));
+    if (r0->lean) {
+        const u64 words = (n + 63) / 64;
+        HIPC(hipMemsetAsync(r0->headw, 0xff, words * sizeof(u64), ctx->stream));
+        HIPC(hipMemsetAsync(r0->keepw, 0, words * sizeof(u64), ctx->stream));
+        flag_tail_kernel<<<dim3(1), dim3(64), 0, ctx->stream>>>(r0->headw, n);
+        HIPC(hipGetLastError());
+        plan.lean_last = true; plan.headw = r0->headw; plan.keepw = r0->keepw; plan.seam_giveup = ctx->d_small + CNT_SEAM;
+    }
     int res = 0;
     STAGE("cyclic patch (before round 0)");
     BWTS_TRY(radix_sort_pairs(ctx, plan, n, al.key_bits, &res));
     STAGE("round-0 sort");
     u64 *K0 = sp.keys[res];
-    K0Keys k0v{K0, nullptr, nullptr};
-    if (plan.keys_split) k0v = K0Keys{nullptr, (const u32 *)K0, al.key_bits > 32 ? (const u8 *)K0 + align_up((size_t)n * 4, 256) : nullptr};
-
-    HIPC(hipMemsetAsync(cnt, 0, 4 * sizeof(u64), ctx->stream));
-    const u64 words = (n + 63) / 64;
-    u64 *headw, *keepw, *pre;
-    const bool flags_outside_rank = sp.carry_buf[0] && sp.carry_buf[1] && n >= 4096;
-    {
-        SpanGuard g(ctx, BWTS_K_RERANK, n, (k0v.wide ? 8 : k0v.hi ? 5 : 4) * n);
-        if (flags_outside_rank) {
-            headw = (u64 *)sp.carry_buf[0]; keepw = headw + words; pre = (u64 *)sp.carry_buf[1];
-        } else {
-            BWTS_TRY(ensure_rank(ctx, sp, n));
-            headw = (u64 *)sp.rank; keepw = headw + words; pre = keepw + words;
-        }
-        u64 waves = (words + GF_WORDS - 1) / GF_WORDS;
-        unsigned blocks = (unsigned)((waves + 3) / 4 < 16384 ? (waves + 3) / 4 : 16384);
-        if (k0v.wide) group_flags_kernel<GfWide><<<dim3(blocks), dim3(256), 0, ctx->stream>>>(GfWide{K0, ~0ull}, n, headw, keepw);
-        else if (k0v.hi) group_flags_kernel<GfSplit<true>><<<dim3(blocks), dim3(256), 0, ctx->stream>>>(GfSplit<true>{k0v.lo, k0v.hi}, n, headw, keepw);
-        else group_flags_kernel<GfSplit<false>><<<dim3(blocks), dim3(256), 0, ctx->stream>>>(GfSplit<false>{k0v.lo, nullptr}, n, headw, keepw);
-        WordIn in{headw, keepw};
-        ScanStoreArr<u64> out{pre};
-        BWTS_TRY((device_scan<false, u64>(ctx, words, in, out, OpHeadCount(), (u64)0, sp.scan_temp)));
-        count_tied_kernel<<<dim3(1), dim3(64), 0, ctx->stream>>>(keepw, pre, words, cnt + 0);
-        HIPC(hipGetLastError());
-        STAGE("group flags + word scan + count");
-    }
-    BWTS_TRY(read_small(ctx, SM_COUNTERS, 4));
-    *r0 = Round0{res, k0v, sp.vals[res], headw, keepw, pre, flags_outside_rank, ctx->h_small[CNT_ACTIVE]};
-    return BWTS_OK;
+    r0->res = res;
+    r0->k0v = K0Keys{K0, nullptr, nullptr};
+    if (plan.keys_split) r0->k0v = K0Keys{nullptr, (const u32 *)K0, al.key_bits > 32 ? (const u8 *)K0 + align_up((size_t)n * 4, 256) : nullptr};
+    r0->SA = sp.vals[res];
+    return round0_flags(ctx, n, sp, r0);
+}
+
+static int round0_redo_classic(bwts_ctx *ctx, u64 n, SortSpace &sp, Round0 *r0)
+{
+    HIPC(hipMemsetAsync(ctx->d_small + SM_COUNTERS, 0, 4 * sizeof(u64), ctx->stream));
+    BWTS_TRY(radix_packed_last_pass(ctx, round0_plan(sp, true), n));
+    STAGE("round-0 sort: classic last pass");
+    r0->lean = false;
+    return round0_flags(ctx, n, sp, r0);
 }
 
 static int early_ranks(bwts_ctx *ctx, u64 n, SortSpace &sp, const Round0 &r0)
@@ -1244,9 +1309,17 @@
 static int tied_list(bwts_ctx *ctx, u64 n, SortSpace &sp, const Round0 &r0, ActiveList *cur)
 {
     u64 *cnt = ctx->d_small + SM_COUNTERS;
-    cur->idx = (u32 *)sp.keys[r0.res ^ 1];
-    cur->slot = cur->idx + n;
-    cur->head = sp.vals[r0.res ^ 1];
+    if (r0.lean) {
+        if (r0.a > n / 32) return BWTS_E_INTERNAL;
+        const u64 cap = n / 32 + 1;
+        cur->idx = (u32 *)sp.keys[r0.res];
+        cur->slot = cur->idx + cap;
+        cur->head = cur->slot + cap;
+    } else {
+        cur->idx = (u32 *)sp.keys[r0.res ^ 1];
+        cur->slot = cur->idx + n;
+        cur->head = sp.vals[r0.res ^ 1];
+    }
     SpanGuard g(ctx, BWTS_K_RERANK, r0.a, 12 * r0.a);
     const u64 waves = ((n + 63) / 64 + 63) / 64;
     const unsigned blocks = (unsigned)((waves + 3) / 4 < 16384 ? (waves + 3) / 4 : 16384);
@@ -1537,8 +1610,24 @@
 static int doubling_sort(bwts_ctx *ctx, const u8 *d_T, u64 n, const Alphabet &al, const u32 *d_fstart, u64 k,
                          SortSpace &sp, bool want_ranks, u32 **sa_out, u32 *rounds_out, u64 *active0_out)
 {
+    const bool direct_ok = CYCLIC && sp.carry_out && !want_ranks && direct_ties_allowed(ctx, n);
+    const bool lean_off = [ctx] { const char *e = bwts_knob(ctx, "BWTS_RX_LEAN"); return e && atoi(e) == 0; }();
+    const bool lean_ok = direct_ok && al.few_ties && !lean_off;
     Round0 r0;
-    BWTS_TRY((round0_sort<CYCLIC>(ctx, n, al, sp, &r0)));
+    BWTS_TRY((round0_sort<CYCLIC>(ctx, n, al, sp, lean_ok, &r0)));
+    u64 lean = FR_LEAN_NONE, direct = FR_DIRECT_NONE;
+    ActiveList cur, none{nullptr, nullptr, nullptr};
+    bool listed = false;
+    if (r0.lean) {
+        lean = r0.seam ? FR_LEAN_SEAM : r0.a > n / 32 ? FR_LEAN_COUNT : FR_LEAN_HELD;
+        if (lean == FR_LEAN_HELD) {
+            BWTS_TRY(tied_list(ctx, n, sp, r0, &cur));
+            listed = true;
+            if (r0.a > 0) BWTS_TRY(direct_ties(ctx, d_T, n, al, d_fstart, k, sp, cur, r0.a, &direct));
+            if (r0.a > 0 && direct != FR_DIRECT_SETTLED) lean = FR_LEAN_DIRECT;
+        }
+        if (lean != FR_LEAN_HELD) { BWTS_TRY(round0_redo_classic(ctx, n, sp, &r0)); listed = false; }
+    }
     u64 a = r0.a;
     u32 *SA = r0.SA;
     *active0_out = a;
@@ -1548,16 +1637,14 @@
     rep[FR_CYCLIC] = CYCLIC; rep[FR_N] = n; rep[FR_K] = k; rep[FR_SIGMA] = (u64)al.sigma; rep[FR_BITS] = (u64)al.bits; rep[FR_MSYM] = (u64)al.msym;
     rep[FR_KEY_BITS] = (u64)al.key_bits; rep[FR_VARLEN] = al.varlen; rep[FR_HSTEP] = (u64)al.hstep;
     rep[FR_KEYS] = r0.k0v.wide ? 0 : r0.k0v.hi ? 2 : 1; rep[FR_FLAGS_OUTSIDE_RANK] = r0.flags_outside_rank; rep[FR_TIED0] = a;
-    rep[FR_RANK_EARLY] = rank_early; rep[FR_ROUNDS] = 1;
+    rep[FR_RANK_EARLY] = rank_early; rep[FR_ROUNDS] = 1; rep[FR_LEAN] = lean;
     if (rank_early) BWTS_TRY(early_ranks(ctx, n, sp, r0));
-    ActiveList cur, none{nullptr, nullptr, nullptr};
-    BWTS_TRY(tied_list(ctx, n, sp, r0, &cur));
+    if (!listed) BWTS_TRY(tied_list(ctx, n, sp, r0, &cur));
     u32 rounds = 1;
 
     if (a > 0xffffffffull) return BWTS_E_NOMEM;
     if (a > 0 && a <= n / 32) {
-        u64 direct = FR_DIRECT_NONE;
-        if (CYCLIC && sp.carry_out && !want_ranks && direct_ties_allowed(ctx, n)) BWTS_TRY(direct_ties(ctx, d_T, n, al, d_fstart, k, sp, cur, a, &direct));
+        if (direct_ok && direct == FR_DIRECT_NONE) BWTS_TRY(direct_ties(ctx, d_T, n, al, d_fstart, k, sp, cur, a, &direct));
         rep[FR_DIRECT] = direct;
         if (direct == FR_DIRECT_SETTLED) {
             rounds++;
diff --git a/bijective-bwt_amd/csrc/internal.h b/bijective-bwt_amd/csrc/internal.h
--- a/bijective-bwt_amd/csrc/internal.h
+++ b/bijective-bwt_amd/csrc/internal.h
@@ -215,6 +215,8 @@
     bool vals_identity = false;
     bool keys_split = false;
     u32 *first_hist = nullptr;
+    bool lean_last = false;
+    u64 *headw = nullptr, *keepw = nullptr, *seam_giveup = nullptr;
 };
 static inline SortPlan sort_plan(u64 *k0, u64 *k1, u32 *v0, u32 *v1, u32 *tile_hist, void *scan_temp)
 {
@@ -225,6 +227,7 @@
 bool radix_packed_applicable(const bwts_ctx *ctx, u64 m, int key_bits);
 size_t radix_tile_hist_bytes(u64 m);
 int radix_sort_pairs(bwts_ctx *ctx, const SortPlan &plan, u64 m, int key_bits, int *result_buf);
+int radix_packed_last_pass(bwts_ctx *ctx, const SortPlan &plan, u64 m);
 int radix_column_scan(bwts_ctx *ctx, u32 *tile_hist, u64 tiles, void *scan_temp);
 int radix_sort_keys(bwts_ctx *ctx, u64 *keys[2], u32 *tile_hist, void *scan_temp, u64 m, int lo_bit, int bits, int *result_buf);
 
diff --git a/bijective-bwt_amd/csrc/radix.hip b/bijective-bwt_amd/csrc/radix.hip
--- a/bijective-bwt_amd/csrc/radix.hip
+++ b/bijective-bwt_amd/csrc/radix.hip
@@ -432,6 +432,155 @@
 #undef PK_VALID
 }
 
+#define LEAN_SEAM 64
+#define LEAN_REACH 1024
+static_assert(LEAN_REACH % LEAN_SEAM == 0 && LEAN_REACH <= RX_TILE, "the elements before a tile that is not the first are all there");
+struct LeanIO {
+    const u32 *lo_in; const u16 *c_in; const u32 *val_in;
+    u8 *sym_out;
+    u32 *val_out;
+    u64 *headw, *keepw, *giveup;
+};
+
+__global__ __launch_bounds__(RX_THREADS, RX_MINW) void radix_scatter_lean_last_kernel(LeanIO io, const u32 *__restrict__ tile_off, u64 m)
+{
+    extern __shared__ __attribute__((aligned(16))) char rx_smem[];
+    using L = RxTile<RX_THREADS, RX_ITEMS>;
+    u32 *stage32 = (u32 *)L::stage(rx_smem);
+    u32 *dbase = L::dbase(rx_smem), *gbase = L::gbase(rx_smem), *scan_sm = L::scan_sm(rx_smem);
+    u16 (*whist)[256] = L::whist(rx_smem);
+    const int tid = threadIdx.x, lane = tid & 63, w = tid >> 6;
+    const u64 tile = rx_tile_of_block((m + RX_TILE - 1) / RX_TILE);
+    const u64 tile_base = tile * RX_TILE;
+    if (tile_base >= m) return;
+    const u64 wave_base = tile_base + (u64)w * (64 * RX_ITEMS);
+    const u64 remain = m - tile_base;
+    const u32 tile_count = remain < RX_TILE ? (u32)remain : (u32)RX_TILE;
+
+    for (int i = tid; i < RX_WAVES * 128; i += RX_THREADS) ((u32 *)whist)[i] = 0;
+
+    const u64 i0 = wave_base + (u64)lane;
+    u32 vmask = 0;
+#pragma unroll
+    for (int j = 0; j < RX_ITEMS; j++) vmask |= (i0 + (u64)j * 64 < m ? 1u : 0u) << j;
+#define PK_VALID(j) ((vmask >> (j)) & 1u)
+
+    u32 dsrc[RX_ITEMS], lo[RX_ITEMS];
+    Pos16<RX_ITEMS> pos;
+    {
+        const u16 *c16 = io.c_in + i0;
+        const u32 *lop = io.lo_in + i0;
+#pragma unroll
+        for (int j = 0; j < RX_ITEMS; j++) dsrc[j] = PK_VALID(j) ? (u32)c16[j * 64] : 0xffffu;
+#pragma unroll
+        for (int j = 0; j < RX_ITEMS; j++) lo[j] = PK_VALID(j) ? lop[j * 64] : 0u;
+    }
+    const bool has_before = tile_base > 0, has_after = tile_base + RX_TILE + (u64)lane < m;
+    u32 b_lo = 0, b_c = 0, a_lo = 0, a_c = 0;
+    if (w == 0) {
+        if (has_before) { const u64 i = tile_base - 1 - (u64)lane; b_lo = io.lo_in[i]; b_c = io.c_in[i]; }
+        if (has_after) { const u64 i = tile_base + RX_TILE + (u64)lane; a_lo = io.lo_in[i]; a_c = io.c_in[i]; }
+    }
+    const u32 lo_first = io.lo_in[tile_base], lo_last = io.lo_in[tile_base + tile_count - 1];
+    __syncthreads();
+#pragma unroll
+    for (int j = 0; j < RX_ITEMS; j++) {
+        const bool valid = PK_VALID(j);
+        wave_rank_step(whist[w], dsrc[j] & 255u, valid, [&](u32 r) { pos.init(j, r); });
+    }
+    __syncthreads();
+    {
+        const u32 exc = digit_bases<RX_WAVES>(whist, scan_sm);
+        if (tid < 256) {
+            dbase[tid] = exc;
+            gbase[tid] = tile_off[tile * 256 + tid] - exc;
+        }
+    }
+    __syncthreads();
+
+    constexpr int HB = 8;
+    u32 *lo_s = stage32, *cx_s = stage32 + RX_TILE;
+#pragma unroll
+    for (int j0 = 0; j0 < RX_ITEMS; j0 += HB) {
+        u32 add[HB];
+#pragma unroll
+        for (int jj = 0; jj < HB; jj++) {
+            const u32 d = dsrc[j0 + jj] & 255u;
+            add[jj] = dbase[d] + whist[w][d];
+        }
+#pragma unroll
+        for (int jj = 0; jj < HB; jj++) {
+            const int j = j0 + jj;
+            const u32 p = pos.get(j) + add[jj];
+            if (PK_VALID(j)) {
+                lo_s[p] = lo[j];
+                cx_s[p] = dsrc[j] | ((u32)w * (64u * RX_ITEMS) + (u32)j * 64u + (u32)lane) << 16;
+            }
+        }
+    }
+    u32 *seam = (u32 *)whist;
+    if (w == 0) {
+        __builtin_amdgcn_fence(__ATOMIC_ACQ_REL, "wavefront");
+        if (lane < 16) seam[lane] = 0;
+        __builtin_amdgcn_fence(__ATOMIC_ACQ_REL, "wavefront");
+        const auto in_run = [](u64 match) { return ~match ? (u32)__ffsll((unsigned long long)~match) - 1u : (u32)LEAN_SEAM; };
+        u32 run_b = in_run(__ballot(has_before && b_lo == lo_first)), run_a = in_run(__ballot(has_after && a_lo == lo_last));
+        if ((u32)lane < run_b) atomicOr(&seam[(b_c & 255u) >> 5], 1u << (b_c & 31u));
+        if ((u32)lane < run_a) atomicOr(&seam[8 + ((a_c & 255u) >> 5)], 1u << (a_c & 31u));
+        for (u32 off = LEAN_SEAM; run_b == off && off < LEAN_REACH; off += LEAN_SEAM) {
+            const u64 i = tile_base - 1 - off - (u64)lane;
+            const u32 l = io.lo_in[i], c = io.c_in[i];
+            const u32 r = in_run(__ballot(l == lo_first));
+            if ((u32)lane < r) atomicOr(&seam[(c & 255u) >> 5], 1u << (c & 31u));
+            run_b += r;
+        }
+        for (u32 off = LEAN_SEAM; run_a == off && off < LEAN_REACH; off += LEAN_SEAM) {
+            const u64 i = tile_base + RX_TILE + off + (u64)lane;
+            const bool there = i < m;
+            const u32 l = there ? io.lo_in[i] : 0u, c = there ? (u32)io.c_in[i] : 0u;
+            const u32 r = in_run(__ballot(there && l == lo_last));
+            if ((u32)lane < r) atomicOr(&seam[8 + ((c & 255u) >> 5)], 1u << (c & 31u));
+            run_a += r;
+        }
+        const bool undecided = run_b == LEAN_REACH || (run_a == LEAN_REACH && tile_base + RX_TILE + LEAN_REACH < m);
+        if (undecided && lane == 0) __hip_atomic_store(io.giveup, (u64)1, __ATOMIC_RELAXED, __HIP_MEMORY_SCOPE_AGENT);
+    }
+    __syncthreads();
+#pragma unroll
+    for (int j0 = 0; j0 < RX_ITEMS; j0 += HB) {
+        u32 cx[HB], x[HB], xp[HB], xn[HB], g[HB];
+#pragma unroll
+        for (int jj = 0; jj < HB; jj++) {
+            const u32 s = (u32)(j0 + jj) * RX_THREADS + tid;
+            const u32 sc = s < tile_count ? s : 0u;
+            cx[jj] = cx_s[sc];
+            x[jj] = lo_s[sc];
+            xp[jj] = lo_s[sc ? sc - 1u : 0u];
+            xn[jj] = lo_s[sc + 1u < tile_count ? sc + 1u : sc];
+        }
+#pragma unroll
+        for (int jj = 0; jj < HB; jj++) g[jj] = gbase[cx[jj] & 255u];
+#pragma unroll
+        for (int jj = 0; jj < HB; jj++) {
+            const u32 s = (u32)(j0 + jj) * RX_THREADS + tid;
+            if (s >= tile_count) continue;
+            const u32 dst = g[jj] + s;
+            io.sym_out[dst] = (u8)(cx[jj] >> 8);
+            const bool eq_p = s > 0 && xp[jj] == x[jj], eq_n = s + 1u < tile_count && xn[jj] == x[jj];
+            if (!(eq_p || eq_n || x[jj] == lo_first || x[jj] == lo_last)) continue;
+            const u32 d = cx[jj] & 255u;
+            const bool run_first = s == 0 || (cx_s[s - 1u] & 255u) != d, run_last = s + 1u == tile_count || (cx_s[s + 1u] & 255u) != d;
+            const bool same_p = run_first ? x[jj] == lo_first && ((seam[d >> 5] >> (d & 31u)) & 1u) : eq_p;
+            const bool same_n = run_last ? x[jj] == lo_last && ((seam[8 + (d >> 5)] >> (d & 31u)) & 1u) : eq_n;
+            if (!(same_p || same_n)) continue;
+            io.val_out[dst] = io.val_in[tile_base + (cx[jj] >> 16)];
+            __hip_atomic_fetch_or(&io.keepw[dst >> 6], 1ull << (dst & 63u), __ATOMIC_RELAXED, __HIP_MEMORY_SCOPE_AGENT);
+            if (same_p) __hip_atomic_fetch_and(&io.headw[dst >> 6], ~(1ull << (dst & 63u)), __ATOMIC_RELAXED, __HIP_MEMORY_SCOPE_AGENT);
+        }
+    }
+#undef PK_VALID
+}
+
 static bool knob_off(const bwts_ctx *ctx, const char *name) { const char *e = bwts_knob(ctx, name); return e && atoi(e) == 0; }
 
 template <typename T>
@@ -467,31 +616,49 @@
 }
 
 template <bool HI16>
-static int radix_sort_packed(bwts_ctx *ctx, const SortPlan &plan, u64 m, int passes, int *result_buf)
+static int radix_packed_pass(bwts_ctx *ctx, const SortPlan &plan, u64 m, int p, int passes, int cur, bool lean)
 {
     const size_t lo_bytes = align_up((size_t)m * 4, 256);
     const u64 pass_bytes = HI16 ? 20 : 18;
+    const int shift = 8 * p;
+    const bool first = p == 0, last = p == passes - 1;
+    char *src = (char *)plan.keys[cur], *dst = (char *)plan.keys[cur ^ 1];
+    PackedIO io{};
+    io.lo_in = (const u32 *)src; io.c_in = src + lo_bytes; io.val_in = plan.vals[cur];
+    io.lo_out = (u32 *)dst; io.c_out = dst + lo_bytes; io.val_out = plan.vals[cur ^ 1];
+    io.hi_out = (u8 *)dst + lo_bytes; io.sym_out = plan.sym_final;
+    u32 *tile_hist = first && plan.first_hist ? plan.first_hist : plan.tile_hist;
+    const bool counted = tile_hist != plan.tile_hist;
+    if (HI16 && shift >= 32) BWTS_TRY(radix_pass_offsets(ctx, (const u16 *)io.c_in, m, 0, tile_hist, counted, plan.scan_temp));
+    else BWTS_TRY(radix_pass_offsets(ctx, io.lo_in, m, shift, tile_hist, counted, plan.scan_temp));
+    if (lean) {
+        if (!HI16 || !last || !plan.headw || !plan.keepw || !plan.seam_giveup) return BWTS_E_INTERNAL;
+        const LeanIO lio{io.lo_in, (const u16 *)io.c_in, io.val_in, io.sym_out, io.val_out, plan.headw, plan.keepw, plan.seam_giveup};
+        return launch_scatter(ctx, radix_scatter_lean_last_kernel, m, 7 * m, false, lio, tile_hist, m);
+    }
+    const u64 bytes = first ? pass_bytes - 4 : last ? pass_bytes / 2 + (HI16 ? 10 : 9) : pass_bytes;
+    const auto kernel = first ? radix_scatter_packed_kernel<true, false, HI16>
+                      : last  ? radix_scatter_packed_kernel<false, true, HI16> : radix_scatter_packed_kernel<false, false, HI16>;
+    return launch_scatter(ctx, kernel, m, bytes * m, !first && !last, io, tile_hist, m, shift);
+}
+
+template <bool HI16>
+static int radix_sort_packed(bwts_ctx *ctx, const SortPlan &plan, u64 m, int passes, int *result_buf)
+{
+    if (plan.lean_last && passes != 5) return BWTS_E_INTERNAL;
     int cur = 0;
     for (int p = 0; p < passes; p++) {
-        const int shift = 8 * p;
-        const bool first = p == 0, last = p == passes - 1;
-        char *src = (char *)plan.keys[cur], *dst = (char *)plan.keys[cur ^ 1];
-        PackedIO io{};
-        io.lo_in = (const u32 *)src; io.c_in = src + lo_bytes; io.val_in = plan.vals[cur];
-        io.lo_out = (u32 *)dst; io.c_out = dst + lo_bytes; io.val_out = plan.vals[cur ^ 1];
-        io.hi_out = (u8 *)dst + lo_bytes; io.sym_out = plan.sym_final;
-        u32 *tile_hist = first && plan.first_hist ? plan.first_hist : plan.tile_hist;
-        const bool counted = tile_hist != plan.tile_hist;
-        if (HI16 && shift >= 32) BWTS_TRY(radix_pass_offsets(ctx, (const u16 *)io.c_in, m, 0, tile_hist, counted, plan.scan_temp));
-        else BWTS_TRY(radix_pass_offsets(ctx, io.lo_in, m, shift, tile_hist, counted, plan.scan_temp));
-        const u64 bytes = first ? pass_bytes - 4 : last ? pass_bytes / 2 + (HI16 ? 10 : 9) : pass_bytes;
-        const auto kernel = first ? radix_scatter_packed_kernel<true, false, HI16>
-                          : last  ? radix_scatter_packed_kernel<false, true, HI16> : radix_scatter_packed_kernel<false, false, HI16>;
-        BWTS_TRY(launch_scatter(ctx, kernel, m, bytes * m, !first && !last, io, tile_hist, m, shift));
+        BWTS_TRY(radix_packed_pass<HI16>(ctx, plan, m, p, passes, cur, plan.lean_last && p == passes - 1));
         cur ^= 1;
     }
     *result_buf = cur;
     return BWTS_OK;
+}
+
+int radix_packed_last_pass(bwts_ctx *ctx, const SortPlan &plan, u64 m)
+{
+    if (!plan.keys_split || !plan.sym_final) return BWTS_E_INTERNAL;
+    return radix_packed_pass<true>(ctx, plan, m, 4, 5, 0, false);
 }
 
 #define RS_THREADS 1024
@@ -668,6 +835,7 @@
     if (key_bits < 1) key_bits = 1;
     if (key_bits > 64) key_bits = 64;
     const int passes = (key_bits + 7) / 8;
+    if (plan.lean_last && !plan.keys_split) return BWTS_E_INTERNAL;
 
     if (!knob_off(ctx, "BWTS_RX_SMALL") && m <= RS_MAX && !plan.sym_src && !plan.vals_identity && !plan.keys_split) {
         SpanGuard g(ctx, BWTS_K_RADIX_SCATTER, m, 24 * m);
```

New measurement: 36270, median of 6. +8.8%, better.
